# nelaturuharsha/TurboPrune

Measured on NVIDIA H100. Metric: images_per_sec_resnet50_erk80_train_step, higher is better.
Workload: dtype bf16

## Files before the change

include/turboprune_b200.h:

```cpp
#ifndef TURBOPRUNE_B200_H
#define TURBOPRUNE_B200_H

#include <stddef.h>
#include <stdint.h>

#ifdef __cplusplus
extern "C" {
#endif

#define TP_OK                 0
#define TP_ERR_INVALID       -1
#define TP_ERR_WORKSPACE     -2
#define TP_ERR_CUDA          -3
#define TP_ERR_K_RANGE       -4
#define TP_ERR_UNSUPPORTED   -5
#define TP_ERR_DEVICE        -6

const char* tp_strerror(int code);
const char* tp_last_cuda_error(void);
int         tp_abi_version(void);
int         tp_device_sm_count(void);
int         tp_set_pdl(int on);

#define TP_SCORE_MAG      0
#define TP_SCORE_SNIP     1
#define TP_SCORE_SYNFLOW  2

size_t tp_topk_workspace_bytes(int n_seg, int64_t total_numel);
int tp_topk_threshold_mask(const void* const* w, const void* const* g, const void* const* m,
                           void* const* mask_out, const int64_t* numel, int n_seg,
                           int64_t k, int score_kind, float* thr_out,
                           void* ws, size_t ws_bytes, int64_t* info_out, void* stream);
int tp_topk_enqueue(const void* const* w, const void* const* g, const void* const* m,
                    void* const* mask_out, const int64_t* numel, int n_seg,
                    int64_t k, int score_kind, float* thr_out,
                    void* ws, size_t ws_bytes, int table_cached, void* stream);
int tp_topk_finish(const void* const* m, void* const* mask_out, const int64_t* numel, int n_seg,
                   int64_t k, int score_kind, float* thr_out,
                   void* ws, size_t ws_bytes, int64_t* info_out, void* stream);

int tp_apply_threshold(const void* const* w, const void* const* g, const void* const* m,
                       void* const* mask_out, const int64_t* numel, int n_seg,
                       int score_kind, const float* thr, void* ws, size_t ws_bytes, void* stream);

int tp_count_zeros(const void* const* m, const int64_t* numel, int n_seg,
                   int64_t* zeros_out, void* ws, size_t ws_bytes, void* stream);

size_t tp_rigl_workspace_bytes(int n_seg, int64_t total_numel);
int tp_rigl_select(const void* const* w, const void* const* g, const void* const* mask, void* const* new_mask_out,
                   const int64_t* numel, const int64_t* k, int n_seg, int64_t* counts_out, void* ws, size_t ws_bytes,
                   void* stream);
int tp_rigl_apply(void* const* mask, const void* const* new_mask, void* const* w, void* const* momentum,
                  const int64_t* numel, int n_seg, void* ws, size_t ws_bytes, void* stream);
int tp_rigl_apply_states(void* const* mask, const void* const* new_mask, void* const* w, void* const* states, int n_states,
                         const int64_t* numel, int n_seg, void* ws, size_t ws_bytes, void* stream);

int tp_stage_weights(const void* w, const void* mask, int cout, int cin, int r, int s,
                     void* wf, int cin_p, int wf_ld, void* wd, int cout_p, int cin_p2,
                     void* kmask_f, void* kmask_d, void* stream);
size_t tp_kblock_mask_words(int64_t columns);

typedef struct tp_stage_item {
  const void* w; const void* mask;
  void* wf; void* wd;
  int32_t cout, cin, r, s, cin_p, cout_p, wf_ld;
  void* kmask_f; void* kmask_d;
} tp_stage_item;
size_t tp_stage_batched_workspace_bytes(int n_items);
int tp_stage_weights_batched(const tp_stage_item* items, int n_items, int table_cached, void* kmask_all, size_t kmask_bytes,
                             void* ws, size_t ws_bytes, void* stream);

int tp_to_nhwc_bf16(const void* src, int src_dtype, int64_t sn, int64_t sc, int64_t sh, int64_t sw,
                    int n, int c, int h, int w, void* dst, int c_pad, void* stream);

int tp_im2col_c8(const void* x, int n, int h, int w, int r, int s, int stride_h, int stride_w,
                 int pad_h, int pad_w, int p, int q, void* xcol, int kp, void* stream);

int tp_im2col_stem(const void* src, int src_dtype, int64_t sn, int64_t sc, int64_t sh, int64_t sw,
                   int n, int c, int h, int w, int r, int s, int cg, int stride_h, int stride_w, int pad_h, int pad_w,
                   int p, int q, void* xcol, int kp, void* stream);

int tp_cifar_augment(const void* src, void* out, const int64_t* idx, const int64_t* shifts, const uint8_t* flip,
                     const int64_t* cut_y, const int64_t* cut_x, int cut_size,
                     int n, int c, int h, int w, int r, void* stream);
typedef struct tp_crop_entry {
  const void* src;
  int32_t H, W;
  int32_t top, left, h, w;
  int32_t flip;
  int32_t reserved;
} tp_crop_entry;
int tp_resized_crop(const tp_crop_entry* table, int n, int size, const float* mean255, const float* std255, void* out,
                    void* stream);
int tp_synth_normal(void* out, int64_t numel, uint64_t seed, uint64_t counter_offset, int raw_words, void* stream);
int tp_synth_labels(void* out, int64_t numel, int num_classes, uint64_t seed, uint64_t counter_offset, void* stream);

typedef struct tp_conv_desc {
  int32_t n, h, w, cin;
  int32_t cout, r, s;
  int32_t stride_h, stride_w, pad_h, pad_w;
  int32_t p, q;
} tp_conv_desc;

size_t tp_conv_workspace_bytes(const tp_conv_desc* d, int op);

int tp_conv_fprop(const tp_conv_desc* d, const void* x, const void* wf, const void* bias_f32,
                  void* y, void* ws, size_t ws_bytes, void* stream);
size_t tp_conv_stats_rows(const tp_conv_desc* d);
int tp_conv_fprop_stats(const tp_conv_desc* d, const void* x, const void* wf, const void* kmask_f, const void* bias_f32,
                        void* y, void* stats, void* ws, size_t ws_bytes, void* stream);
int tp_conv_dgrad(const tp_conv_desc* d, const void* dy, const void* wd, const void* kmask_d, const void* addend,
                  void* dx, void* ws, size_t ws_bytes, void* stream);
size_t tp_conv_dgrad_partial_rows(const tp_conv_desc* d);
int tp_conv_dgrad_bnrelu(const tp_conv_desc* d, const void* dy, const void* wd, const void* kmask_d,
                         const void* bn_y, const void* bn_weight, const void* bn_bias, const void* bn_mean, const void* bn_invstd,
                         void* g, void* partial, void* stream);
int tp_conv_wgrad(const tp_conv_desc* d, const void* x, const void* dy, const void* mask, const void* kmask_f,
                  int cin_real, void* dw, void* db, void* ws, size_t ws_bytes, void* stream);

int tp_conv_fprop_f32(const tp_conv_desc* d, const void* x, const void* wf, const void* bias_f32, void* y, void* stream);
int tp_conv_dgrad_f32(const tp_conv_desc* d, const void* dy, const void* wd, void* dx, void* stream);
int tp_wgrad_split3(const void* src, int64_t sn, int64_t sc, int64_t sh, int64_t sw,
                    int n, int c, int h, int w, void* dst, int c_pad, int lo_block, void* stream);
int tp_stage_weights_f32(const void* w, const void* mask, int cout, int cin, int r, int s,
                         void* wf, int cin_p, int wf_ld, void* wd, int cout_p, void* stream);
int tp_stage_weights_batched_f32(const tp_stage_item* items, int n_items, int table_cached, void* ws, size_t ws_bytes,
                                 void* stream);
int tp_to_nhwc_f32(const void* src, int64_t sn, int64_t sc, int64_t sh, int64_t sw,
                   int n, int c, int h, int w, void* dst, int c_pad, void* stream);
int tp_im2col_stem_f32(const void* src, int64_t sn, int64_t sc, int64_t sh, int64_t sw,
                       int n, int c, int h, int w, int r, int s, int cg, int stride_h, int stride_w, int pad_h, int pad_w,
                       int p, int q, void* xcol, int kp, void* stream);

int tp_bn_forward_ext(const void* y, const void* residual, void* z, int64_t M, int C,
                      const void* weight, const void* bias, void* running_mean, void* running_var,
                      void* num_batches_tracked, float momentum, float eps, int training, int relu,
                      void* save_mean, void* save_invstd, const void* ext_stats, int64_t ext_rows,
                      void* ws, size_t ws_bytes, void* stream);

size_t tp_bn_workspace_bytes(int64_t m, int c);
int tp_bn_forward(const void* y, const void* residual, void* z, int64_t m, int c,
                  const void* weight, const void* bias, void* running_mean, void* running_var,
                  void* num_batches_tracked, float momentum, float eps, int training, int relu,
                  void* save_mean, void* save_invstd, void* ws, size_t ws_bytes, void* stream);
int tp_bn_backward(const void* dz, const void* z, const void* y, int64_t m, int c, const void* weight, const void* bias,
                   const void* save_mean, const void* save_invstd, int relu, void* dy, void* dres,
                   void* dweight, void* dbias, void* ws, size_t ws_bytes, void* stream);

int tp_bn_backward_ext(const void* g, const void* y, int64_t M, int C, const void* weight, const void* bias,
                       const void* save_mean, const void* save_invstd, const void* partial_rows, int64_t n_rows,
                       void* dy, void* dweight, void* dbias, void* ws, size_t ws_bytes, void* stream);
int tp_maxpool_forward(const void* x, void* y, void* idx, int n, int h, int w, int c, int k, int stride, int pad,
                       int p, int q, void* stream);
int tp_maxpool_backward(const void* dy, const void* idx, void* dx, int n, int h, int w, int c, int k, int stride, int pad,
                        int p, int q, void* stream);

int tp_sgd_momentum(void* const* w, const void* const* g, void* const* buf, const int64_t* numel,
                    int n_seg, const float* lr_dev, float momentum, float weight_decay,
                    int first_step, int table_cached, void* ws, size_t ws_bytes, void* stream);
size_t tp_segtable_workspace_bytes(int n_seg);
int tp_adamw(void* const* w, const void* const* g, void* const* exp_avg, void* const* exp_avg_sq, void* const* step,
             const int64_t* numel, int n_seg, const float* inv_lr_dev, const float* decay_dev,
             double beta1, double beta2, double eps, int table_cached, void* ws, size_t ws_bytes, void* stream);

int tp_p2p_allreduce_mask(void* const* peer_bufs, void* const* signal_pads, int rank, int world,
                          int64_t numel, const void* mask, float scale, void* out,
                          int algo, int timeout_ms, int* status_dev, void* stream);

int tp_p2p_allreduce_nvls(void* const* peer_bufs, void* const* signal_pads, void* multicast_buf, int rank, int world,
                          int64_t numel, const void* mask, float scale, void* out,
                          int timeout_ms, int* status_dev, void* stream);

#ifdef __cplusplus
}
#endif
#endif
```

turboprune_b200/_cabi.py:

```python
import ctypes
import os
from ctypes import POINTER, c_char_p, c_double, c_float, c_int, c_int32, c_int64, c_size_t, c_uint64, c_void_p

from . import build as _build

TP_SCORE_MAG, TP_SCORE_SNIP, TP_SCORE_SYNFLOW = 0, 1, 2
TP_ERR_K_RANGE = -4

_lib = None


class ConvDesc(ctypes.Structure):
    _fields_ = [(n, c_int32) for n in
                ("n", "h", "w", "cin", "cout", "r", "s", "stride_h", "stride_w", "pad_h", "pad_w", "p", "q")]


class StageItem(ctypes.Structure):
    _fields_ = [("w", c_void_p), ("mask", c_void_p), ("wf", c_void_p), ("wd", c_void_p)] + \
               [(n, c_int32) for n in ("cout", "cin", "r", "s", "cin_p", "cout_p", "wf_ld")] + \
               [("kmask_f", c_void_p), ("kmask_d", c_void_p)]


class CropEntry(ctypes.Structure):
    _fields_ = [("src", c_void_p)] + [(n, c_int32) for n in ("H", "W", "top", "left", "h", "w", "flip", "reserved")]


SIGNATURES = {
    "tp_strerror": (c_char_p, [c_int]),
    "tp_last_cuda_error": (c_char_p, []),
    "tp_abi_version": (c_int, []),
    "tp_device_sm_count": (c_int, []),
    "tp_set_pdl": (c_int, [c_int]),
    "tp_topk_workspace_bytes": (c_size_t, [c_int, c_int64]),
    "tp_topk_threshold_mask": (c_int, [POINTER(c_void_p), POINTER(c_void_p), POINTER(c_void_p), POINTER(c_void_p),
                                       POINTER(c_int64), c_int, c_int64, c_int, c_void_p, c_void_p, c_size_t,
                                       POINTER(c_int64), c_void_p]),
    "tp_topk_enqueue": (c_int, [POINTER(c_void_p), POINTER(c_void_p), POINTER(c_void_p), POINTER(c_void_p),
                                POINTER(c_int64), c_int, c_int64, c_int, c_void_p, c_void_p, c_size_t, c_int, c_void_p]),
    "tp_topk_finish": (c_int, [POINTER(c_void_p), POINTER(c_void_p), POINTER(c_int64), c_int, c_int64, c_int, c_void_p,
                               c_void_p, c_size_t, POINTER(c_int64), c_void_p]),
    "tp_apply_threshold": (c_int, [POINTER(c_void_p), POINTER(c_void_p), POINTER(c_void_p), POINTER(c_void_p),
                                   POINTER(c_int64), c_int, c_int, c_void_p, c_void_p, c_size_t, c_void_p]),
    "tp_count_zeros": (c_int, [POINTER(c_void_p), POINTER(c_int64), c_int, c_void_p, c_void_p, c_size_t, c_void_p]),
    "tp_rigl_workspace_bytes": (c_size_t, [c_int, c_int64]),
    "tp_rigl_select": (c_int, [POINTER(c_void_p), POINTER(c_void_p), POINTER(c_void_p), POINTER(c_void_p), POINTER(c_int64),
                               POINTER(c_int64), c_int, c_void_p, c_void_p, c_size_t, c_void_p]),
    "tp_rigl_apply": (c_int, [POINTER(c_void_p), POINTER(c_void_p), POINTER(c_void_p), POINTER(c_void_p), POINTER(c_int64), c_int,
                              c_void_p, c_size_t, c_void_p]),
    "tp_stage_weights": (c_int, [c_void_p, c_void_p, c_int, c_int, c_int, c_int, c_void_p, c_int, c_int, c_void_p, c_int,
                                 c_int, c_void_p, c_void_p, c_void_p]),
    "tp_kblock_mask_words": (c_size_t, [c_int64]),
    "tp_stage_batched_workspace_bytes": (c_size_t, [c_int]),
    "tp_stage_weights_batched": (c_int, [POINTER(StageItem), c_int, c_int, c_void_p, c_size_t, c_void_p, c_size_t, c_void_p]),
    "tp_to_nhwc_bf16": (c_int, [c_void_p, c_int, c_int64, c_int64, c_int64, c_int64, c_int, c_int, c_int, c_int,
                                c_void_p, c_int, c_void_p]),
    "tp_im2col_c8": (c_int, [c_void_p] + [c_int] * 11 + [c_void_p, c_int, c_void_p]),
    "tp_im2col_stem": (c_int, [c_void_p, c_int, c_int64, c_int64, c_int64, c_int64] + [c_int] * 13 + [c_void_p, c_int, c_void_p]),
    "tp_cifar_augment": (c_int, [c_void_p, c_void_p, c_void_p, c_void_p, c_void_p, c_void_p, c_void_p, c_int, c_int, c_int, c_int, c_int, c_int, c_void_p]),
    "tp_resized_crop": (c_int, [c_void_p, c_int, c_int, POINTER(c_float), POINTER(c_float), c_void_p, c_void_p]),
    "tp_synth_normal": (c_int, [c_void_p, c_int64, c_uint64, c_uint64, c_int, c_void_p]),
    "tp_synth_labels": (c_int, [c_void_p, c_int64, c_int, c_uint64, c_uint64, c_void_p]),
    "tp_conv_workspace_bytes": (c_size_t, [POINTER(ConvDesc), c_int]),
    "tp_conv_fprop": (c_int, [POINTER(ConvDesc), c_void_p, c_void_p, c_void_p, c_void_p, c_void_p, c_size_t, c_void_p]),
    "tp_conv_stats_rows": (c_size_t, [POINTER(ConvDesc)]),
    "tp_conv_fprop_stats": (c_int, [POINTER(ConvDesc), c_void_p, c_void_p, c_void_p, c_void_p, c_void_p, c_void_p, c_void_p, c_size_t, c_void_p]),
    "tp_conv_dgrad": (c_int, [POINTER(ConvDesc), c_void_p, c_void_p, c_void_p, c_void_p, c_void_p, c_void_p, c_size_t, c_void_p]),
    "tp_conv_dgrad_partial_rows": (c_size_t, [POINTER(ConvDesc)]),
    "tp_conv_dgrad_bnrelu": (c_int, [POINTER(ConvDesc), c_void_p, c_void_p, c_void_p, c_void_p, c_void_p, c_void_p, c_void_p, c_void_p,
                                     c_void_p, c_void_p, c_void_p]),
    "tp_bn_backward_ext": (c_int, [c_void_p, c_void_p, c_int64, c_int, c_void_p, c_void_p, c_void_p, c_void_p, c_void_p, c_int64,
                                   c_void_p, c_void_p, c_void_p, c_void_p, c_size_t, c_void_p]),
    "tp_conv_wgrad": (c_int, [POINTER(ConvDesc), c_void_p, c_void_p, c_void_p, c_void_p, c_int, c_void_p, c_void_p, c_void_p,
                              c_size_t, c_void_p]),
    "tp_sgd_momentum": (c_int, [POINTER(c_void_p), POINTER(c_void_p), POINTER(c_void_p), POINTER(c_int64), c_int,
                                c_void_p, c_float, c_float, c_int, c_int, c_void_p, c_size_t, c_void_p]),
    "tp_segtable_workspace_bytes": (c_size_t, [c_int]),
    "tp_adamw": (c_int, [POINTER(c_void_p), POINTER(c_void_p), POINTER(c_void_p), POINTER(c_void_p), POINTER(c_void_p),
                         POINTER(c_int64), c_int, c_void_p, c_void_p, c_double, c_double, c_double, c_int, c_void_p,
                         c_size_t, c_void_p]),
    "tp_rigl_apply_states": (c_int, [POINTER(c_void_p), POINTER(c_void_p), POINTER(c_void_p), POINTER(c_void_p), c_int,
                                     POINTER(c_int64), c_int, c_void_p, c_size_t, c_void_p]),
    "tp_p2p_allreduce_mask": (c_int, [POINTER(c_void_p), POINTER(c_void_p), c_int, c_int, c_int64, c_void_p, c_float,
                                      c_void_p, c_int, c_int, c_void_p, c_void_p]),
    "tp_bn_workspace_bytes": (c_size_t, [c_int64, c_int]),
    "tp_bn_forward": (c_int, [c_void_p, c_void_p, c_void_p, c_int64, c_int, c_void_p, c_void_p, c_void_p, c_void_p, c_void_p,
                              c_float, c_float, c_int, c_int, c_void_p, c_void_p, c_void_p, c_size_t, c_void_p]),
    "tp_bn_forward_ext": (c_int, [c_void_p, c_void_p, c_void_p, c_int64, c_int, c_void_p, c_void_p, c_void_p, c_void_p, c_void_p,
                                  c_float, c_float, c_int, c_int, c_void_p, c_void_p, c_void_p, c_int64, c_void_p, c_size_t, c_void_p]),
    "tp_bn_backward": (c_int, [c_void_p, c_void_p, c_void_p, c_int64, c_int, c_void_p, c_void_p, c_void_p, c_void_p, c_int, c_void_p,
                               c_void_p, c_void_p, c_void_p, c_void_p, c_size_t, c_void_p]),
    "tp_maxpool_forward": (c_int, [c_void_p, c_void_p, c_void_p] + [c_int] * 9 + [c_void_p]),
    "tp_maxpool_backward": (c_int, [c_void_p, c_void_p, c_void_p] + [c_int] * 9 + [c_void_p]),
    "tp_p2p_allreduce_nvls": (c_int, [POINTER(c_void_p), POINTER(c_void_p), c_void_p, c_int, c_int, c_int64, c_void_p, c_float,
                                      c_void_p, c_int, c_void_p, c_void_p]),
    "tp_conv_fprop_f32": (c_int, [POINTER(ConvDesc), c_void_p, c_void_p, c_void_p, c_void_p, c_void_p]),
    "tp_conv_dgrad_f32": (c_int, [POINTER(ConvDesc), c_void_p, c_void_p, c_void_p, c_void_p]),
    "tp_wgrad_split3": (c_int, [c_void_p, c_int64, c_int64, c_int64, c_int64, c_int, c_int, c_int, c_int, c_void_p, c_int, c_int,
                                c_void_p]),
    "tp_stage_weights_f32": (c_int, [c_void_p, c_void_p, c_int, c_int, c_int, c_int, c_void_p, c_int, c_int, c_void_p, c_int,
                                     c_void_p]),
    "tp_stage_weights_batched_f32": (c_int, [POINTER(StageItem), c_int, c_int, c_void_p, c_size_t, c_void_p]),
    "tp_to_nhwc_f32": (c_int, [c_void_p, c_int64, c_int64, c_int64, c_int64, c_int, c_int, c_int, c_int, c_void_p, c_int, c_void_p]),
    "tp_im2col_stem_f32": (c_int, [c_void_p, c_int64, c_int64, c_int64, c_int64] + [c_int] * 13 + [c_void_p, c_int, c_void_p]),
}


def lib_path() -> str:
    return _build.lib_path()


def load(build_if_missing: bool = False):
    global _lib
    if _lib is not None:
        return _lib
    path = lib_path()
    if not os.path.isfile(path):
        if build_if_missing:
            _build.build()
        else:
            raise RuntimeError(
                f"turboprune_b200: CUDA library not built ({path} missing). "
                "Run `python -c 'import __graft_entry__ as g; g.build()'`; there is no CPU fallback.")
    lib = ctypes.CDLL(path)
    for name, (res, args) in SIGNATURES.items():
        fn = getattr(lib, name)
        fn.restype = res
        fn.argtypes = args
    _lib = lib
    return lib


class TurboPruneError(RuntimeError):
    def __init__(self, code, where):
        lib = load()
        msg = lib.tp_strerror(code).decode()
        detail = lib.tp_last_cuda_error().decode() if code == -3 else ""
        super().__init__(f"{where}: {msg} (code {code}) {detail}".strip())
        self.code = code


def check(code: int, where: str):
    if code != 0:
        raise TurboPruneError(code, where)


def ptr_array(tensors):
    if tensors is None:
        return None
    arr = (c_void_p * len(tensors))()
    for i, t in enumerate(tensors):
        arr[i] = t.data_ptr() if t is not None else None
    return arr


def i64_array(vals):
    arr = (c_int64 * len(vals))()
    for i, v in enumerate(vals):
        arr[i] = int(v)
    return arr


def stream_ptr(device=None):
    import torch
    return c_void_p(torch.cuda.current_stream(device).cuda_stream)
```

turboprune_b200/csrc/tp_igemm.cu:

```cuda
#include "tp_common.cuh"
#include "tp_ptx.cuh"
#include <cuda.h>
#include <mutex>

namespace tp {
using namespace ptx;

constexpr int kBlockM = 128;
constexpr int kBlockK = 64;
constexpr int kConsumers = 256;
constexpr int kThreads = kConsumers + 32;
constexpr int kProducerWarp = kConsumers / 32;
constexpr int kFwdThreads = 3 * 128;
constexpr int kMaxTaps = 64;

constexpr int kFwdProducerRegs = 56, kFwdConsumerRegs = 224;
static_assert(kFwdProducerRegs * 128 + kFwdConsumerRegs * 256 <= 168 * kFwdThreads, "fwd register split");

__host__ __device__ constexpr int fwd_stages(int block_n) { return block_n == 128 ? 5 : 8; }
__host__ __device__ constexpr int fwd_stg_bytes(int block_n) { return kBlockM * block_n * 2; }
__host__ __device__ constexpr int fwd_smem(int block_n) {
  return fwd_stages(block_n) * (kBlockM * kBlockK * 2 + block_n * kBlockK * 2) + 2 * fwd_stg_bytes(block_n) + 1024 + 512;
}

struct TapEntry { uint16_t off_w, off_h; int32_t kofs; };

constexpr int kMaxCls = 4;

struct ClsEntry {
  int M;
  int P_it, Q_it;
  int ntaps, tap0;
  int base_w, base_h;
  int oah, oaw;
  int tile0, m_groups;
};

struct FwdParams {
  int M, N;
  int ncls;
  ClsEntry cls[kMaxCls];
  int cchunks;
  int a_mode;
  int step_w, step_h;
  long long out_img_pix;
  int out_row_pix;
  int osh, osw;
  int linear;
  int ldc;
  int staged_store;
  __nv_bfloat16* out;
  const float* bias;
  const __nv_bfloat16* addend;
  float* stats;
  const __nv_bfloat16* bn_y;
  const float* bn_weight; const float* bn_bias; const float* bn_mean; const float* bn_invstd;
  const uint32_t* kmask;
  int kmask_words;
  TapEntry taps[kMaxTaps];
};

__device__ __forceinline__ const uint32_t* live_kmask(const uint32_t* km, int words, int N) {
  if (km && __ldg(km + (size_t)((N + 63) >> 6) * words) == 0u) return nullptr;
  return km;
}

struct KSkip {
  const uint32_t* base; int words, g0, g1; int cur_w; uint32_t bits;
  __device__ __forceinline__ void begin(const uint32_t* km, int wds, int n0, int block_n, int N) {
    base = km; words = wds; cur_w = -1; bits = 0u;
    g0 = n0 >> 6; g1 = min((min(n0 + block_n, N) + 63) >> 6, ((N + 63) >> 6));
  }
  __device__ __forceinline__ bool on(int kb) {
    const int wi = kb >> 5;
    if (wi != cur_w) {
      cur_w = wi; bits = 0u;
      if (wi < words) for (int g = g0; g < g1; ++g) bits |= __ldg(base + (size_t)g * words + wi);
      else bits = 0xffffffffu;
    }
    return (bits >> (kb & 31)) & 1u;
  }
  __device__ __forceinline__ bool take(int kb, bool last, bool any) { return on(kb) || (last && !any); }
};

struct WgParams {
  int Mc;
  int Kpix;
  int P_it, Q_it;
  int chunks, cchunks;
  int nb;
  int b_mode;
  int base_w, base_h, step_w, step_h;
  int m_tiles, n_tiles, splits, kb_per_split, kblocks;
  float* partial;
  const uint32_t* kmask;
  int kmask_words;
  TapEntry taps[kMaxTaps];
};

struct WgItem {
  int split, tile, m_t, n_t, chunk0, nvalid, kb0, kb1;
  __device__ __forceinline__ void set_tile(int m, int n, int m_tiles, int nb, int chunks) {
    m_t = m; n_t = n; tile = n * m_tiles + m;
    chunk0 = n * nb; nvalid = min(nb, chunks - chunk0);
  }
  __device__ __forceinline__ bool empty(const uint32_t* __restrict__ km, int words, int Mc) const {
    const int row_groups = (Mc + 63) >> 6;
    for (int r = 2 * m_t; r < 2 * m_t + 2 && r < row_groups; ++r)
      for (int c = chunk0; c < chunk0 + nvalid; ++c)
        if ((__ldg(km + (size_t)r * words + (c >> 5)) >> (c & 31)) & 1u) return false;
    return true;
  }
};

__device__ __forceinline__ WgItem wg_item(const WgParams& p, int nb, int item) {
  WgItem w;
  const int ntile = p.m_tiles * p.n_tiles;
  w.split = item / ntile;
  const int tile = item - w.split * ntile, n_t = tile / p.m_tiles;
  w.set_tile(tile - n_t * p.m_tiles, n_t, p.m_tiles, nb, p.chunks);
  w.kb0 = w.split * p.kb_per_split; w.kb1 = min(p.kblocks, w.kb0 + p.kb_per_split);
  return w;
}

__device__ __forceinline__ void decompose_pixel(int m, int P, int Q, int& n, int& p, int& q) {
  q = m % Q; int t = m / Q; p = t % P; n = t / P;
}

struct AMaps { CUtensorMap m[kMaxCls]; };

__device__ __forceinline__ void decode_tile(const FwdParams& p, int tile, int n_tiles, int& c, int& m_g, int& n_t) {
  c = 0;
#pragma unroll
  for (int j = 1; j < kMaxCls; ++j) if (j < p.ncls && tile >= p.cls[j].tile0) c = j;
  const int local = tile - p.cls[c].tile0;
  m_g = local / n_tiles; n_t = local - m_g * n_tiles;
}

template <int BLOCK_N, typename T = __nv_bfloat16>
__device__ __forceinline__ void fwd_mma_block(float (&acc)[BLOCK_N], uint32_t a_addr, uint32_t b_addr, uint32_t accumulate) {
  const uint64_t adesc = make_smem_desc(a_addr, 16, 1024);
  const uint64_t adesc_hi = make_smem_desc(a_addr + 64 * kBlockK * 2, 16, 1024);
  const uint64_t bdesc = make_smem_desc(b_addr, 16, 1024);
#pragma unroll
  for (int k = 0; k < kBlockK / 16; ++k) {
    if constexpr (sizeof(T) == 4) {
      if constexpr (BLOCK_N == 128) {
        wgmma_m64n128_tf32(acc, adesc + (uint64_t)(2 * k), bdesc + (uint64_t)(2 * k), accumulate | (uint32_t)k);
        wgmma_m64n128_tf32(acc + BLOCK_N / 2, adesc_hi + (uint64_t)(2 * k), bdesc + (uint64_t)(2 * k), accumulate | (uint32_t)k);
      } else {
        wgmma_m64n64_tf32(acc, adesc + (uint64_t)(2 * k), bdesc + (uint64_t)(2 * k), accumulate | (uint32_t)k);
        wgmma_m64n64_tf32(acc + BLOCK_N / 2, adesc_hi + (uint64_t)(2 * k), bdesc + (uint64_t)(2 * k), accumulate | (uint32_t)k);
      }
    } else if constexpr (BLOCK_N == 128) {
      wgmma_m64n128<0, 0>(acc, adesc + (uint64_t)(2 * k), bdesc + (uint64_t)(2 * k), accumulate | (uint32_t)k);
      wgmma_m64n128<0, 0>(acc + BLOCK_N / 2, adesc_hi + (uint64_t)(2 * k), bdesc + (uint64_t)(2 * k), accumulate | (uint32_t)k);
    } else {
      wgmma_m64n64<0, 0>(acc, adesc + (uint64_t)(2 * k), bdesc + (uint64_t)(2 * k), accumulate | (uint32_t)k);
      wgmma_m64n64<0, 0>(acc + BLOCK_N / 2, adesc_hi + (uint64_t)(2 * k), bdesc + (uint64_t)(2 * k), accumulate | (uint32_t)k);
    }
  }
}

template <int BLOCK_N, bool MULTI, bool BNB, typename T = __nv_bfloat16>
__global__ void __launch_bounds__(kFwdThreads, 1)
k_igemm_fwd(const __grid_constant__ AMaps tmA, const __grid_constant__ CUtensorMap tmB,
            const __grid_constant__ FwdParams p) {
  static_assert(BLOCK_N == 64 || BLOCK_N == 128, "wgmma N of the fwd kernel");
  static_assert(!BNB || !MULTI, "BatchNorm-backward epilogue: single class");
  constexpr bool kF32 = sizeof(T) == 4;
  static_assert(!kF32 || !BNB, "fp32 operands: no BatchNorm-backward epilogue");
  constexpr int kKe = 128 / (int)sizeof(T);
  constexpr int kABytes = kBlockM * kBlockK * 2;
  constexpr int kBBytes = BLOCK_N * kBlockK * 2;
  constexpr int kStageBytes = kABytes + kBBytes;
  constexpr int kStages = fwd_stages(BLOCK_N);
  extern __shared__ __align__(1024) uint8_t smem_raw[];
  uint8_t* smem = (uint8_t*)(((uintptr_t)smem_raw + 1023) & ~(uintptr_t)1023);
  pdl_trigger();
  constexpr int kStgBytes = fwd_stg_bytes(BLOCK_N);
  constexpr int kChunkStg = kBlockM * 64 * 2;
  uint8_t* const stg_base = smem + kStages * kStageBytes;
  uint64_t* full_bar = (uint64_t*)(stg_base + 2 * kStgBytes);
  uint64_t* empty_bar = full_bar + kStages;
  uint64_t* order_bar = empty_bar + kStages;
  int* ring_pos = (int*)(order_bar + 2);

  const int warp = threadIdx.x >> 5, lane = threadIdx.x & 31;
  const int n_tiles = (p.N + BLOCK_N - 1) / BLOCK_N;
  const int total_tiles = p.cls[p.ncls - 1].tile0 + p.cls[p.ncls - 1].m_groups * n_tiles;
  const int my_items = total_tiles > (int)blockIdx.x ? (total_tiles - (int)blockIdx.x + (int)gridDim.x - 1) / (int)gridDim.x : 0;
  auto get_tile = [&](int w, int& ci, int& m_g, int& n_t) {
    ci = 0;
    const int tile = (int)blockIdx.x + w * (int)gridDim.x;
    if (MULTI) decode_tile(p, tile, n_tiles, ci, m_g, n_t);
    else { m_g = tile / n_tiles; n_t = tile - m_g * n_tiles; }
  };

  if (threadIdx.x == 0) {
    for (int j = 0; j < p.ncls; ++j) prefetch_tmap(&tmA.m[j]);
    prefetch_tmap(&tmB);
    for (int i = 0; i < kStages; ++i) { mbar_init(&full_bar[i], 1); mbar_init(&empty_bar[i], 1); }
    mbar_init(&order_bar[0], 1); mbar_init(&order_bar[1], 1);
    fence_mbar_init();
  }
  __syncthreads();
  pdl_wait();

  if (warp < 4) {
    setmaxnreg_dec<kFwdProducerRegs>();
    if (threadIdx.x == 0) {
      int stage = 0; uint32_t phase = 0;
      const uint32_t* const km = kF32 ? nullptr : live_kmask(p.kmask, p.kmask_words, p.N);
      for (int w = 0; w < my_items; ++w) {
        int ci, m_g, n_t; get_tile(w, ci, m_g, n_t);
        const ClsEntry& ce = p.cls[MULTI ? ci : 0];
        const CUtensorMap* const mapA = &tmA.m[MULTI ? ci : 0];
        const int m0 = m_g * kBlockM;
        int cn = 0, cp = 0, cq = 0;
        if (p.a_mode == 1) decompose_pixel(m0, ce.P_it, ce.Q_it, cn, cp, cq);
        const int cw = ce.base_w + cq * p.step_w, ch = ce.base_h + cp * p.step_h;
        auto load_block = [&](const TapEntry& te, int cc) {
          mbar_wait(&empty_bar[stage], phase ^ 1);
          uint8_t* sA = smem + stage * kStageBytes;
          uint8_t* sB = sA + kABytes;
          mbar_arrive_expect_tx(&full_bar[stage], kStageBytes);
          if (p.a_mode == 1)
            tma_load_im2col_4d(sA, mapA, &full_bar[stage], cc * kKe, cw, ch, cn, te.off_w, te.off_h);
          else
            tma_load_2d(sA, mapA, &full_bar[stage], te.kofs + cc * kKe, m0);
          tma_load_2d(sB, &tmB, &full_bar[stage], te.kofs + cc * kKe, n_t * BLOCK_N);
          if (++stage == kStages) { stage = 0; phase ^= 1; }
        };
        const int tap_base = MULTI ? ce.tap0 : 0;
        if (!km) {
          for (int tap = 0; tap < ce.ntaps; ++tap) {
            const TapEntry te = p.taps[tap_base + tap];
            for (int cc = 0; cc < p.cchunks; ++cc) load_block(te, cc);
          }
        } else {
          KSkip ks; bool any = false;
          ks.begin(km, p.kmask_words, n_t * BLOCK_N, BLOCK_N, p.N);
          for (int tap = 0; tap < ce.ntaps; ++tap) {
            const TapEntry te = p.taps[tap_base + tap];
            for (int cc = 0; cc < p.cchunks; ++cc) {
              const bool last = tap == ce.ntaps - 1 && cc == p.cchunks - 1;
              if (!ks.take((te.kofs >> 6) + cc, last, any)) continue;
              any = true;
              load_block(te, cc);
            }
          }
        }
      }
    }
  } else {
    setmaxnreg_inc<kFwdConsumerRegs>();
    const int cw = (warp >> 2) - 1;
    const int q = warp & 3;
    const int wtid = threadIdx.x & 127;
    const int bar_id = 1 + cw;
    const uint32_t* const km = kF32 ? nullptr : live_kmask(p.kmask, p.kmask_words, p.N);
    const uint32_t stg = smem_u32(stg_base + cw * kStgBytes);
    const int fr0 = q * 16 + (lane >> 2);
    const uint32_t fsw = (uint32_t)(lane >> 2);
    const uint32_t frag_base = stg + (uint32_t)(fr0 * 128 + (lane & 3) * 4);
    const int r_in = lane >> 3, c16 = lane & 7;
    const uint32_t buf = stg + (uint32_t)(q * 32 * 128);
    const uint32_t rd_even = buf + r_in * 128 + ((uint32_t)(c16 ^ r_in) << 4);
    const uint32_t rd_odd = buf + (r_in + 4) * 128 + ((uint32_t)(c16 ^ (r_in + 4)) << 4);
    for (int it = 0, w = cw; w < my_items; ++it, w += 2) {
      int ci, m_g, n_t; get_tile(w, ci, m_g, n_t);
      const ClsEntry& ce = p.cls[MULTI ? ci : 0];
      const bool has_acc = MULTI ? ce.ntaps > 0 : true;
      const int m_t = m_g;

      int stage = 0; uint32_t phase = 0;
      const int turn = it + cw;
      if (turn > 0) {
        mbar_wait(&order_bar[cw], (uint32_t)((turn - 1) & 1));
        const int pos = *(volatile int*)ring_pos;
        stage = pos >> 1; phase = (uint32_t)(pos & 1);
      }
      bar_sync(bar_id, 128);
      auto pass_turn = [&]() {
        if (wtid == 0) { *(volatile int*)ring_pos = stage * 2 + (int)phase; mbar_arrive(&order_bar[cw ^ 1]); }
      };
      float acc[BLOCK_N];
      if (has_acc) {
#pragma unroll
        for (int i = 0; i < BLOCK_N; ++i) acc[i] = 0.f;
        int prev = -1;
        auto mma_block = [&](uint32_t accumulate) {
          mbar_wait(&full_bar[stage], phase);
          const uint32_t s_addr = smem_u32(smem + stage * kStageBytes);
          wgmma_fence();
          fwd_mma_block<BLOCK_N, T>(acc, s_addr, s_addr + kABytes, accumulate);
          wgmma_commit();
          wgmma_wait<1>();
          if (prev >= 0 && wtid == 0) mbar_arrive(&empty_bar[prev]);
          prev = stage;
          if (++stage == kStages) { stage = 0; phase ^= 1; }
        };
        KSkip ks; uint32_t any = 0;
        if (km) ks.begin(km, p.kmask_words, n_t * BLOCK_N, BLOCK_N, p.N);
        for (int tap = 0; tap < ce.ntaps; ++tap) {
          const int kb0 = p.taps[(MULTI ? ce.tap0 : 0) + tap].kofs >> 6;
          for (int cc = 0; cc < p.cchunks; ++cc) {
            const bool last = tap == ce.ntaps - 1 && cc == p.cchunks - 1;
            if (km && !ks.take(kb0 + cc, last, any)) continue;
            mma_block(any);
            any = 1;
          }
        }
        pass_turn();
        wgmma_wait<0>();
        acc_fence(acc);
        if (prev >= 0 && wtid == 0) mbar_arrive(&empty_bar[prev]);
      } else {
        pass_turn();
      }

      const long long wrow0 = (long long)m_t * kBlockM + q * 32;
      const int rows_left = (int)(ce.M - wrow0 < 32 ? (ce.M - wrow0 < 0 ? 0 : ce.M - wrow0) : 32);
      const long long ldc = p.ldc;
      const int N = p.N;
      long long ooff[MULTI ? 8 : 1];
      const long long rbase = (wrow0 + r_in) * ldc + c16 * 8;
      if (MULTI && p.staged_store) {
        int n, pp, qq; decompose_pixel((int)(wrow0 + r_in), ce.P_it, ce.Q_it, n, pp, qq);
#pragma unroll
        for (int i = 0; i < 8; ++i) {
          const long long px = (long long)n * p.out_img_pix + (long long)(pp * p.osh + ce.oah) * p.out_row_pix + (qq * p.osw + ce.oaw);
          ooff[i] = px * ldc + c16 * 8;
          qq += 4;
          while (qq >= ce.Q_it) { qq -= ce.Q_it; if (++pp == ce.P_it) { pp = 0; ++n; } }
        }
      }
      auto row_off = [&](int i) -> long long { return MULTI ? ooff[MULTI ? i : 0] : rbase + (long long)(i * 4) * ldc; };
      if constexpr (kF32) {
        float* const out = reinterpret_cast<float*>(p.out);
        const bool pair_ok = (p.ldc & 1) == 0 && (((uintptr_t)out) & 7) == 0;
#pragma unroll
        for (int mh = 0; mh < 2; ++mh)
#pragma unroll
          for (int h = 0; h < 2; ++h) {
            const int row = m_t * kBlockM + fr0 + 8 * h + 64 * mh;
            if (row >= ce.M) continue;
            long long opix = row;
            if (MULTI || !p.linear) {
              int n, pp, qq; decompose_pixel(row, ce.P_it, ce.Q_it, n, pp, qq);
              opix = (long long)n * p.out_img_pix + (long long)(pp * p.osh + ce.oah) * p.out_row_pix + (qq * p.osw + ce.oaw);
            }
            float* const orow = out + opix * p.ldc;
#pragma unroll
            for (int j = 0; j < BLOCK_N / 8; ++j) {
              const int n = n_t * BLOCK_N + 8 * j + 2 * (lane & 3);
              if (n >= N) continue;
              const int i = mh * (BLOCK_N / 2) + 4 * j + 2 * h;
              float f0 = has_acc ? acc[i] : 0.f, f1 = has_acc ? acc[i + 1] : 0.f;
              if (p.bias && has_acc) {
                f0 += p.bias[n];
                if (n + 1 < N) f1 += p.bias[n + 1];
              }
              if (n + 1 < N && pair_ok) *reinterpret_cast<float2*>(orow + n) = make_float2(f0, f1);
              else {
                orow[n] = f0;
                if (n + 1 < N) orow[n + 1] = f1;
              }
            }
          }
        continue;
      }
      if (MULTI && !has_acc) {
        if (p.staged_store) {
#pragma unroll 1
          for (int c = 0; c < BLOCK_N; c += 64) {
            const int n0 = n_t * BLOCK_N + c;
            if (n0 >= N) break;
            if (n0 + c16 * 8 + 8 > N) continue;
            uint4 z[8];
#pragma unroll
            for (int i = 0; i < 8; ++i) {
              z[i] = make_uint4(0u, 0u, 0u, 0u);
              if (p.addend && i * 4 + r_in < rows_left) z[i] = *reinterpret_cast<const uint4*>(p.addend + row_off(i) + n0);
            }
#pragma unroll
            for (int i = 0; i < 8; ++i)
              if (i * 4 + r_in < rows_left) *reinterpret_cast<uint4*>(p.out + row_off(i) + n0) = z[i];
          }
        } else {
          const int row = m_t * kBlockM + wtid;
          if (row < ce.M) {
            int n, pp, qq; decompose_pixel(row, ce.P_it, ce.Q_it, n, pp, qq);
            const long long opix = (long long)n * p.out_img_pix + (long long)(pp * p.osh + ce.oah) * p.out_row_pix + (qq * p.osw + ce.oaw);
            for (int j = n_t * BLOCK_N; j < min(p.N, (n_t + 1) * BLOCK_N); ++j)
              p.out[opix * p.ldc + j] = p.addend ? p.addend[opix * p.ldc + j] : __float2bfloat16_rn(0.f);
          }
        }
        continue;
      }
      if (p.staged_store) {
        __nv_bfloat16* const gout = p.out;
        const __nv_bfloat16* const gadd = p.addend;
        const float* bias = p.bias;
        float* stats = p.stats ? p.stats + (long long)(m_t * 4 + q) * 2 * N + c16 * 8 : nullptr;
        if (gadd) {
          __syncwarp();
#pragma unroll
          for (int ch = 0; ch < BLOCK_N / 64; ++ch) {
            const int n0 = n_t * BLOCK_N + ch * 64;
            if (n0 >= N) break;
            const bool col_ok = n0 + c16 * 8 + 8 <= N;
            uint4 a[8];
#pragma unroll
            for (int i = 0; i < 8; ++i) {
              a[i] = make_uint4(0u, 0u, 0u, 0u);
              if (i * 4 + r_in < rows_left && col_ok) a[i] = *reinterpret_cast<const uint4*>(gadd + row_off(i) + n0);
            }
#pragma unroll
            for (int i = 0; i < 8; ++i) sts128(((i & 1) ? rd_odd : rd_even) + (uint32_t)(ch * kChunkStg + (i >> 1) * 1024), a[i]);
          }
        }
        bar_sync(bar_id, 128);
#pragma unroll
        for (int ch = 0; ch < BLOCK_N / 64; ++ch) {
          const int n0 = n_t * BLOCK_N + ch * 64;
          if (n0 >= N) break;
#pragma unroll
          for (int mh = 0; mh < 2; ++mh)
#pragma unroll
            for (int h = 0; h < 2; ++h)
#pragma unroll
              for (int j = 0; j < 8; ++j) {
                const int i = mh * (BLOCK_N / 2) + 4 * (ch * 8 + j) + 2 * h;
                float f0 = acc[i], f1 = acc[i + 1];
                const int n = n0 + 8 * j + 2 * (lane & 3);
                if (bias) {
                  if (n < N) f0 += bias[n];
                  if (n + 1 < N) f1 += bias[n + 1];
                }
                const uint32_t addr = frag_base + (uint32_t)(ch * kChunkStg + (64 * mh + 8 * h) * 128) + (((uint32_t)j ^ fsw) << 4);
                if (gadd) {
                  const uint32_t a = lds32(addr);
                  const float2 t2 = __bfloat1622float2(*reinterpret_cast<const __nv_bfloat162*>(&a));
                  f0 += t2.x; f1 += t2.y;
                }
                const __nv_bfloat162 hv = __floats2bfloat162_rn(f0, f1);
                sts32(addr, *reinterpret_cast<const uint32_t*>(&hv));
              }
        }
        bar_sync(bar_id, 128);
#pragma unroll 1
        for (int ch = 0; ch < BLOCK_N / 64; ++ch) {
          const int n0 = n_t * BLOCK_N + ch * 64;
          if (n0 >= N) break;
          const bool col_ok = n0 + c16 * 8 + 8 <= N;
          uint4 o[8];
#pragma unroll
          for (int i = 0; i < 8; ++i) o[i] = lds128(((i & 1) ? rd_odd : rd_even) + (uint32_t)(ch * kChunkStg + (i >> 1) * 1024));
          float s1[8], s2[8];
#pragma unroll
          for (int qq = 0; qq < 8; ++qq) { s1[qq] = 0.f; s2[qq] = 0.f; }
          if (BNB) {
            uint4 yv[8];
#pragma unroll
            for (int i = 0; i < 8; ++i) {
              yv[i] = make_uint4(0u, 0u, 0u, 0u);
              if (i * 4 + r_in < rows_left && col_ok) yv[i] = *reinterpret_cast<const uint4*>(p.bn_y + row_off(i) + n0);
            }
            float sc[8], sf[8], is_[8], nm[8];
            if (col_ok) {
              const int cb = n0 + c16 * 8;
#pragma unroll
              for (int qq = 0; qq < 8; qq += 4) {
                const float4 one4 = make_float4(1.f, 1.f, 1.f, 1.f), zero4 = make_float4(0.f, 0.f, 0.f, 0.f);
                const float4 a4 = p.bn_weight ? *reinterpret_cast<const float4*>(p.bn_weight + cb + qq) : one4;
                const float4 b4 = p.bn_bias ? *reinterpret_cast<const float4*>(p.bn_bias + cb + qq) : zero4;
                const float4 m4 = *reinterpret_cast<const float4*>(p.bn_mean + cb + qq), i4 = *reinterpret_cast<const float4*>(p.bn_invstd + cb + qq);
                is_[qq] = i4.x; is_[qq + 1] = i4.y; is_[qq + 2] = i4.z; is_[qq + 3] = i4.w;
                nm[qq] = m4.x; nm[qq + 1] = m4.y; nm[qq + 2] = m4.z; nm[qq + 3] = m4.w;
                sc[qq] = a4.x * i4.x; sc[qq + 1] = a4.y * i4.y; sc[qq + 2] = a4.z * i4.z; sc[qq + 3] = a4.w * i4.w;
                sf[qq] = fmaf(-m4.x, sc[qq], b4.x); sf[qq + 1] = fmaf(-m4.y, sc[qq + 1], b4.y);
                sf[qq + 2] = fmaf(-m4.z, sc[qq + 2], b4.z); sf[qq + 3] = fmaf(-m4.w, sc[qq + 3], b4.w);
              }
            } else {
#pragma unroll
              for (int qq = 0; qq < 8; ++qq) { sc[qq] = 0.f; sf[qq] = 0.f; is_[qq] = 0.f; nm[qq] = 0.f; }
            }
#pragma unroll
            for (int i = 0; i < 8; ++i) {
              if (i * 4 + r_in < rows_left) {
                __nv_bfloat162* gh = reinterpret_cast<__nv_bfloat162*>(&o[i]);
                const __nv_bfloat162* yh = reinterpret_cast<const __nv_bfloat162*>(&yv[i]);
#pragma unroll
                for (int qq = 0; qq < 4; ++qq) {
                  float2 d2 = __bfloat1622float2(gh[qq]);
                  const float2 y2 = __bfloat1622float2(yh[qq]);
                  if (!(fmaf(y2.x, sc[2 * qq], sf[2 * qq]) > 0.f)) d2.x = 0.f;
                  if (!(fmaf(y2.y, sc[2 * qq + 1], sf[2 * qq + 1]) > 0.f)) d2.y = 0.f;
                  gh[qq] = __floats2bfloat162_rn(d2.x, d2.y);
                  s1[2 * qq] += d2.x;     s2[2 * qq] = fmaf(d2.x, (y2.x - nm[2 * qq]) * is_[2 * qq], s2[2 * qq]);
                  s1[2 * qq + 1] += d2.y; s2[2 * qq + 1] = fmaf(d2.y, (y2.y - nm[2 * qq + 1]) * is_[2 * qq + 1], s2[2 * qq + 1]);
                }
              }
            }
          }
#pragma unroll
          for (int i = 0; i < 8; ++i)
            if (i * 4 + r_in < rows_left && col_ok) *reinterpret_cast<uint4*>(gout + row_off(i) + n0) = o[i];
          if (!BNB && stats) {
#pragma unroll
            for (int i = 0; i < 8; ++i) {
              if (i * 4 + r_in < rows_left) {
                const __nv_bfloat162* h2 = reinterpret_cast<const __nv_bfloat162*>(&o[i]);
#pragma unroll
                for (int qq = 0; qq < 4; ++qq) {
                  const float2 t2 = __bfloat1622float2(h2[qq]);
                  s1[2 * qq] += t2.x; s2[2 * qq] = fmaf(t2.x, t2.x, s2[2 * qq]);
                  s1[2 * qq + 1] += t2.y; s2[2 * qq + 1] = fmaf(t2.y, t2.y, s2[2 * qq + 1]);
                }
              }
            }
          }
          if (BNB || stats) {
#pragma unroll
            for (int qq = 0; qq < 8; ++qq) {
              s1[qq] += __shfl_xor_sync(0xffffffffu, s1[qq], 8);  s2[qq] += __shfl_xor_sync(0xffffffffu, s2[qq], 8);
              s1[qq] += __shfl_xor_sync(0xffffffffu, s1[qq], 16); s2[qq] += __shfl_xor_sync(0xffffffffu, s2[qq], 16);
            }
            if (r_in == 0 && col_ok) {
              float4* d1 = reinterpret_cast<float4*>(stats + n0);
              float4* d2 = reinterpret_cast<float4*>(stats + N + n0);
              d1[0] = make_float4(s1[0], s1[1], s1[2], s1[3]); d1[1] = make_float4(s1[4], s1[5], s1[6], s1[7]);
              d2[0] = make_float4(s2[0], s2[1], s2[2], s2[3]); d2[1] = make_float4(s2[4], s2[5], s2[6], s2[7]);
            }
          }
        }
      } else {
#pragma unroll
        for (int mh = 0; mh < 2; ++mh)
#pragma unroll
          for (int h = 0; h < 2; ++h) {
            const int row = m_t * kBlockM + fr0 + 8 * h + 64 * mh;
            if (row >= ce.M) continue;
            long long opix = row;
            if (MULTI || !p.linear) {
              int n, pp, qq; decompose_pixel(row, ce.P_it, ce.Q_it, n, pp, qq);
              opix = (long long)n * p.out_img_pix + (long long)(pp * p.osh + ce.oah) * p.out_row_pix + (qq * p.osw + ce.oaw);
            }
            __nv_bfloat16* const orow = p.out + opix * p.ldc;
#pragma unroll
            for (int j = 0; j < BLOCK_N / 8; ++j)
#pragma unroll
              for (int e = 0; e < 2; ++e) {
                const int n = n_t * BLOCK_N + 8 * j + 2 * (lane & 3) + e;
                if (n >= N) continue;
                float f = acc[mh * (BLOCK_N / 2) + 4 * j + 2 * h + e];
                if (p.bias) f += p.bias[n];
                if (p.addend) f += __bfloat162float(p.addend[opix * p.ldc + n]);
                orow[n] = __float2bfloat16_rn(f);
              }
          }
      }
    }
  }
}

template <int NB>
__device__ __forceinline__ void wgrad_mma_block(float (&acc)[NB * 32], uint32_t a_addr, uint32_t b_addr, bool first) {
  constexpr uint32_t kChunk = 64 * kBlockK * 2;
#pragma unroll
  for (int k = 0; k < kBlockK / 16; ++k) {
    const uint32_t acc_on = (!first || k > 0) ? 1u : 0u;
    const uint64_t adesc = make_smem_desc(a_addr + (uint32_t)(2048 * k), kChunk, 1024);
    const uint32_t bk = b_addr + (uint32_t)(2048 * k);
    if constexpr (NB >= 2) wgmma_m64n128<1, 1>(acc, adesc, make_smem_desc(bk, kChunk, 1024), acc_on);
    else wgmma_m64n64<1, 1>(acc, adesc, make_smem_desc(bk, kChunk, 1024), acc_on);
    if constexpr (NB == 4) wgmma_m64n128<1, 1>(acc + 64, adesc, make_smem_desc(bk + 2 * kChunk, kChunk, 1024), acc_on);
    if constexpr (NB == 3) wgmma_m64n64<1, 1>(acc + 64, adesc, make_smem_desc(bk + 2 * kChunk, kChunk, 1024), acc_on);
  }
}

template <int NB>
__global__ void __launch_bounds__(kThreads, 1)
k_igemm_wgrad(const __grid_constant__ CUtensorMap tmA ,
              const __grid_constant__ CUtensorMap tmB ,
              const __grid_constant__ WgParams p) {
  constexpr int kABytes = kBlockM * kBlockK * 2;
  constexpr int kChunkBytes = 64 * kBlockK * 2;
  constexpr int kMaxNb = 4;
  constexpr int kStageBytes = kABytes + kMaxNb * kChunkBytes;
  constexpr int kStages = 4;
  pdl_trigger();
  extern __shared__ __align__(1024) uint8_t smem_raw[];
  uint8_t* smem = (uint8_t*)(((uintptr_t)smem_raw + 1023) & ~(uintptr_t)1023);
  uint64_t* full_bar = (uint64_t*)(smem + kStages * kStageBytes);
  uint64_t* empty_bar = full_bar + kStages;

  const int warp = threadIdx.x >> 5, lane = threadIdx.x & 31;
  const int items = p.m_tiles * p.n_tiles * p.splits;
  constexpr int ncols = NB * 64;

  if (threadIdx.x == 0) {
    prefetch_tmap(&tmA); prefetch_tmap(&tmB);
    for (int i = 0; i < kStages; ++i) { mbar_init(&full_bar[i], 1); mbar_init(&empty_bar[i], kConsumers / 128); }
    fence_mbar_init();
  }
  __syncthreads();
  pdl_wait();
  const uint32_t* const km = live_kmask(p.kmask, p.kmask_words, p.Mc);

  if (warp == kProducerWarp) {
    if (lane == 0) {
      int stage = 0; uint32_t phase = 0;
      for (int item = blockIdx.x; item < items; item += gridDim.x) {
        const WgItem it = wg_item(p, NB, item);
        if (km && it.empty(km, p.kmask_words, p.Mc)) continue;
        const int m_t = it.m_t, chunk0 = it.chunk0, nvalid = it.nvalid, kb0 = it.kb0, kb1 = it.kb1;
        int c_c[4]; uint16_t c_ow[4], c_oh[4];
#pragma unroll
        for (int j = 0; j < 4; ++j) {
          const int chunk = min(chunk0 + j, p.chunks - 1), tap = chunk / p.cchunks;
          c_c[j] = (chunk - tap * p.cchunks) * 64; c_ow[j] = p.taps[tap].off_w; c_oh[j] = p.taps[tap].off_h;
        }
        int cn, cp, cq; decompose_pixel(kb0 * kBlockK, p.P_it, p.Q_it, cn, cp, cq);
        const int sq = kBlockK % p.Q_it, t1 = kBlockK / p.Q_it, sp = t1 % p.P_it, sn = t1 / p.P_it;
        for (int kb = kb0; kb < kb1; ++kb) {
          const int pix0 = kb * kBlockK;
          mbar_wait(&empty_bar[stage], phase ^ 1);
          mbar_arrive_expect_tx(&full_bar[stage], kABytes + nvalid * kChunkBytes);
          uint8_t* sA = smem + stage * kStageBytes;
          uint8_t* sB = sA + kABytes;
          tma_load_2d(sA, &tmA, &full_bar[stage], m_t * kBlockM, pix0);
          tma_load_2d(sA + kChunkBytes, &tmA, &full_bar[stage], m_t * kBlockM + 64, pix0);
          if (p.b_mode == 1) {
            const int cw = p.base_w + cq * p.step_w, ch = p.base_h + cp * p.step_h;
#pragma unroll
            for (int j = 0; j < 4; ++j)
              if (j < nvalid)
                tma_load_im2col_4d(sB + j * kChunkBytes, &tmB, &full_bar[stage], c_c[j], cw, ch, cn, c_ow[j], c_oh[j]);
            cq += sq; if (cq >= p.Q_it) { cq -= p.Q_it; cp += 1; }
            cp += sp; if (cp >= p.P_it) { cp -= p.P_it; cn += 1; }
            cn += sn;
          } else {
#pragma unroll
            for (int j = 0; j < 4; ++j)
              if (j < nvalid) tma_load_2d(sB + j * kChunkBytes, &tmB, &full_bar[stage], (chunk0 + j) * 64, pix0);
          }
          if (++stage == kStages) { stage = 0; phase ^= 1; }
        }
      }
    }
  } else {
    const int wg = warp >> 2;
    int stage = 0; uint32_t phase = 0;
    for (int item = blockIdx.x; item < items; item += gridDim.x) {
      const WgItem it = wg_item(p, NB, item);
      if (km && it.empty(km, p.kmask_words, p.Mc)) continue;
      const int kb0 = it.kb0, kb1 = it.kb1;
      float acc[NB * 32];
#pragma unroll
      for (int i = 0; i < NB * 32; ++i) acc[i] = 0.f;
      int prev = -1;
      for (int kb = kb0; kb < kb1; ++kb) {
        mbar_wait(&full_bar[stage], phase);
        const uint32_t a_addr = smem_u32(smem + stage * kStageBytes);
        wgmma_fence();
        wgrad_mma_block<NB>(acc, a_addr + (uint32_t)(wg * kChunkBytes), a_addr + kABytes, kb == kb0);
        wgmma_commit();
        wgmma_wait<1>();
        if (prev >= 0 && (threadIdx.x & 127) == 0) mbar_arrive(&empty_bar[prev]);
        prev = stage;
        if (++stage == kStages) { stage = 0; phase ^= 1; }
      }
      wgmma_wait<0>();
      acc_fence(acc);
      if (prev >= 0 && (threadIdx.x & 127) == 0) mbar_arrive(&empty_bar[prev]);
      float* ptile = p.partial + ((long long)it.tile * p.splits + it.split) * kBlockM * ncols;
      const int r0 = wg * 64 + (warp & 3) * 16 + (lane >> 2);
#pragma unroll
      for (int j = 0; j < ncols / 8; ++j)
#pragma unroll
        for (int h = 0; h < 2; ++h)
          *reinterpret_cast<float2*>(ptile + (long long)(r0 + 8 * h) * ncols + 8 * j + 2 * (lane & 3)) =
              make_float2(acc[4 * j + 2 * h], acc[4 * j + 2 * h + 1]);
    }
  }
}

__global__ void __launch_bounds__(256) k_wgrad_finalize(const float* __restrict__ partial, const float* __restrict__ mask,
                                                        float* __restrict__ dw, int cout, int cin_real, int cin_p, int rs,
                                                        int nb, int m_tiles, int splits, int sl,
                                                        const uint32_t* __restrict__ kmask, int kmask_words) {
  pdl_enter();
  __shared__ float s_lane[256];
  const uint32_t* const km = live_kmask(kmask, kmask_words, cout);
  const int co = blockIdx.x;
  const int r = co % kBlockM;
  const int ktot = rs * cin_p;
  const int ncols = nb * 64;
  const int KT = 256 / sl;
  const int kl = threadIdx.x % KT, sj = threadIdx.x / KT;
  const int kk = blockIdx.y * KT + kl;
  const long long sstride = (long long)kBlockM * ncols;
  float a[8] = {0.f, 0.f, 0.f, 0.f, 0.f, 0.f, 0.f, 0.f};
  bool skipped = false;
  if (kk < ktot) {
    const int chunk = kk >> 6;
    WgItem it; it.set_tile(co / kBlockM, chunk / nb, m_tiles, nb, (ktot + 63) >> 6);
    skipped = km && it.empty(km, kmask_words, cout);
    if (!skipped) {
      const float* base = partial + (((long long)it.tile * splits) * kBlockM + r) * ncols + (chunk - it.chunk0) * 64 + (kk & 63);
      int sp = sj;
      for (; sp + 7 * sl < splits; sp += 8 * sl) {
        float v[8];
#pragma unroll
        for (int j = 0; j < 8; ++j) v[j] = __ldcs(base + (long long)(sp + j * sl) * sstride);
#pragma unroll
        for (int j = 0; j < 8; ++j) a[j] += v[j];
      }
      for (; sp < splits; sp += sl) a[0] += __ldcs(base + (long long)sp * sstride);
    }
  }
  s_lane[sj * KT + kl] = ((a[0] + a[1]) + (a[2] + a[3])) + ((a[4] + a[5]) + (a[6] + a[7]));
  __syncthreads();
  if (sj == 0 && kk < ktot) {
    float acc = 0.f;
    for (int j = 0; j < sl; ++j) acc += s_lane[j * KT + kl];
    const int tap = kk / cin_p, ci = kk - tap * cin_p;
    if (ci < cin_real) {
      const long long o = ((long long)co * cin_real + ci) * rs + tap;
      dw[o] = skipped ? 0.f : mask[o] * acc;
    }
  }
}

__global__ void __launch_bounds__(256) k_colsum_part(const __nv_bfloat16* __restrict__ dy, long long npix, int c, int ldc,
                                                     float* __restrict__ part) {
  pdl_enter();
  __shared__ float s_acc[256][9];
  const int tx = threadIdx.x, ty = threadIdx.y, TX = blockDim.x, TY = blockDim.y;
  const int cvec = blockIdx.y * TX + tx;
  const bool act = cvec * 8 < c;
  float a[8];
#pragma unroll
  for (int i = 0; i < 8; ++i) a[i] = 0.f;
  auto add8 = [&](const uint4& v) {
    const __nv_bfloat162* h = reinterpret_cast<const __nv_bfloat162*>(&v);
#pragma unroll
    for (int i = 0; i < 4; ++i) { const float2 f = __bfloat1622float2(h[i]); a[2 * i] += f.x; a[2 * i + 1] += f.y; }
  };
  if (act) {
    const long long stride = (long long)gridDim.x * TY;
    long long p = (long long)blockIdx.x * TY + ty;
    const __nv_bfloat16* src = dy + (size_t)cvec * 8;
    for (; p + 3 * stride < npix; p += 4 * stride) {
      uint4 v[4];
#pragma unroll
      for (int u = 0; u < 4; ++u) v[u] = *reinterpret_cast<const uint4*>(src + (size_t)(p + u * stride) * ldc);
#pragma unroll
      for (int u = 0; u < 4; ++u) add8(v[u]);
    }
    for (; p < npix; p += stride) add8(*reinterpret_cast<const uint4*>(src + (size_t)p * ldc));
  }
  const int tid = ty * TX + tx;
#pragma unroll
  for (int i = 0; i < 8; ++i) s_acc[tid][i] = a[i];
  __syncthreads();
  if (ty == 0 && act) {
    float r[8];
#pragma unroll
    for (int i = 0; i < 8; ++i) r[i] = 0.f;
    for (int j = 0; j < TY; ++j)
#pragma unroll
      for (int i = 0; i < 8; ++i) r[i] += s_acc[j * TX + tx][i];
#pragma unroll
    for (int i = 0; i < 8; ++i) part[(size_t)blockIdx.x * c + cvec * 8 + i] = r[i];
  }
}

__global__ void __launch_bounds__(256) k_colsum_fold(const float* __restrict__ part, int nparts, int c, float* __restrict__ db) {
  pdl_enter();
  const int ch = blockIdx.x * blockDim.x + threadIdx.x;
  if (ch >= c) return;
  float s0 = 0.f, s1 = 0.f, s2 = 0.f, s3 = 0.f;
  int j = 0;
  for (; j + 3 < nparts; j += 4) {
    s0 += part[(size_t)j * c + ch]; s1 += part[(size_t)(j + 1) * c + ch];
    s2 += part[(size_t)(j + 2) * c + ch]; s3 += part[(size_t)(j + 3) * c + ch];
  }
  for (; j < nparts; ++j) s0 += part[(size_t)j * c + ch];
  db[ch] = (s0 + s1) + (s2 + s3);
}

typedef CUresult (*PFN_encodeTiled)(CUtensorMap*, CUtensorMapDataType, cuuint32_t, void*, const cuuint64_t*, const cuuint64_t*,
                                    const cuuint32_t*, const cuuint32_t*, CUtensorMapInterleave, CUtensorMapSwizzle,
                                    CUtensorMapL2promotion, CUtensorMapFloatOOBfill);
typedef CUresult (*PFN_encodeIm2col)(CUtensorMap*, CUtensorMapDataType, cuuint32_t, void*, const cuuint64_t*, const cuuint64_t*,
                                     const int*, const int*, cuuint32_t, cuuint32_t, const cuuint32_t*, CUtensorMapInterleave,
                                     CUtensorMapSwizzle, CUtensorMapL2promotion, CUtensorMapFloatOOBfill);
static PFN_encodeTiled g_encodeTiled = nullptr;
static PFN_encodeIm2col g_encodeIm2col = nullptr;
static int g_driver_version = 0;

static int load_driver_fns() {
  static std::once_flag once;
  static int rc = TP_OK;
  std::call_once(once, []() {
    void* f1 = nullptr; void* f2 = nullptr;
    cudaDriverEntryPointQueryResult q;
    if (cudaGetDriverEntryPoint("cuTensorMapEncodeTiled", &f1, cudaEnableDefault, &q) != cudaSuccess || !f1 ||
        cudaGetDriverEntryPoint("cuTensorMapEncodeIm2col", &f2, cudaEnableDefault, &q) != cudaSuccess || !f2) {
      set_last_cuda_error(cudaErrorUnknown, "cudaGetDriverEntryPoint(cuTensorMapEncode*)");
      rc = TP_ERR_CUDA;
      return;
    }
    g_encodeTiled = (PFN_encodeTiled)f1;
    g_encodeIm2col = (PFN_encodeIm2col)f2;
    cudaDriverGetVersion(&g_driver_version);
  });
  return rc;
}

static int fail_cu(CUresult r, const char* what) {
  static thread_local char buf[128];
  snprintf(buf, sizeof(buf), "%s -> CUresult %d", what, (int)r);
  set_last_cuda_error(cudaErrorInvalidValue, buf);
  return TP_ERR_CUDA;
}

static int make_tiled_map(CUtensorMap* m, const void* ptr, uint64_t cols, uint64_t rows, uint64_t ld_elems, uint32_t box_rows,
                          bool f32 = false) {
  cuuint64_t dims[2] = {cols, rows};
  cuuint64_t strides[1] = {ld_elems * (f32 ? 4 : 2)};
  cuuint32_t box[2] = {f32 ? 32u : 64u, box_rows};
  cuuint32_t es[2] = {1, 1};
  CUresult r = g_encodeTiled(m, f32 ? CU_TENSOR_MAP_DATA_TYPE_FLOAT32 : CU_TENSOR_MAP_DATA_TYPE_BFLOAT16, 2, const_cast<void*>(ptr),
                             dims, strides, box, es,
                             CU_TENSOR_MAP_INTERLEAVE_NONE, CU_TENSOR_MAP_SWIZZLE_128B,
                             CU_TENSOR_MAP_L2_PROMOTION_L2_256B, CU_TENSOR_MAP_FLOAT_OOB_FILL_NONE);
  if (r != CUDA_SUCCESS) return fail_cu(r, "cuTensorMapEncodeTiled");
  return TP_OK;
}

static int make_im2col_map(CUtensorMap* m, const void* ptr, int n, int h, int w, int c,
                           int base_w, int base_h, int step_w, int step_h, int P_it, int Q_it, uint32_t pixels, bool f32 = false) {
  const cuuint64_t es_b = f32 ? 4 : 2;
  cuuint64_t dims[4] = {(cuuint64_t)c, (cuuint64_t)w, (cuuint64_t)h, (cuuint64_t)n};
  cuuint64_t strides[3] = {(cuuint64_t)c * es_b, (cuuint64_t)w * c * es_b, (cuuint64_t)h * w * c * es_b};
  int lower[2] = {base_w, base_h};
  int upper[2] = {(Q_it - 1) * step_w + 1 + base_w - w, (P_it - 1) * step_h + 1 + base_h - h};
  cuuint32_t es[4] = {1, (cuuint32_t)step_w, (cuuint32_t)step_h, 1};
  CUresult r = g_encodeIm2col(m, f32 ? CU_TENSOR_MAP_DATA_TYPE_FLOAT32 : CU_TENSOR_MAP_DATA_TYPE_BFLOAT16, 4, const_cast<void*>(ptr),
                              dims, strides, lower, upper,
                              f32 ? 32 : 64, pixels, es, CU_TENSOR_MAP_INTERLEAVE_NONE, CU_TENSOR_MAP_SWIZZLE_128B,
                              CU_TENSOR_MAP_L2_PROMOTION_L2_256B, CU_TENSOR_MAP_FLOAT_OOB_FILL_NONE);
  if (r != CUDA_SUCCESS) return fail_cu(r, "cuTensorMapEncodeIm2col");
  if (g_driver_version <= 13010 && (size_t)n * h * w * c * es_b < 131072)
    reinterpret_cast<uint64_t*>(m)[1] &= ~(1ull << 21);
  return TP_OK;
}

struct WgGeom {
  int chunks, nb, m_tiles, n_tiles, kblocks, smax;
  size_t partial_bytes(int splits) const { return (size_t)m_tiles * n_tiles * splits * kBlockM * nb * 64 * sizeof(float); }
};

static WgGeom wgrad_geom(const tp_conv_desc* d) {
  WgGeom g;
  g.chunks = (d->r * d->s * d->cin + 63) / 64;
  g.nb = g.chunks >= 4 ? 4 : g.chunks;
  g.m_tiles = (d->cout + kBlockM - 1) / kBlockM;
  g.n_tiles = (g.chunks + g.nb - 1) / g.nb;
  g.kblocks = (int)(((long long)d->n * d->p * d->q + 63) / 64);
  g.smax = (2 * sm_count()) / (g.m_tiles * g.n_tiles);
  if (g.smax > g.kblocks) g.smax = g.kblocks;
  if (g.smax < 1) g.smax = 1;
  return g;
}

static int pick_wgrad_splits(const WgGeom& g) {
  const int sms = sm_count();
  const int tiles = g.m_tiles * g.n_tiles, kblocks = g.kblocks, nb = g.nb;
  const double c_kb = 0.30;
  const double c_part = 0.33 * nb;
  const double c_fin = 0.013 * nb;
  int best = 1; double best_cost = 1e30;
  for (int s = 1; s <= g.smax; ++s) {
    const int kb = (kblocks + s - 1) / s;
    const int s_eff = (kblocks + kb - 1) / kb;
    const long long items = (long long)tiles * s_eff;
    const long long waves = (items + sms - 1) / sms;
    const double cost = (double)waves * (kb * c_kb + c_part) + (double)items * c_fin;
    if (cost < best_cost - 1e-9) { best_cost = cost; best = s_eff; }
  }
  return best;
}

static bool is_plain_gemm(const tp_conv_desc* d) {
  return d->r == 1 && d->s == 1 && d->stride_h == 1 && d->stride_w == 1 && d->pad_h == 0 && d->pad_w == 0;
}

static void fill_taps(TapEntry* taps, int R, int S, int cin) {
  for (int r = 0; r < R; ++r) for (int s = 0; s < S; ++s) {
    TapEntry& t = taps[r * S + s];
    t.off_w = (uint16_t)s; t.off_h = (uint16_t)r; t.kofs = (r * S + s) * cin;
  }
}

static int pick_block_n(long long m_tiles, int n) {
  const int sms = sm_count();
  int best = 64; double best_score = -1;
  const int cands[2] = {128, 64};
  const double weight[2] = {1.0, 0.82};
  for (int i = 0; i < 2; ++i) {
    int bn = cands[i];
    if (bn > 64 && n <= bn / 2) continue;
    long long tiles = m_tiles * ((n + bn - 1) / bn);
    long long waves = (tiles + sms - 1) / sms;
    double eff = (double)tiles / (double)(waves * sms) * weight[i];
    if (eff > best_score) { best_score = eff; best = bn; }
  }
  return best;
}

constexpr int kSmemMax = 232448;

template <int BN, bool MULTI, bool BNB = false, typename T = __nv_bfloat16>
static int launch_fwd(const AMaps& a, const CUtensorMap& b, FwdParams& p, cudaStream_t st) {
  constexpr int smem = fwd_smem(BN);
  static_assert(smem <= kSmemMax, "fwd smem budget");
  const int n_tiles = (p.N + BN - 1) / BN;
  static bool attr_set = false;
  if (!attr_set) {
    TP_CUDA_CHECK(cudaFuncSetAttribute(k_igemm_fwd<BN, MULTI, BNB, T>, cudaFuncAttributeMaxDynamicSharedMemorySize, smem));
    attr_set = true;
  }
  long long ctiles = 0;
  for (int c = 0; c < p.ncls; ++c) {
    p.cls[c].m_groups = (int)((p.cls[c].M + kBlockM - 1) / kBlockM);
    if (ctiles > 0x7fffffffll) return TP_ERR_UNSUPPORTED;
    p.cls[c].tile0 = (int)ctiles;
    ctiles += (long long)p.cls[c].m_groups * n_tiles;
  }
  if (ctiles > 0x7fffffffll || ctiles <= 0) return TP_ERR_UNSUPPORTED;
  const int grid = (int)(ctiles < sm_count() ? ctiles : sm_count());
  TP_CUDA_CHECK(launch(k_igemm_fwd<BN, MULTI, BNB, T>, dim3(grid), dim3(kFwdThreads), (size_t)smem, st, a, b, p));
  TP_LAUNCH_CHECK();
  return TP_OK;
}

static int run_fwd(const AMaps& a, const CUtensorMap& b, FwdParams& p, int bn, cudaStream_t st, bool f32 = false) {
  p.linear = p.ncls == 1 && p.osh == 1 && p.osw == 1 && p.cls[0].oah == 0 && p.cls[0].oaw == 0 &&
             p.out_row_pix == p.cls[0].Q_it && p.out_img_pix == (long long)p.cls[0].P_it * p.cls[0].Q_it;
  if (f32) {
    if (p.stats || p.bn_y || p.addend || p.kmask) return TP_ERR_UNSUPPORTED;
    p.staged_store = 0;
    if (!p.linear) {
      if (bn == 128) return launch_fwd<128, true, false, float>(a, b, p, st);
      return launch_fwd<64, true, false, float>(a, b, p, st);
    }
    if (bn == 128) return launch_fwd<128, false, false, float>(a, b, p, st);
    return launch_fwd<64, false, false, float>(a, b, p, st);
  }
  p.staged_store = (p.ldc % 8 == 0 && p.N % 8 == 0 && (((uintptr_t)p.out) & 15) == 0 &&
                    (!p.addend || (((uintptr_t)p.addend) & 15) == 0)) ? 1 : 0;
  if (p.stats && !(p.staged_store && p.linear)) return TP_ERR_UNSUPPORTED;
  const bool multi = !p.linear;
  if (multi) {
    if (bn == 128) return launch_fwd<128, true>(a, b, p, st);
    return launch_fwd<64, true>(a, b, p, st);
  }
  if (p.bn_y) {
    if (!p.staged_store || !p.stats) return TP_ERR_UNSUPPORTED;
    if (bn == 128) return launch_fwd<128, false, true>(a, b, p, st);
    return launch_fwd<64, false, true>(a, b, p, st);
  }
  if (bn == 128) return launch_fwd<128, false>(a, b, p, st);
  return launch_fwd<64, false>(a, b, p, st);
}

template <int NB>
static int launch_wgrad(int grid, const CUtensorMap& ta, const CUtensorMap& tb, const WgParams& p, cudaStream_t st) {
  constexpr int smem = 4 * (kBlockM * kBlockK * 2 + 4 * 64 * kBlockK * 2) + 1024 + 256;
  static bool attr_set = false;
  if (!attr_set) {
    TP_CUDA_CHECK(cudaFuncSetAttribute(k_igemm_wgrad<NB>, cudaFuncAttributeMaxDynamicSharedMemorySize, smem));
    attr_set = true;
  }
  TP_CUDA_CHECK(launch(k_igemm_wgrad<NB>, dim3(grid), dim3(kThreads), (size_t)smem, st, ta, tb, p));
  TP_LAUNCH_CHECK();
  return TP_OK;
}

}

using namespace tp;

extern "C" {

size_t tp_conv_workspace_bytes(const tp_conv_desc* d, int op) {
  if (!d) return 0;
  if (op != 2) return 256;
  const WgGeom g = wgrad_geom(d);
  return g.partial_bytes(g.smax) + 1024;
}

size_t tp_conv_stats_rows(const tp_conv_desc* d) {
  if (!d) return 0;
  const long long M = (long long)d->n * d->p * d->q;
  return (size_t)((M + kBlockM - 1) / kBlockM) * 4;
}

int tp_conv_fprop(const tp_conv_desc* d, const void* x, const void* wf, const void* bias_f32,
                  void* y, void* ws, size_t ws_bytes, void* stream) {
  return tp_conv_fprop_stats(d, x, wf, nullptr, bias_f32, y, nullptr, ws, ws_bytes, stream);
}

static int conv_fprop_impl(const tp_conv_desc* d, const void* x, const void* wf, const void* kmask_f, const void* bias_f32,
                           void* y, void* stats, void* stream, bool f32);

int tp_conv_fprop_stats(const tp_conv_desc* d, const void* x, const void* wf, const void* kmask_f, const void* bias_f32,
                        void* y, void* stats, void* ws, size_t ws_bytes, void* stream) {
  (void)ws; (void)ws_bytes;
  return conv_fprop_impl(d, x, wf, kmask_f, bias_f32, y, stats, stream, false);
}

int tp_conv_fprop_f32(const tp_conv_desc* d, const void* x, const void* wf, const void* bias_f32, void* y, void* stream) {
  return conv_fprop_impl(d, x, wf, nullptr, bias_f32, y, nullptr, stream, true);
}

static int conv_fprop_impl(const tp_conv_desc* d, const void* x, const void* wf, const void* kmask_f, const void* bias_f32,
                           void* y, void* stats, void* stream, bool f32) {
  if (!d || !x || !wf || !y) return TP_ERR_INVALID;
  if (stats && (d->cout % 8 != 0 || (((uintptr_t)y) & 15) != 0 || (((uintptr_t)stats) & 15) != 0)) return TP_ERR_UNSUPPORTED;
  if (d->cin % 8 != 0 || d->r * d->s > kMaxTaps) return TP_ERR_UNSUPPORTED;
  if (d->r * d->s > 1 && d->cin % 64 != 0) return TP_ERR_UNSUPPORTED;
  int rc = load_driver_fns(); if (rc) return rc;
  rc = bind_device_of(d ? (const void*)x : nullptr); if (rc) return rc;
  cudaStream_t st = (cudaStream_t)stream;
  FwdParams p = {};
  p.M = d->n * d->p * d->q; p.N = d->cout;
  p.ncls = 1;
  ClsEntry& ce = p.cls[0];
  ce.M = p.M; ce.P_it = d->p; ce.Q_it = d->q; ce.ntaps = d->r * d->s; ce.tap0 = 0; ce.oah = 0; ce.oaw = 0;
  const int ke = f32 ? 32 : 64;
  p.cchunks = (d->cin + ke - 1) / ke;
  p.out_img_pix = (long long)d->p * d->q; p.out_row_pix = d->q;
  p.osh = 1; p.osw = 1;
  p.ldc = d->cout; p.out = (__nv_bfloat16*)y; p.bias = (const float*)bias_f32;
  p.stats = (float*)stats;
  p.kmask = (const uint32_t*)kmask_f; p.kmask_words = (int)tp_kblock_mask_words((int64_t)d->r * d->s * d->cin);
  fill_taps(p.taps, d->r, d->s, d->cin);
  AMaps ta; CUtensorMap tb;
  if (is_plain_gemm(d)) {
    p.a_mode = 0;
    rc = make_tiled_map(&ta.m[0], x, (uint64_t)d->cin, (uint64_t)p.M, (uint64_t)d->cin, kBlockM, f32); if (rc) return rc;
  } else {
    p.a_mode = 1;
    ce.base_w = -d->pad_w; ce.base_h = -d->pad_h; p.step_w = d->stride_w; p.step_h = d->stride_h;
    rc = make_im2col_map(&ta.m[0], x, d->n, d->h, d->w, d->cin, ce.base_w, ce.base_h, p.step_w, p.step_h, d->p, d->q, kBlockM, f32);
    if (rc) return rc;
  }
  for (int c = 1; c < kMaxCls; ++c) ta.m[c] = ta.m[0];
  const int bn = pick_block_n((p.M + kBlockM - 1) / kBlockM, p.N);
  rc = make_tiled_map(&tb, wf, (uint64_t)d->r * d->s * d->cin, (uint64_t)d->cout, (uint64_t)d->r * d->s * d->cin, (uint32_t)bn, f32);
  if (rc) return rc;
  return run_fwd(ta, tb, p, bn, st, f32);
}

struct BnGate { const void* y; const float* weight; const float* bias; const float* mean; const float* invstd; float* partial; };

static int conv_dgrad_impl(const tp_conv_desc* d, const void* dy, const void* wd, const void* kmask_d, const void* addend,
                           void* dx, const BnGate* gate, void* stream, bool f32 = false);

int tp_conv_dgrad(const tp_conv_desc* d, const void* dy, const void* wd, const void* kmask_d, const void* addend,
                  void* dx, void* ws, size_t ws_bytes, void* stream) {
  (void)ws; (void)ws_bytes;
  return conv_dgrad_impl(d, dy, wd, kmask_d, addend, dx, nullptr, stream);
}

int tp_conv_dgrad_f32(const tp_conv_desc* d, const void* dy, const void* wd, void* dx, void* stream) {
  return conv_dgrad_impl(d, dy, wd, nullptr, nullptr, dx, nullptr, stream, true);
}

int tp_conv_dgrad_bnrelu(const tp_conv_desc* d, const void* dy, const void* wd, const void* kmask_d,
                         const void* bn_y, const void* bn_weight, const void* bn_bias, const void* bn_mean, const void* bn_invstd,
                         void* g, void* partial, void* stream) {
  if (!d || !bn_y || !bn_mean || !bn_invstd || !partial) return TP_ERR_INVALID;
  if (d->stride_h != 1 || d->stride_w != 1 || d->cin % 8 != 0) return TP_ERR_UNSUPPORTED;
  if ((((uintptr_t)bn_y) | ((uintptr_t)bn_weight) | ((uintptr_t)bn_bias) | ((uintptr_t)bn_mean) | ((uintptr_t)bn_invstd) | ((uintptr_t)partial)) & 15)
    return TP_ERR_UNSUPPORTED;
  BnGate bn = {bn_y, (const float*)bn_weight, (const float*)bn_bias, (const float*)bn_mean, (const float*)bn_invstd, (float*)partial};
  return conv_dgrad_impl(d, dy, wd, kmask_d, nullptr, g, &bn, stream);
}

size_t tp_conv_dgrad_partial_rows(const tp_conv_desc* d) {
  if (!d) return 0;
  const long long M = (long long)d->n * d->h * d->w;
  return (size_t)((M + kBlockM - 1) / kBlockM) * 4;
}

static int conv_dgrad_impl(const tp_conv_desc* d, const void* dy, const void* wd, const void* kmask_d, const void* addend,
                           void* dx, const BnGate* gate, void* stream, bool f32) {
  if (!d || !dy || !wd || !dx) return TP_ERR_INVALID;
  const int cop = d->cout;
  if (cop % 8 != 0 || d->r * d->s > kMaxTaps) return TP_ERR_UNSUPPORTED;
  if (d->r * d->s > 1 && cop % 64 != 0) return TP_ERR_UNSUPPORTED;
  int rc = load_driver_fns(); if (rc) return rc;
  rc = bind_device_of(d ? (const void*)dy : nullptr); if (rc) return rc;
  cudaStream_t st = (cudaStream_t)stream;
  const int R = d->r, S = d->s;
  const long long ktot = (long long)R * S * cop;
  const int sh = d->stride_h, sw = d->stride_w;
  FwdParams p = {};
  p.N = d->cin;
  p.cchunks = f32 ? (cop + 31) / 32 : (cop + 63) / 64;
  p.out_img_pix = (long long)d->h * d->w; p.out_row_pix = d->w;
  p.ldc = d->cin; p.out = (__nv_bfloat16*)dx; p.bias = nullptr; p.addend = (const __nv_bfloat16*)addend;
  p.kmask = (const uint32_t*)kmask_d; p.kmask_words = (int)tp_kblock_mask_words(ktot);
  p.step_w = 1; p.step_h = 1;
  if (gate) {
    p.bn_y = (const __nv_bfloat16*)gate->y; p.bn_weight = gate->weight; p.bn_bias = gate->bias; p.bn_mean = gate->mean; p.bn_invstd = gate->invstd;
    p.stats = gate->partial;
  }
  AMaps ta; CUtensorMap tb;
  if (sh == 1 && sw == 1) {
    p.M = d->n * d->h * d->w;
    p.ncls = 1; p.osh = 1; p.osw = 1;
    ClsEntry& ce = p.cls[0];
    ce.M = p.M; ce.P_it = d->h; ce.Q_it = d->w; ce.ntaps = R * S; ce.tap0 = 0; ce.oah = 0; ce.oaw = 0;
    fill_taps(p.taps, R, S, cop);
    if (is_plain_gemm(d)) {
      p.a_mode = 0;
      rc = make_tiled_map(&ta.m[0], dy, (uint64_t)cop, (uint64_t)p.M, (uint64_t)cop, kBlockM, f32); if (rc) return rc;
    } else {
      p.a_mode = 1;
      ce.base_w = -(S - 1 - d->pad_w); ce.base_h = -(R - 1 - d->pad_h);
      rc = make_im2col_map(&ta.m[0], dy, d->n, d->p, d->q, cop, ce.base_w, ce.base_h, 1, 1, d->h, d->w, kBlockM, f32);
      if (rc) return rc;
    }
    for (int c = 1; c < kMaxCls; ++c) ta.m[c] = ta.m[0];
  } else {
    if (sh * sw > kMaxCls || R * S > kMaxTaps) return TP_ERR_UNSUPPORTED;
    p.a_mode = 1; p.osh = sh; p.osw = sw;
    int nc = 0, nt = 0; long long Mtot = 0;
    for (int a = 0; a < sh; ++a) for (int b = 0; b < sw; ++b) {
      const int Hc = (d->h - a + sh - 1) / sh, Wc = (d->w - b + sw - 1) / sw;
      if (Hc <= 0 || Wc <= 0) continue;
      ClsEntry& ce = p.cls[nc];
      ce.M = d->n * Hc * Wc; ce.P_it = Hc; ce.Q_it = Wc; ce.oah = a; ce.oaw = b; ce.tap0 = nt; ce.ntaps = 0;
      int dh_min = 1 << 30, dw_min = 1 << 30;
      for (int r = 0; r < R; ++r) if ((a + d->pad_h - r) % sh == 0) dh_min = min(dh_min, (a + d->pad_h - r) / sh);
      for (int s = 0; s < S; ++s) if ((b + d->pad_w - s) % sw == 0) dw_min = min(dw_min, (b + d->pad_w - s) / sw);
      if (dh_min != (1 << 30) && dw_min != (1 << 30)) {
        for (int r = 0; r < R; ++r) {
          if ((a + d->pad_h - r) % sh != 0) continue;
          for (int s = 0; s < S; ++s) {
            if ((b + d->pad_w - s) % sw != 0) continue;
            TapEntry& t = p.taps[nt++];
            t.off_h = (uint16_t)((a + d->pad_h - r) / sh - dh_min);
            t.off_w = (uint16_t)((b + d->pad_w - s) / sw - dw_min);
            t.kofs = ((R - 1 - r) * S + (S - 1 - s)) * cop;
            ++ce.ntaps;
          }
        }
      } else { dh_min = 0; dw_min = 0; }
      ce.base_w = dw_min; ce.base_h = dh_min;
      rc = make_im2col_map(&ta.m[nc], dy, d->n, d->p, d->q, cop, ce.base_w, ce.base_h, 1, 1, Hc, Wc, kBlockM, f32); if (rc) return rc;
      Mtot += ce.M; ++nc;
    }
    if (nc == 0) return TP_OK;
    for (int c = nc; c < kMaxCls; ++c) ta.m[c] = ta.m[0];
    p.ncls = nc; p.M = (int)Mtot;
  }
  long long m_tiles = 0;
  for (int c = 0; c < p.ncls; ++c) m_tiles += (p.cls[c].M + kBlockM - 1) / kBlockM;
  const int bn = pick_block_n(m_tiles, p.N);
  rc = make_tiled_map(&tb, wd, (uint64_t)ktot, (uint64_t)d->cin, (uint64_t)ktot, (uint32_t)bn, f32); if (rc) return rc;
  return run_fwd(ta, tb, p, bn, st, f32);
}

int tp_conv_wgrad(const tp_conv_desc* d, const void* x, const void* dy, const void* mask, const void* kmask_f,
                  int cin_real, void* dw, void* db, void* ws, size_t ws_bytes, void* stream) {
  if (!d || !x || !dy || !mask || !dw || !ws) return TP_ERR_INVALID;
  if (d->cin % 8 != 0 || d->cout % 8 != 0 || d->r * d->s > kMaxTaps || cin_real > d->cin) return TP_ERR_UNSUPPORTED;
  if (d->r * d->s > 1 && d->cin % 64 != 0) return TP_ERR_UNSUPPORTED;
  int rc = load_driver_fns(); if (rc) return rc;
  rc = bind_device_of(d ? (const void*)x : nullptr); if (rc) return rc;
  cudaStream_t st = (cudaStream_t)stream;
  const int rs = d->r * d->s;
  WgParams p = {};
  p.Mc = d->cout;
  p.Kpix = d->n * d->p * d->q;
  p.P_it = d->p; p.Q_it = d->q;
  const WgGeom g = wgrad_geom(d);
  p.chunks = g.chunks;
  p.cchunks = (d->cin + 63) / 64;
  p.nb = g.nb;
  p.m_tiles = g.m_tiles;
  p.n_tiles = g.n_tiles;
  p.kblocks = g.kblocks;
  const int sms = sm_count();
  int splits = pick_wgrad_splits(g);
  p.kb_per_split = (p.kblocks + splits - 1) / splits;
  splits = (p.kblocks + p.kb_per_split - 1) / p.kb_per_split;
  p.splits = splits;
  if (ws_bytes < g.partial_bytes(splits)) return TP_ERR_WORKSPACE;
  p.partial = (float*)ws;
  p.kmask = (const uint32_t*)kmask_f; p.kmask_words = (int)tp_kblock_mask_words((int64_t)rs * d->cin);
  fill_taps(p.taps, d->r, d->s, d->cin);
  CUtensorMap ta, tb;
  rc = make_tiled_map(&ta, dy, (uint64_t)d->cout, (uint64_t)p.Kpix, (uint64_t)d->cout, 64); if (rc) return rc;
  if (is_plain_gemm(d)) {
    p.b_mode = 0;
    rc = make_tiled_map(&tb, x, (uint64_t)d->cin, (uint64_t)p.Kpix, (uint64_t)d->cin, 64); if (rc) return rc;
  } else {
    p.b_mode = 1;
    p.base_w = -d->pad_w; p.base_h = -d->pad_h; p.step_w = d->stride_w; p.step_h = d->stride_h;
    rc = make_im2col_map(&tb, x, d->n, d->h, d->w, d->cin, p.base_w, p.base_h, p.step_w, p.step_h, d->p, d->q, 64);
    if (rc) return rc;
  }
  const int items = p.m_tiles * p.n_tiles * splits;
  const int grid = items < sms ? items : sms;
  switch (p.nb) {
    case 1: rc = launch_wgrad<1>(grid, ta, tb, p, st); break;
    case 2: rc = launch_wgrad<2>(grid, ta, tb, p, st); break;
    case 3: rc = launch_wgrad<3>(grid, ta, tb, p, st); break;
    default: rc = launch_wgrad<4>(grid, ta, tb, p, st); break;
  }
  if (rc) return rc;
  const int sl = splits >= 64 ? 8 : (splits >= 32 ? 4 : (splits >= 16 ? 2 : 1));
  const int fin_kt = 256 / sl;
  launch(k_wgrad_finalize, dim3(d->cout, (rs * d->cin + fin_kt - 1) / fin_kt), 256, 0, st,
      p.partial, (const float*)mask, (float*)dw, d->cout, cin_real, d->cin, rs, p.nb, p.m_tiles, splits, sl,
      p.kmask, p.kmask_words);
  TP_LAUNCH_CHECK();
  if (db) {
    const int c = d->cout, cv = c / 8;
    int tx = 1;
    while (tx < cv && tx < 256) tx <<= 1;
    const int ty = 256 / tx, ctiles = (cv + tx - 1) / tx;
    long long gx = ((long long)p.Kpix + (long long)ty * 4 - 1) / ((long long)ty * 4);
    const long long want = (long long)sms * 4 / ctiles, fit = (long long)(ws_bytes / ((size_t)c * sizeof(float)));
    if (gx > want) gx = want;
    if (gx > fit) gx = fit;
    if (gx < 1) gx = 1;
    if ((((uintptr_t)dy) & 15) != 0) return TP_ERR_INVALID;
    launch(k_colsum_part, dim3((unsigned)gx, (unsigned)ctiles), dim3(tx, ty), 0, st, (const __nv_bfloat16*)dy, (long long)p.Kpix, c, c, (float*)ws);
    launch(k_colsum_fold, (c + 255) / 256, 256, 0, st, (const float*)ws, (int)gx, c, (float*)db);
    TP_LAUNCH_CHECK();
  }
  return TP_OK;
}

}
```

turboprune_b200/csrc/tp_optim.cu:

```cuda
#include "tp_common.cuh"
#include <vector>

namespace tp {

constexpr int kCoT = 8;
constexpr int kSlabFloats = 8192;

template <typename T> __device__ __forceinline__ T to_operand(float v);
template <> __device__ __forceinline__ __nv_bfloat16 to_operand<__nv_bfloat16>(float v) { return __float2bfloat16_rn(v); }
template <> __device__ __forceinline__ float to_operand<float>(float v) { return v; }

template <typename T>
__device__ __forceinline__ void stage_slab(const float* __restrict__ w, const float* __restrict__ mask, int co0, int cout,
                                           int c0, int c1, int cin, int rs, T* __restrict__ wf, int cin_p, int wf_ld,
                                           T* __restrict__ wd, int cout_p, bool zero_pad, float* s_slab,
                                           uint32_t* __restrict__ kmf, int kmf_words, uint32_t* __restrict__ kmd, int kmd_words) {
  const int t = threadIdx.x;
  const int cw = c1 - c0;
  const int per_co = cw * rs;
  const int nco = min(kCoT, cout - co0);
  for (int i = t; i < nco * per_co; i += blockDim.x) {
    const int cl = i / per_co, j = i - cl * per_co;
    const long long gi = ((long long)(co0 + cl) * cin + c0) * rs + j;
    const float mk = mask[gi], prod = mk * w[gi];
    s_slab[i] = prod;
    if (kmf && prod == 0.f && mk != 0.f) {
      const int c = j / rs, tap = j - c * rs, kb = (tap * cin_p + c0 + c) >> 6;
      atomicOr(&kmf[(size_t)(co0 >> 6) * kmf_words + (kb >> 5)], 1u << (kb & 31));
    }
  }
  __syncthreads();
  for (int i = t; i < nco * per_co; i += blockDim.x) {
    const int cl = i / per_co, j = i - cl * per_co;
    const int tap = j / cw, c = j - tap * cw;
    wf[(long long)(co0 + cl) * wf_ld + tap * cin_p + c0 + c] = to_operand<T>(s_slab[cl * per_co + c * rs + tap]);
  }
  if (wd) {
    for (int j = t; j < per_co; j += blockDim.x) {
      const int c = j / rs, tap = j - c * rs;
      float f[kCoT];
#pragma unroll
      for (int cl = 0; cl < kCoT; ++cl) f[cl] = cl < nco ? s_slab[cl * per_co + j] : 0.f;
      T* dst = wd + ((long long)(c0 + c) * rs + (rs - 1 - tap)) * cout_p + co0;
      if (co0 + kCoT <= cout_p) {
        if constexpr (sizeof(T) == 4) {
          reinterpret_cast<float4*>(dst)[0] = make_float4(f[0], f[1], f[2], f[3]);
          reinterpret_cast<float4*>(dst)[1] = make_float4(f[4], f[5], f[6], f[7]);
        } else {
          uint4 v;
          __nv_bfloat162* hv = reinterpret_cast<__nv_bfloat162*>(&v);
#pragma unroll
          for (int q = 0; q < 4; ++q) hv[q] = __floats2bfloat162_rn(f[2 * q], f[2 * q + 1]);
          *reinterpret_cast<uint4*>(dst) = v;
        }
      } else {
        for (int cl = 0; cl < kCoT && co0 + cl < cout_p; ++cl) dst[cl] = to_operand<T>(f[cl]);
      }
    }
  }
  if (kmf || (kmd && wd)) {
    const int warp = t >> 5, lane = t & 31, nwarps = blockDim.x >> 5;
    if (kmf) {
      for (int tap = 0; tap < rs; ++tap) {
        const int col0 = tap * cin_p + c0, col1 = tap * cin_p + c1;
        for (int kb = (col0 >> 6) + warp; kb <= ((col1 - 1) >> 6); kb += nwarps) {
          const int a = max(col0, kb << 6), b = min(col1, (kb + 1) << 6), wdt = b - a;
          bool nz = false;
          for (int e = lane; e < nco * wdt; e += 32) {
            const int cl = e / wdt, c = a + (e - cl * wdt) - tap * cin_p - c0;
            nz |= s_slab[cl * per_co + c * rs + tap] != 0.f;
          }
          if (__any_sync(0xffffffffu, nz) && lane == 0) atomicOr(&kmf[(size_t)(co0 >> 6) * kmf_words + (kb >> 5)], 1u << (kb & 31));
        }
      }
    }
    if (kmd && wd) {
      const int g0 = c0 >> 6, g1 = (c1 - 1) >> 6;
      for (int item = warp; item < rs * (g1 - g0 + 1); item += nwarps) {
        const int tap = item / (g1 - g0 + 1), g = g0 + item % (g1 - g0 + 1);
        const int a = max(c0, g << 6), b = min(c1, (g + 1) << 6), wdt = b - a;
        bool nz = false;
        for (int e = lane; e < nco * wdt; e += 32) {
          const int cl = e / wdt, c = a + (e - cl * wdt) - c0;
          nz |= s_slab[cl * per_co + c * rs + tap] != 0.f;
        }
        const int kb = ((rs - 1 - tap) * cout_p + co0) >> 6;
        if (__any_sync(0xffffffffu, nz) && lane == 0) atomicOr(&kmd[(size_t)g * kmd_words + (kb >> 5)], 1u << (kb & 31));
      }
    }
  }
  if (zero_pad && c0 == 0 && cin_p > cin) {
    const int padw = cin_p - cin;
    for (int i = t; i < nco * padw * rs; i += blockDim.x) {
      const int cl = i / (padw * rs), j = i - cl * (padw * rs);
      const int tap = j / padw, c = j - tap * padw;
      wf[(long long)(co0 + cl) * wf_ld + tap * cin_p + cin + c] = to_operand<T>(0.f);
    }
  }
}

template <typename T>
__global__ void __launch_bounds__(256) k_stage_weights(const float* __restrict__ w, const float* __restrict__ mask,
                                                       int cout, int cin, int rs,
                                                       T* __restrict__ wf, int cin_p,
                                                       T* __restrict__ wd, int cout_p, int wf_ld,
                                                       uint32_t* __restrict__ kmf, int kmf_words,
                                                       uint32_t* __restrict__ kmd, int kmd_words) {
  pdl_enter();
  extern __shared__ float s_slab[];
  const int CC = (cin + gridDim.y - 1) / gridDim.y;
  const int c0 = blockIdx.y * CC;
  const int c1 = min(cin, c0 + CC);
  if (c0 >= c1) return;
  stage_slab(w, mask, blockIdx.x * kCoT, cout, c0, c1, cin, rs, wf, cin_p, wf_ld, wd, cout_p, true, s_slab, kmf, kmf_words, kmd, kmd_words);
}

struct StageItem {
  const float* w; const float* mask; __nv_bfloat16* wf; __nv_bfloat16* wd;
  int cout, cin, rs, cin_p, cout_p, ysplit, cc, wf_ld;
  long long cta0;
  uint32_t* kmf; uint32_t* kmd;
  int kmf_words, kmd_words;
};

template <typename T>
__global__ void __launch_bounds__(256) k_stage_weights_batched(const StageItem* __restrict__ items, int n_items) {
  pdl_enter();
  extern __shared__ float s_slab[];
  int lo = 0, hi = n_items - 1;
  const long long b = blockIdx.x;
  while (lo < hi) {
    const int mid = (lo + hi + 1) >> 1;
    if (items[mid].cta0 <= b) lo = mid; else hi = mid - 1;
  }
  const StageItem it = items[lo];
  const int local = (int)(b - it.cta0);
  const int ct = local / it.ysplit, y = local - ct * it.ysplit;
  const int c0 = y * it.cc, c1 = min(it.cin, c0 + it.cc);
  if (ct * kCoT >= it.cout || c0 >= c1) return;
  stage_slab(it.w, it.mask, ct * kCoT, it.cout, c0, c1, it.cin, it.rs, reinterpret_cast<T*>(it.wf), it.cin_p, it.wf_ld,
             reinterpret_cast<T*>(it.wd), it.cout_p, false, s_slab, it.kmf, it.kmf_words, it.kmd, it.kmd_words);
}

__device__ __forceinline__ void kmask_count_empty(uint32_t* km, int rows, int words, int kblocks) {
  __shared__ unsigned int s_n;
  if (threadIdx.x == 0) s_n = 0;
  __syncthreads();
  unsigned int n = 0;
  for (int i = threadIdx.x; i < rows * words; i += blockDim.x) {
    const int wi = i % words;
    const int valid = min(32, kblocks - wi * 32);
    const uint32_t vm = valid >= 32 ? 0xffffffffu : ((1u << valid) - 1u);
    n += __popc(~km[i] & vm);
  }
  if (n) atomicAdd(&s_n, n);
  __syncthreads();
  if (threadIdx.x == 0) km[(size_t)rows * words] = s_n;
  __syncthreads();
}

__global__ void __launch_bounds__(256) k_kmask_summary(const StageItem* __restrict__ items, int n_items) {
  pdl_enter();
  const StageItem it = items[blockIdx.x];
  if (it.kmf) kmask_count_empty(it.kmf, (it.cout + 63) / 64, it.kmf_words, (it.wf_ld + 63) / 64);
  if (it.kmd && it.wd) kmask_count_empty(it.kmd, (it.cin + 63) / 64, it.kmd_words, (it.rs * it.cout_p + 63) / 64);
}

__global__ void __launch_bounds__(256) k_kmask_summary1(uint32_t* kmf, int rows_f, int words_f, int kb_f,
                                                         uint32_t* kmd, int rows_d, int words_d, int kb_d) {
  pdl_enter();
  if (kmf) kmask_count_empty(kmf, rows_f, words_f, kb_f);
  if (kmd) kmask_count_empty(kmd, rows_d, words_d, kb_d);
}

__global__ void k_zero_bf16(__nv_bfloat16* p, long long n) {
  pdl_enter();
  long long i = blockIdx.x * (long long)blockDim.x + threadIdx.x;
  long long stride = (long long)gridDim.x * blockDim.x;
  for (; i < n; i += stride) p[i] = __float2bfloat16_rn(0.f);
}

template <typename T>
__global__ void __launch_bounds__(256) k_to_nhwc(const T* __restrict__ src, long long sn, long long sc, long long sh, long long sw,
                                                 int n, int c, int h, int w, __nv_bfloat16* __restrict__ dst, int c_pad) {
  pdl_enter();
  long long total = (long long)n * h * w * c_pad;
  long long i = blockIdx.x * (long long)blockDim.x + threadIdx.x;
  long long stride = (long long)gridDim.x * blockDim.x;
  for (; i < total; i += stride) {
    int ci = (int)(i % c_pad);
    long long pix = i / c_pad;
    int wi = (int)(pix % w);
    long long t2 = pix / w;
    int hi = (int)(t2 % h);
    int ni = (int)(t2 / h);
    float v = 0.f;
    if (ci < c) v = (float)src[ni * sn + ci * sc + hi * sh + wi * sw];
    dst[i] = __float2bfloat16_rn(v);
  }
}

__global__ void __launch_bounds__(256) k_to_nhwc_f32(const float* __restrict__ src, long long sn, long long sc, long long sh, long long sw,
                                                     int n, int c, int h, int w, float* __restrict__ dst, int c_pad) {
  pdl_enter();
  const long long total = (long long)n * h * w * c_pad;
  long long i = blockIdx.x * (long long)blockDim.x + threadIdx.x;
  const long long stride = (long long)gridDim.x * blockDim.x;
  for (; i < total; i += stride) {
    const int ci = (int)(i % c_pad);
    const long long pix = i / c_pad;
    const int wi = (int)(pix % w);
    const long long t2 = pix / w;
    const int hi = (int)(t2 % h), ni = (int)(t2 / h);
    dst[i] = ci < c ? src[ni * sn + ci * sc + hi * sh + wi * sw] : 0.f;
  }
}

__global__ void __launch_bounds__(256) k_wgrad_split3(const float* __restrict__ src, long long sn, long long sc, long long sh, long long sw,
                                                      int n, int c, int h, int w, __nv_bfloat16* __restrict__ dst, int c_pad,
                                                      int lo_block) {
  pdl_enter();
  const long long total = (long long)n * h * w * c_pad;
  long long i = blockIdx.x * (long long)blockDim.x + threadIdx.x;
  const long long stride = (long long)gridDim.x * blockDim.x;
  for (; i < total; i += stride) {
    const int ci = (int)(i % c_pad);
    const long long pix = i / c_pad;
    const int wi = (int)(pix % w);
    const long long t2 = pix / w;
    const int hi_ = (int)(t2 % h), ni = (int)(t2 / h);
    const float v = ci < c ? src[ni * sn + ci * sc + hi_ * sh + wi * sw] : 0.f;
    const __nv_bfloat16 vh = __float2bfloat16_rn(v);
    const __nv_bfloat16 vl = __float2bfloat16_rn(v - __bfloat162float(vh));
#pragma unroll
    for (int b = 0; b < 3; ++b) dst[i + b * total] = b == lo_block ? vl : vh;
  }
}


__global__ void __launch_bounds__(256) k_im2col_c8(const uint4* __restrict__ x, int n, int h, int w,
                                                   int R, int S, int stride_h, int stride_w, int pad_h, int pad_w,
                                                   int P, int Q, uint4* __restrict__ xcol, int kp8) {
  pdl_enter();
  const long long total = (long long)n * P * Q * kp8;
  long long i = blockIdx.x * (long long)blockDim.x + threadIdx.x;
  const long long step = (long long)gridDim.x * blockDim.x;
  for (; i < total; i += step) {
    const int cell = (int)(i % kp8);
    const long long pix = i / kp8;
    uint4 v = make_uint4(0u, 0u, 0u, 0u);
    if (cell < R * S) {
      const int r = cell / S, s = cell - r * S;
      const int q = (int)(pix % Q); const long long t2 = pix / Q;
      const int pp = (int)(t2 % P); const int ni = (int)(t2 / P);
      const int hi = pp * stride_h - pad_h + r, wi = q * stride_w - pad_w + s;
      if (hi >= 0 && hi < h && wi >= 0 && wi < w) v = x[((long long)ni * h + hi) * w + wi];
    }
    xcol[i] = v;
  }
}

template <typename T>
__global__ void __launch_bounds__(256) k_im2col_stem(const T* __restrict__ src, long long sn, long long sc, long long sh, long long sw,
                                                     int n, int c, int h, int w, int R, int S, int cg, int stride_h, int stride_w,
                                                     int pad_h, int pad_w, int P, int Q, uint4* __restrict__ xcol, int kp8) {
  pdl_enter();
  extern __shared__ uint32_t s_col[];
  const int kp = kp8 * 8;
  for (int e = threadIdx.x; e < kp; e += blockDim.x) {
    uint32_t v = 0xFFFFFFFFu;
    const int tap = e / cg, ch = e - tap * cg;
    if (tap < R * S && ch < c) { const int r = tap / S, s_ = tap - r * S; v = ((uint32_t)r << 16) | ((uint32_t)s_ << 8) | (uint32_t)ch; }
    s_col[e] = v;
  }
  __syncthreads();
  const long long total = (long long)n * P * Q * kp8;
  long long i = blockIdx.x * (long long)blockDim.x + threadIdx.x;
  const long long step = (long long)gridDim.x * blockDim.x;
  for (; i < total; i += step) {
    const int cell = (int)(i % kp8);
    const long long pix = i / kp8;
    const int q = (int)(pix % Q); const long long t2 = pix / Q;
    const int pp = (int)(t2 % P); const int ni = (int)(t2 / P);
    const int h0 = pp * stride_h - pad_h, w0 = q * stride_w - pad_w;
    const T* base = src + ni * sn;
    float f[8];
#pragma unroll
    for (int j = 0; j < 8; ++j) {
      const uint32_t cd = s_col[cell * 8 + j];
      const int hi = h0 + (int)(cd >> 16), wi = w0 + (int)((cd >> 8) & 0xFF);
      f[j] = 0.f;
      if (cd != 0xFFFFFFFFu && hi >= 0 && hi < h && wi >= 0 && wi < w) f[j] = (float)base[hi * sh + wi * sw + (long long)(cd & 0xFF) * sc];
    }
    uint4 v;
    __nv_bfloat162* hv = reinterpret_cast<__nv_bfloat162*>(&v);
#pragma unroll
    for (int j = 0; j < 4; ++j) hv[j] = __floats2bfloat162_rn(f[2 * j], f[2 * j + 1]);
    xcol[i] = v;
  }
}

template <typename T, typename TO = __nv_bfloat16>
__global__ void __launch_bounds__(256) k_im2col_stem_rows(const T* __restrict__ src, long long sn, long long sc, long long sh, long long sw,
                                                          int n, int c, int h, int w, int R, int S, int cg, int stride_h, int stride_w,
                                                          int pad_h, int pad_w, int P, int Q, int QS, uint4* __restrict__ xcol, int kp8) {
  pdl_enter();
  constexpr bool kF32 = sizeof(TO) == 4;
  extern __shared__ __align__(16) unsigned short s_patch[];
  float* const s_patch_f = reinterpret_cast<float*>(s_patch);
  const int pw = (QS - 1) * stride_w + S;
  const int pitch = pw * c;
  const int zero_slot = R * pitch;
  const int strips_q = (Q + QS - 1) / QS;
  const long long n_strips = (long long)n * P * strips_q;
  const int cells_per_pass = blockDim.x / kp8 * kp8 > 0 ? blockDim.x / kp8 : 0;
  const int cell = threadIdx.x % kp8, plane = threadIdx.x / kp8;
  const bool worker = plane < cells_per_pass;
  int off[8];
#pragma unroll
  for (int j = 0; j < 8; ++j) {
    const int e = cell * 8 + j, tap = e / cg, ch = e - tap * cg;
    off[j] = zero_slot;
    if (tap < R * S && ch < c) { const int r = tap / S, s_ = tap - r * S; off[j] = r * pitch + s_ * c + ch; }
  }
  for (long long strip = blockIdx.x; strip < n_strips; strip += gridDim.x) {
    const int sq = (int)(strip % strips_q); long long t = strip / strips_q;
    const int pp = (int)(t % P); const int ni = (int)(t / P);
    const int q0 = sq * QS, nq = min(QS, Q - q0);
    const int h0 = pp * stride_h - pad_h, w0 = q0 * stride_w - pad_w;
    __syncthreads();
    const T* base = src + ni * sn;
    const float inv_c = 1.0f / (float)c;
    for (int r = 0; r < R; ++r) {
      const int hh = h0 + r;
      const bool row_in = hh >= 0 && hh < h;
      const T* rowp = base + hh * sh;
      for (int rem = threadIdx.x; rem < pitch; rem += blockDim.x) {
        const int wi = (int)(((float)rem + 0.5f) * inv_c), ch = rem - wi * c;
        const int ww = w0 + wi;
        float v = 0.f;
        if (row_in && ww >= 0 && ww < w) v = (float)rowp[ww * sw + (long long)ch * sc];
        if constexpr (kF32) s_patch_f[r * pitch + rem] = v;
        else s_patch[r * pitch + rem] = __bfloat16_as_ushort(__float2bfloat16_rn(v));
      }
    }
    if constexpr (kF32) { if (threadIdx.x == 0) s_patch_f[zero_slot] = 0.f; }
    else { if (threadIdx.x == 0) s_patch[zero_slot] = 0; }
    __syncthreads();
    if (worker) {
      const long long row0 = ((long long)ni * P + pp) * Q + q0;
      for (int ql = plane; ql < nq; ql += cells_per_pass) {
        const int qo = ql * stride_w * c;
        if constexpr (kF32) {
          float hf[8];
#pragma unroll
          for (int j = 0; j < 8; ++j) hf[j] = s_patch_f[off[j] == zero_slot ? zero_slot : off[j] + qo];
          float4* const dst = reinterpret_cast<float4*>(xcol) + ((row0 + ql) * kp8 + cell) * 2;
          dst[0] = make_float4(hf[0], hf[1], hf[2], hf[3]);
          dst[1] = make_float4(hf[4], hf[5], hf[6], hf[7]);
        } else {
          unsigned short hv[8];
#pragma unroll
          for (int j = 0; j < 8; ++j) hv[j] = s_patch[off[j] == zero_slot ? zero_slot : off[j] + qo];
          uint4 v;
          v.x = hv[0] | ((unsigned)hv[1] << 16); v.y = hv[2] | ((unsigned)hv[3] << 16);
          v.z = hv[4] | ((unsigned)hv[5] << 16); v.w = hv[6] | ((unsigned)hv[7] << 16);
          xcol[(row0 + ql) * kp8 + cell] = v;
        }
      }
    }
  }
}

__global__ void __launch_bounds__(256) k_sgd(const Seg* __restrict__ segs, int n_seg, long long tiles,
                                             const float* __restrict__ lr_p, float mu, float wd, int first) {
  pdl_enter();
  const float lr = *lr_p;
  const int t = threadIdx.x;
  for (long long tile = blockIdx.x; tile < tiles; tile += gridDim.x) {
    const int si = find_seg(segs, n_seg, tile);
    const Seg sg = segs[si];
    const long long base = (tile - sg.tile0) * kTileElems;
    const long long rem = sg.n - base;
    const int n_in = rem < kTileElems ? (int)rem : kTileElems;
    float* wp = const_cast<float*>(sg.w) + base;
    const float* gp = sg.g + base;
    float* bp = sg.buf + base;
    bool vec = n_in == kTileElems && ((((uintptr_t)wp) | ((uintptr_t)gp) | ((uintptr_t)bp)) & 15) == 0;
    if (vec) {
#pragma unroll
      for (int it = 0; it < kTileElems / (256 * 4); ++it) {
        int q = it * 256 + t;
        float4 w = ((const float4*)wp)[q];
        float4 g = ld_stream((const float4*)gp + q);
        float4 b = first ? make_float4(0.f, 0.f, 0.f, 0.f) : ((const float4*)bp)[q];
        float4 d;
        d.x = fmaf(wd, w.x, g.x); d.y = fmaf(wd, w.y, g.y); d.z = fmaf(wd, w.z, g.z); d.w = fmaf(wd, w.w, g.w);
        if (!first) { b.x = __fadd_rn(__fmul_rn(mu, b.x), d.x); b.y = __fadd_rn(__fmul_rn(mu, b.y), d.y); b.z = __fadd_rn(__fmul_rn(mu, b.z), d.z); b.w = __fadd_rn(__fmul_rn(mu, b.w), d.w); }
        else b = d;
        w.x = fmaf(-lr, b.x, w.x); w.y = fmaf(-lr, b.y, w.y); w.z = fmaf(-lr, b.z, w.z); w.w = fmaf(-lr, b.w, w.w);
        ((float4*)bp)[q] = b;
        ((float4*)wp)[q] = w;
      }
    } else {
      for (int i = t; i < n_in; i += 256) {
        float w = wp[i], g = gp[i];
        float d = fmaf(wd, w, g);
        float b = first ? d : __fadd_rn(__fmul_rn(mu, bp[i]), d);
        bp[i] = b;
        wp[i] = fmaf(-lr, b, w);
      }
    }
  }
}

__device__ __forceinline__ float adamw_lerp(float m, float g, float wt, float omw, bool small) {
  return small ? fmaf(wt, __fsub_rn(g, m), m) : fmaf(-__fsub_rn(g, m), omw, g);
}

struct AdamWCoef { float c, w1, omw1, b2, w2, eps, s, b; bool decay, small; };

__device__ __forceinline__ void adamw_elem(float& w, float g, float& m, float& v, const AdamWCoef& k) {
  if (k.decay) w = __fmul_rn(w, k.c);
  m = adamw_lerp(m, g, k.w1, k.omw1, k.small);
  v = fmaf(k.w2, __fmul_rn(g, g), __fmul_rn(v, k.b2));
  const float d = __fdiv_rn(__fadd_rn(__fdiv_rn(__fsqrt_rn(v), k.b), k.eps), k.s);
  w = __fadd_rn(w, __fdiv_rn(m, d));
}

__global__ void k_adamw_count(const Seg* __restrict__ segs, int n_seg) {
  pdl_enter();
  const int i = blockIdx.x * blockDim.x + threadIdx.x;
  if (i < n_seg) {
    float* st = const_cast<float*>(segs[i].m);
    *st = __fadd_rn(*st, 1.f);
  }
}

__global__ void __launch_bounds__(256) k_adamw(const Seg* __restrict__ segs, int n_seg, long long tiles,
                                               const float* __restrict__ inv_lr_p, const float* __restrict__ decay_p,
                                               float b1, float b2, float w1, float w2, float eps) {
  pdl_enter();
  AdamWCoef k;
  const float inv_lr = *inv_lr_p;
  k.decay = decay_p != nullptr;
  k.c = k.decay ? *decay_p : 1.f;
  k.w1 = w1; k.omw1 = __fsub_rn(1.f, w1); k.small = fabsf(w1) < 0.5f;
  k.b2 = b2; k.w2 = w2; k.eps = eps;
  const int t = threadIdx.x;
  for (long long tile = blockIdx.x; tile < tiles; tile += gridDim.x) {
    const int si = find_seg(segs, n_seg, tile);
    const Seg sg = segs[si];
    const float step = *sg.m;
    k.s = __fdiv_rn(1.f, __fmul_rn(__fsub_rn(powf(b1, step), 1.f), inv_lr));
    k.b = __fsqrt_rn(-__fsub_rn(powf(b2, step), 1.f));
    const long long base = (tile - sg.tile0) * kTileElems;
    const long long rem = sg.n - base;
    const int n_in = rem < kTileElems ? (int)rem : kTileElems;
    float* wp = const_cast<float*>(sg.w) + base;
    const float* gp = sg.g + base;
    float* mp = sg.buf + base;
    float* vp = sg.mo + base;
    const bool vec = n_in == kTileElems && ((((uintptr_t)wp) | ((uintptr_t)gp) | ((uintptr_t)mp) | ((uintptr_t)vp)) & 15) == 0;
    if (vec) {
#pragma unroll
      for (int it = 0; it < kTileElems / (256 * 4); ++it) {
        const int q = it * 256 + t;
        float4 w = ((const float4*)wp)[q], m = ((const float4*)mp)[q], v = ((const float4*)vp)[q];
        const float4 g = ld_stream((const float4*)gp + q);
        adamw_elem(w.x, g.x, m.x, v.x, k); adamw_elem(w.y, g.y, m.y, v.y, k);
        adamw_elem(w.z, g.z, m.z, v.z, k); adamw_elem(w.w, g.w, m.w, v.w, k);
        ((float4*)mp)[q] = m;
        ((float4*)vp)[q] = v;
        ((float4*)wp)[q] = w;
      }
    } else {
      for (int i = t; i < n_in; i += 256) {
        float w = wp[i], m = mp[i], v = vp[i];
        adamw_elem(w, gp[i], m, v, k);
        mp[i] = m; vp[i] = v; wp[i] = w;
      }
    }
  }
}

}

using namespace tp;

extern "C" {

size_t tp_kblock_mask_words(int64_t columns) {
  if (columns <= 0) return 0;
  return (size_t)(((columns + 63) / 64 + 31) / 32);
}

int tp_stage_weights(const void* w, const void* mask, int cout, int cin, int r, int s,
                     void* wf, int cin_p, int wf_ld, void* wd, int cout_p, int cin_p2,
                     void* kmask_f, void* kmask_d, void* stream) {
  if (!w || !mask || !wf || cout <= 0 || cin <= 0 || r <= 0 || s <= 0 || cin_p < cin) return TP_ERR_INVALID;
  if (wd && (cout_p < cout || cin_p2 < cin)) return TP_ERR_INVALID;
  if (wf_ld <= 0) wf_ld = r * s * cin_p;
  if (wf_ld < r * s * cin_p) return TP_ERR_INVALID;
  cudaStream_t st = (cudaStream_t)stream;
  const int rs = r * s;
  int max_c = kSlabFloats / (kCoT * rs); if (max_c < 1) return TP_ERR_UNSUPPORTED;
  int ysplit = (cin + max_c - 1) / max_c;
  int cc = (cin + ysplit - 1) / ysplit;
  size_t smem = (size_t)kCoT * cc * rs * sizeof(float);
  if (wd) {
    long long nz = (long long)cin_p2 * rs * cout_p;
    if (cout_p > cout || cin_p2 > cin) {
      launch(k_zero_bf16, (unsigned)min((nz + 255) / 256, (long long)sm_count() * 16), 256, 0, st, (__nv_bfloat16*)wd, nz);
    }
  }
  const int kmf_words = (int)tp_kblock_mask_words(wf_ld), kmd_words = (int)tp_kblock_mask_words((int64_t)rs * cout_p);
  if (kmask_f) TP_CUDA_CHECK(cudaMemsetAsync(kmask_f, 0, ((size_t)((cout + 63) / 64) * kmf_words + 1) * 4, st));
  if (kmask_d && wd) TP_CUDA_CHECK(cudaMemsetAsync(kmask_d, 0, ((size_t)((cin + 63) / 64) * kmd_words + 1) * 4, st));
  dim3 grid((cout + kCoT - 1) / kCoT, ysplit);
  launch(k_stage_weights<__nv_bfloat16>, grid, 256, smem, st, (const float*)w, (const float*)mask, cout, cin, rs,
                                           (__nv_bfloat16*)wf, cin_p, (__nv_bfloat16*)wd, cout_p, wf_ld,
                                           (uint32_t*)kmask_f, kmf_words, (uint32_t*)kmask_d, kmd_words);
  if (kmask_f || (kmask_d && wd))
    launch(k_kmask_summary1, 1, 256, 0, st, (uint32_t*)kmask_f, (cout + 63) / 64, kmf_words, (wf_ld + 63) / 64,
                                         wd ? (uint32_t*)kmask_d : nullptr, (cin + 63) / 64, kmd_words, (rs * cout_p + 63) / 64);
  TP_LAUNCH_CHECK();
  return TP_OK;
}

int tp_stage_weights_f32(const void* w, const void* mask, int cout, int cin, int r, int s,
                         void* wf, int cin_p, int wf_ld, void* wd, int cout_p, void* stream) {
  if (!w || !mask || !wf || cout <= 0 || cin <= 0 || r <= 0 || s <= 0 || cin_p < cin) return TP_ERR_INVALID;
  if (wd && cout_p < cout) return TP_ERR_INVALID;
  if (wf_ld <= 0) wf_ld = r * s * cin_p;
  if (wf_ld < r * s * cin_p) return TP_ERR_INVALID;
  cudaStream_t st = (cudaStream_t)stream;
  const int rs = r * s;
  int max_c = kSlabFloats / (kCoT * rs); if (max_c < 1) return TP_ERR_UNSUPPORTED;
  const int ysplit = (cin + max_c - 1) / max_c;
  const int cc = (cin + ysplit - 1) / ysplit;
  const size_t smem = (size_t)kCoT * cc * rs * sizeof(float);
  if (wd && cout_p > cout) TP_CUDA_CHECK(cudaMemsetAsync(wd, 0, (size_t)cin * rs * cout_p * sizeof(float), st));
  launch(k_stage_weights<float>, dim3((cout + kCoT - 1) / kCoT, ysplit), 256, smem, st, (const float*)w, (const float*)mask,
         cout, cin, rs, (float*)wf, cin_p, (float*)wd, cout_p, wf_ld, (uint32_t*)nullptr, 0, (uint32_t*)nullptr, 0);
  TP_LAUNCH_CHECK();
  return TP_OK;
}

size_t tp_stage_batched_workspace_bytes(int n_items) {
  return n_items > 0 ? (size_t)n_items * sizeof(StageItem) + 512 : 0;
}

static int stage_batched_impl(const tp_stage_item* items, int n_items, int table_cached, void* kmask_all, size_t kmask_bytes,
                              void* ws, size_t ws_bytes, void* stream, bool f32);

int tp_stage_weights_batched(const tp_stage_item* items, int n_items, int table_cached, void* kmask_all, size_t kmask_bytes,
                             void* ws, size_t ws_bytes, void* stream) {
  return stage_batched_impl(items, n_items, table_cached, kmask_all, kmask_bytes, ws, ws_bytes, stream, false);
}

int tp_stage_weights_batched_f32(const tp_stage_item* items, int n_items, int table_cached, void* ws, size_t ws_bytes, void* stream) {
  for (int i = 0; items && i < n_items; ++i)
    if (items[i].kmask_f || items[i].kmask_d) return TP_ERR_INVALID;
  return stage_batched_impl(items, n_items, table_cached, nullptr, 0, ws, ws_bytes, stream, true);
}

static int stage_batched_impl(const tp_stage_item* items, int n_items, int table_cached, void* kmask_all, size_t kmask_bytes,
                              void* ws, size_t ws_bytes, void* stream, bool f32) {
  if (!items || n_items <= 0 || !ws) return TP_ERR_INVALID;
  cudaStream_t st = (cudaStream_t)stream;
  Arena ar(ws, ws_bytes);
  StageItem* d_items = (StageItem*)ar.take(sizeof(StageItem) * n_items);
  if (!d_items) return TP_ERR_WORKSPACE;
  std::vector<StageItem> h(n_items);
  long long cta = 0; size_t smem = 0;
  for (int i = 0; i < n_items; ++i) {
    const tp_stage_item& q = items[i];
    if (!q.w || !q.mask || !q.wf || q.cout <= 0 || q.cin <= 0 || q.r <= 0 || q.s <= 0 || q.cin_p < q.cin) return TP_ERR_INVALID;
    if (q.wd && q.cout_p < q.cout) return TP_ERR_INVALID;
    const int rs = q.r * q.s;
    int max_c = kSlabFloats / (kCoT * rs); if (max_c < 1) return TP_ERR_UNSUPPORTED;
    const int ysplit = (q.cin + max_c - 1) / max_c;
    const int cc = (q.cin + ysplit - 1) / ysplit;
    StageItem& t = h[i];
    t.w = (const float*)q.w; t.mask = (const float*)q.mask; t.wf = (__nv_bfloat16*)q.wf; t.wd = (__nv_bfloat16*)q.wd;
    t.cout = q.cout; t.cin = q.cin; t.rs = rs; t.cin_p = q.cin_p; t.cout_p = q.cout_p; t.ysplit = ysplit; t.cc = cc;
    t.wf_ld = q.wf_ld > 0 ? q.wf_ld : rs * q.cin_p;
    if (t.wf_ld < rs * q.cin_p) return TP_ERR_INVALID;
    t.cta0 = cta;
    t.kmf = (uint32_t*)q.kmask_f; t.kmd = (uint32_t*)q.kmask_d;
    t.kmf_words = (int)tp_kblock_mask_words(t.wf_ld); t.kmd_words = (int)tp_kblock_mask_words((int64_t)rs * q.cout_p);
    cta += (long long)((q.cout + kCoT - 1) / kCoT) * ysplit;
    const size_t need = (size_t)kCoT * cc * rs * sizeof(float);
    if (need > smem) smem = need;
  }
  if (cta > 0x7fffffffll) return TP_ERR_UNSUPPORTED;
  if (!table_cached)
    TP_CUDA_CHECK(cudaMemcpyAsync(d_items, h.data(), sizeof(StageItem) * n_items, cudaMemcpyHostToDevice, st));
  if (kmask_all && kmask_bytes) TP_CUDA_CHECK(cudaMemsetAsync(kmask_all, 0, kmask_bytes, st));
  if (f32) launch(k_stage_weights_batched<float>, (unsigned)cta, 256, smem, st, d_items, n_items);
  else launch(k_stage_weights_batched<__nv_bfloat16>, (unsigned)cta, 256, smem, st, d_items, n_items);
  if (kmask_all && kmask_bytes) launch(k_kmask_summary, n_items, 256, 0, st, d_items, n_items);
  TP_LAUNCH_CHECK();
  return TP_OK;
}

int tp_to_nhwc_bf16(const void* src, int src_dtype, int64_t sn, int64_t sc, int64_t sh, int64_t sw,
                    int n, int c, int h, int w, void* dst, int c_pad, void* stream) {
  if (!src || !dst || n <= 0 || c <= 0 || h <= 0 || w <= 0 || c_pad < c) return TP_ERR_INVALID;
  cudaStream_t st = (cudaStream_t)stream;
  long long total = (long long)n * h * w * c_pad;
  unsigned grid = (unsigned)min((total + 255) / 256, (long long)sm_count() * 32);
  if (src_dtype == 0) launch(k_to_nhwc<float>, grid, 256, 0, st, (const float*)src, sn, sc, sh, sw, n, c, h, w, (__nv_bfloat16*)dst, c_pad);
  else if (src_dtype == 1) launch(k_to_nhwc<__nv_bfloat16>, grid, 256, 0, st, (const __nv_bfloat16*)src, sn, sc, sh, sw, n, c, h, w, (__nv_bfloat16*)dst, c_pad);
  else return TP_ERR_INVALID;
  TP_LAUNCH_CHECK();
  return TP_OK;
}

int tp_to_nhwc_f32(const void* src, int64_t sn, int64_t sc, int64_t sh, int64_t sw,
                   int n, int c, int h, int w, void* dst, int c_pad, void* stream) {
  if (!src || !dst || n <= 0 || c <= 0 || h <= 0 || w <= 0 || c_pad < c) return TP_ERR_INVALID;
  cudaStream_t st = (cudaStream_t)stream;
  const long long total = (long long)n * h * w * c_pad;
  const unsigned grid = (unsigned)min((total + 255) / 256, (long long)sm_count() * 32);
  launch(k_to_nhwc_f32, grid, 256, 0, st, (const float*)src, sn, sc, sh, sw, n, c, h, w, (float*)dst, c_pad);
  TP_LAUNCH_CHECK();
  return TP_OK;
}

int tp_wgrad_split3(const void* src, int64_t sn, int64_t sc, int64_t sh, int64_t sw,
                    int n, int c, int h, int w, void* dst, int c_pad, int lo_block, void* stream) {
  if (!src || !dst || n <= 0 || c <= 0 || h <= 0 || w <= 0 || c_pad < c || lo_block < 0 || lo_block > 2) return TP_ERR_INVALID;
  cudaStream_t st = (cudaStream_t)stream;
  const long long total = (long long)n * h * w * c_pad;
  const unsigned grid = (unsigned)min((total + 255) / 256, (long long)sm_count() * 32);
  launch(k_wgrad_split3, grid, 256, 0, st, (const float*)src, sn, sc, sh, sw, n, c, h, w, (__nv_bfloat16*)dst, c_pad, lo_block);
  TP_LAUNCH_CHECK();
  return TP_OK;
}

int tp_im2col_stem_f32(const void* src, int64_t sn, int64_t sc, int64_t sh, int64_t sw,
                       int n, int c, int h, int w, int r, int s, int cg, int stride_h, int stride_w, int pad_h, int pad_w,
                       int p, int q, void* xcol, int kp, void* stream) {
  if (!src || !xcol || n <= 0 || c <= 0 || c > 8 || cg < c || cg > 8 || kp % 8 != 0 || kp < r * s * cg) return TP_ERR_INVALID;
  if (r > 255 || s > 255 || kp > 8192) return TP_ERR_UNSUPPORTED;
  cudaStream_t st = (cudaStream_t)stream;
  const int QS = q < 128 ? q : 128;
  const int pw = (QS - 1) * stride_w + s;
  const size_t patch = ((size_t)r * pw * c + 8) * sizeof(float);
  if (patch > 80 * 1024 || kp / 8 > 256) return TP_ERR_UNSUPPORTED;
  if (patch > 48 * 1024)
    TP_CUDA_CHECK(cudaFuncSetAttribute(k_im2col_stem_rows<float, float>, cudaFuncAttributeMaxDynamicSharedMemorySize, (int)patch));
  const long long strips = (long long)n * p * ((q + QS - 1) / QS);
  const unsigned g2 = (unsigned)min(strips, (long long)sm_count() * 8);
  launch(k_im2col_stem_rows<float, float>, g2, 256, patch, st, (const float*)src, sn, sc, sh, sw, n, c, h, w, r, s, cg, stride_h,
         stride_w, pad_h, pad_w, p, q, QS, (uint4*)xcol, kp / 8);
  TP_LAUNCH_CHECK();
  return TP_OK;
}

int tp_im2col_c8(const void* x, int n, int h, int w, int r, int s, int stride_h, int stride_w,
                 int pad_h, int pad_w, int p, int q, void* xcol, int kp, void* stream) {
  if (!x || !xcol || n <= 0 || kp % 8 != 0 || kp < r * s * 8) return TP_ERR_INVALID;
  cudaStream_t st = (cudaStream_t)stream;
  const long long total = (long long)n * p * q * (kp / 8);
  unsigned grid = (unsigned)min((total + 255) / 256, (long long)sm_count() * 32);
  launch(k_im2col_c8, grid, 256, 0, st, (const uint4*)x, n, h, w, r, s, stride_h, stride_w, pad_h, pad_w, p, q, (uint4*)xcol, kp / 8);
  TP_LAUNCH_CHECK();
  return TP_OK;
}

int tp_im2col_stem(const void* src, int src_dtype, int64_t sn, int64_t sc, int64_t sh, int64_t sw,
                   int n, int c, int h, int w, int r, int s, int cg, int stride_h, int stride_w, int pad_h, int pad_w,
                   int p, int q, void* xcol, int kp, void* stream) {
  if (!src || !xcol || n <= 0 || c <= 0 || c > 8 || cg < c || cg > 8 || kp % 8 != 0 || kp < r * s * cg) return TP_ERR_INVALID;
  if (r > 255 || s > 255 || kp > 8192) return TP_ERR_UNSUPPORTED;
  cudaStream_t st = (cudaStream_t)stream;
  {
    const int QS = q < 128 ? q : 128;
    const int pw = (QS - 1) * stride_w + s;
    const size_t patch = ((size_t)r * pw * c + 8) * sizeof(unsigned short);
    const char* e = getenv("TP_STEM_IM2COL");
    if (patch <= 40 * 1024 && kp / 8 <= 256 && !(e && e[0] == 'c')) {
      const long long strips = (long long)n * p * ((q + QS - 1) / QS);
      const unsigned g2 = (unsigned)min(strips, (long long)sm_count() * 8);
      if (src_dtype == 0)
        launch(k_im2col_stem_rows<float>, g2, 256, patch, st, (const float*)src, sn, sc, sh, sw, n, c, h, w, r, s, cg, stride_h, stride_w, pad_h, pad_w, p, q, QS, (uint4*)xcol, kp / 8);
      else if (src_dtype == 1)
        launch(k_im2col_stem_rows<__nv_bfloat16>, g2, 256, patch, st, (const __nv_bfloat16*)src, sn, sc, sh, sw, n, c, h, w, r, s, cg, stride_h, stride_w, pad_h, pad_w, p, q, QS, (uint4*)xcol, kp / 8);
      else return TP_ERR_INVALID;
      TP_LAUNCH_CHECK();
      return TP_OK;
    }
  }
  const long long total = (long long)n * p * q * (kp / 8);
  unsigned grid = (unsigned)min((total + 255) / 256, (long long)sm_count() * 32);
  const size_t smem = (size_t)kp * sizeof(uint32_t);
  if (src_dtype == 0)
    launch(k_im2col_stem<float>, grid, 256, smem, st, (const float*)src, sn, sc, sh, sw, n, c, h, w, r, s, cg, stride_h, stride_w, pad_h, pad_w, p, q, (uint4*)xcol, kp / 8);
  else if (src_dtype == 1)
    launch(k_im2col_stem<__nv_bfloat16>, grid, 256, smem, st, (const __nv_bfloat16*)src, sn, sc, sh, sw, n, c, h, w, r, s, cg, stride_h, stride_w, pad_h, pad_w, p, q, (uint4*)xcol, kp / 8);
  else return TP_ERR_INVALID;
  TP_LAUNCH_CHECK();
  return TP_OK;
}

int tp_sgd_momentum(void* const* w, const void* const* g, void* const* buf, const int64_t* numel,
                    int n_seg, const float* lr_dev, float momentum, float weight_decay,
                    int first_step, int table_cached, void* ws, size_t ws_bytes, void* stream) {
  if (!numel || n_seg <= 0 || !lr_dev || !ws) return TP_ERR_INVALID;
  if (!table_cached && (!w || !g || !buf)) return TP_ERR_INVALID;
  cudaStream_t st = (cudaStream_t)stream;
  Arena ar(ws, ws_bytes);
  Seg* d_segs = nullptr; long long tiles = 0;
  if (table_cached) {
    d_segs = (Seg*)ar.take(sizeof(Seg) * n_seg);
    if (!d_segs) return TP_ERR_WORKSPACE;
    for (int i = 0; i < n_seg; ++i) tiles += (numel[i] + kTileElems - 1) / kTileElems;
  } else {
    int rc = upload_segs(ar, (const void* const*)w, g, nullptr, nullptr, buf, numel, n_seg, &d_segs, &tiles, nullptr, st);
    if (rc) return rc;
  }
  if (tiles == 0) return TP_OK;
  long long gmax = (long long)sm_count() * 8;
  launch(k_sgd, (unsigned)(tiles < gmax ? tiles : gmax), 256, 0, st, d_segs, n_seg, tiles, lr_dev, momentum, weight_decay, first_step);
  TP_LAUNCH_CHECK();
  return TP_OK;
}

int tp_adamw(void* const* w, const void* const* g, void* const* exp_avg, void* const* exp_avg_sq, void* const* step,
             const int64_t* numel, int n_seg, const float* inv_lr_dev, const float* decay_dev,
             double beta1, double beta2, double eps, int table_cached, void* ws, size_t ws_bytes, void* stream) {
  if (!numel || n_seg <= 0 || !inv_lr_dev || !ws) return TP_ERR_INVALID;
  if (!table_cached && (!w || !g || !exp_avg || !exp_avg_sq || !step)) return TP_ERR_INVALID;
  cudaStream_t st = (cudaStream_t)stream;
  Arena ar(ws, ws_bytes);
  Seg* d_segs = nullptr; long long tiles = 0;
  if (table_cached) {
    d_segs = (Seg*)ar.take(sizeof(Seg) * n_seg);
    if (!d_segs) return TP_ERR_WORKSPACE;
    for (int i = 0; i < n_seg; ++i) tiles += (numel[i] + kTileElems - 1) / kTileElems;
  } else {
    int rc = upload_segs(ar, (const void* const*)w, g, (const void* const*)step, exp_avg_sq, exp_avg, numel, n_seg,
                         &d_segs, &tiles, nullptr, st);
    if (rc) return rc;
  }
  launch(k_adamw_count, (unsigned)((n_seg + 255) / 256), 256, 0, st, (const Seg*)d_segs, n_seg);
  if (tiles > 0) {
    const long long gmax = (long long)sm_count() * 8;
    launch(k_adamw, (unsigned)(tiles < gmax ? tiles : gmax), 256, 0, st, (const Seg*)d_segs, n_seg, tiles, inv_lr_dev, decay_dev,
           (float)beta1, (float)beta2, (float)(1.0 - beta1), (float)(1.0 - beta2), (float)eps);
  }
  TP_LAUNCH_CHECK();
  return TP_OK;
}

}
```

turboprune_b200/ops.py:

```python
import ctypes
import threading
from contextlib import contextmanager
from ctypes import c_void_p
from typing import Callable, NamedTuple, Optional

import torch

from . import _cabi

_launches = 0


_precision = threading.local()


def current_precision():
    return getattr(_precision, "dtype", torch.bfloat16)


@contextmanager
def compute_precision(dtype):
    if dtype not in (torch.bfloat16, torch.float32):
        raise ValueError(f"compute_precision: bfloat16 or float32, not {dtype}")
    prev = getattr(_precision, "dtype", None)
    _precision.dtype = dtype
    try:
        yield
    finally:
        if prev is None:
            del _precision.dtype
        else:
            _precision.dtype = prev


_dense_grad = threading.local()


def dense_grad_enabled():
    return getattr(_dense_grad, "on", False)


@contextmanager
def dense_weight_grad(on=True):
    prev = dense_grad_enabled()
    _dense_grad.on = bool(on)
    try:
        yield
    finally:
        _dense_grad.on = prev


_ones_cache = {}


def _ones_like_mask(m):
    key = (tuple(m.shape), m.device)
    t = _ones_cache.get(key)
    if t is None:
        t = _ones_cache[key] = torch.ones(m.shape, dtype=torch.float32, device=m.device)
    return t


def _count(n=1):
    global _launches
    _launches += n


def launch_count() -> int:
    return _launches


class KernelTimer:

    def __init__(self):
        self.records = []

    def totals(self):
        out = {}
        for kind, flops, e0, e1 in self.records:
            ms = e0.elapsed_time(e1)
            t = out.setdefault(kind, [0.0, 0.0, 0])
            t[0] += ms; t[1] += flops; t[2] += 1
        return out


_timer = None


def set_timer(timer):
    global _timer
    _timer = timer


class _Timed:
    def __init__(self, kind, desc, cin_real=None):
        self.on = _timer is not None
        if self.on:
            cin = desc.cin if cin_real is None else cin_real
            self.flops = 2.0 * desc.n * desc.p * desc.q * desc.cout * cin * desc.r * desc.s
            self.kind = kind

    def __enter__(self):
        if self.on:
            self.e0 = torch.cuda.Event(enable_timing=True); self.e0.record()

    def __exit__(self, *a):
        if self.on:
            e1 = torch.cuda.Event(enable_timing=True); e1.record()
            _timer.records.append((self.kind, self.flops, self.e0, e1))


_grad_ready_hook = None


def set_grad_ready_hook(fn):
    global _grad_ready_hook
    _grad_ready_hook = fn


def get_grad_ready_hook():
    return _grad_ready_hook


def grad_ready(*slots):
    if _grad_ready_hook is not None:
        for s in slots:
            if s is not None:
                _grad_ready_hook(s.data_ptr())


WGRAD_SIDE_STREAM = False
_wgrad_streams = {}
_wgrad_pending = set()


def set_wgrad_side_stream(on: bool):
    global WGRAD_SIDE_STREAM
    WGRAD_SIDE_STREAM = bool(on)


def _wgrad_stream(device):
    st = _wgrad_streams.get(device.index)
    if st is None:
        st = _wgrad_streams[device.index] = torch.cuda.Stream(device)
    return st


def join_wgrad(device=None):
    for d in _wgrad_pending:
        if device is None or d == device:
            torch.cuda.current_stream(d).wait_stream(_wgrad_stream(d))
    _wgrad_pending.clear()


def _require_cuda(*tensors):
    for t in tensors:
        if t is not None and not t.is_cuda:
            raise RuntimeError("turboprune_b200 kernels need CUDA tensors (H100 / sm_90a); there is no CPU path")


_ws_cache = {}


def _workspace(nbytes: int, device, tag="default") -> torch.Tensor:
    key = (device.index, torch.cuda.current_stream(device).cuda_stream, tag)
    buf = _ws_cache.get(key)
    if buf is None or buf.numel() < nbytes:
        buf = torch.empty(max(int(nbytes), 1 << 16), dtype=torch.uint8, device=device)
        _ws_cache[key] = buf
    return buf


def topk_threshold_mask(ws, ms, k, gs=None, kind=_cabi.TP_SCORE_MAG, write_masks=True):
    lib = _cabi.load()
    _require_cuda(*ws, *ms)
    dev = ws[0].device
    ws = [w.detach().contiguous() for w in ws]
    ms = [m.detach().contiguous() for m in ms]
    gs = None if gs is None else [g.detach().contiguous() for g in gs]
    for t in ws + ms + (gs or []):
        if t.dtype != torch.float32:
            raise TypeError("pruning kernels operate on fp32 weights / masks / grads")
    numel = [w.numel() for w in ws]
    total = sum(numel)
    outs = [torch.empty_like(m) for m in ms] if write_masks else None
    thr = torch.empty((), dtype=torch.float32, device=dev)
    nbytes = lib.tp_topk_workspace_bytes(len(ws), total)
    wsb = _workspace(nbytes, dev, "topk")
    info = (ctypes.c_int64 * 4)()
    with torch.cuda.device(dev):
        rc = lib.tp_topk_threshold_mask(
            _cabi.ptr_array(ws), _cabi.ptr_array(gs), _cabi.ptr_array(ms), _cabi.ptr_array(outs),
            _cabi.i64_array(numel), len(ws), int(k), int(kind), c_void_p(thr.data_ptr()),
            c_void_p(wsb.data_ptr()), wsb.numel(), info, _cabi.stream_ptr(dev))
    if rc == _cabi.TP_ERR_K_RANGE:
        raise RuntimeError(f"kthvalue(): selected number k out of range for dimension 0 (k={k}, N={total})")
    _cabi.check(rc, "tp_topk_threshold_mask")
    _count(1)
    return outs, thr, {"path": int(info[0]), "candidates": int(info[1]), "n_lt": int(info[2]), "nan_thr": bool(info[3])}


class TopKPlan:

    def __init__(self, ws, ms, gs=None, kind=_cabi.TP_SCORE_MAG):
        self.lib = _cabi.load()
        self.dev = ws[0].device
        self.ws = [w.detach().contiguous() for w in ws]
        self.ms = [m.detach().contiguous() for m in ms]
        self.gs = None if gs is None else [g.detach().contiguous() for g in gs]
        self.outs = [torch.empty_like(m) for m in self.ms]
        self.thr = torch.empty((), dtype=torch.float32, device=self.dev)
        self.n = len(self.ws)
        self.total = sum(w.numel() for w in self.ws)
        self.kind = int(kind)
        self.wsb = torch.empty(self.lib.tp_topk_workspace_bytes(self.n, self.total), dtype=torch.uint8, device=self.dev)
        self.args = (_cabi.ptr_array(self.ws), _cabi.ptr_array(self.gs), _cabi.ptr_array(self.ms), _cabi.ptr_array(self.outs),
                     _cabi.i64_array([w.numel() for w in self.ws]))
        self.info = (ctypes.c_int64 * 4)()
        self._cached = False

    def enqueue(self, k):
        with torch.cuda.device(self.dev):
            rc = self.lib.tp_topk_enqueue(*self.args, self.n, int(k), self.kind, c_void_p(self.thr.data_ptr()),
                                          c_void_p(self.wsb.data_ptr()), self.wsb.numel(), int(self._cached),
                                          _cabi.stream_ptr(self.dev))
        if rc == _cabi.TP_ERR_K_RANGE:
            raise RuntimeError(f"kthvalue(): selected number k out of range for dimension 0 (k={k}, N={self.total})")
        _cabi.check(rc, "tp_topk_enqueue")
        self._cached = True
        _count(1)

    def finish(self, k):
        with torch.cuda.device(self.dev):
            rc = self.lib.tp_topk_finish(self.args[2], self.args[3], self.args[4], self.n, int(k), self.kind,
                                         c_void_p(self.thr.data_ptr()), c_void_p(self.wsb.data_ptr()), self.wsb.numel(),
                                         self.info, _cabi.stream_ptr(self.dev))
        _cabi.check(rc, "tp_topk_finish")
        return self.outs, self.thr, {"path": int(self.info[0]), "candidates": int(self.info[1]), "n_lt": int(self.info[2]),
                                     "nan_thr": bool(self.info[3])}

    def run(self, k):
        self.enqueue(k)
        return self.finish(k)

    def state(self):
        return topk_state(self.wsb, self.n)


_SELSTATE = ("<QQQQ IIIi II II QQQQ II 8Q", ("k", "n_lt", "n_eq", "n_cand", "lo", "hi", "thr_key", "status", "prefix",
                                           "prefix_mask", "c_lo", "c_hi", "before_lo", "before_hi", "k_rem", "n_cand2",
                                           "barrier", "pad"))


def topk_state(wsb, n_seg):
    import struct
    import numpy as np
    off = (64 * n_seg + 255) // 256 * 256
    raw = wsb[off:off + 256 + 4 * 4 * 2048].cpu().numpy().tobytes()
    fmt, names = _SELSTATE
    vals = struct.unpack_from(fmt.replace(" ", ""), raw, 0)
    st = dict(zip(names, vals[:len(names)]))
    st["t_phase"] = list(vals[len(names):])
    st["hist"] = np.frombuffer(raw, dtype=np.uint32, offset=256).copy()
    return st


def apply_threshold(ws, ms, thr, gs=None, kind=_cabi.TP_SCORE_MAG):
    lib = _cabi.load()
    _require_cuda(*ws, *ms, thr)
    dev = ws[0].device
    ws = [w.detach().contiguous() for w in ws]
    ms = [m.detach().contiguous() for m in ms]
    gs = None if gs is None else [g.detach().contiguous() for g in gs]
    outs = [torch.empty_like(m) for m in ms]
    thr = thr.to(device=dev, dtype=torch.float32).reshape(())
    wsb = _workspace(lib.tp_segtable_workspace_bytes(len(ws)), dev, "seg")
    with torch.cuda.device(dev):
        rc = lib.tp_apply_threshold(_cabi.ptr_array(ws), _cabi.ptr_array(gs), _cabi.ptr_array(ms), _cabi.ptr_array(outs),
                                    _cabi.i64_array([w.numel() for w in ws]), len(ws), int(kind),
                                    c_void_p(thr.data_ptr()), c_void_p(wsb.data_ptr()), wsb.numel(), _cabi.stream_ptr(dev))
    _cabi.check(rc, "tp_apply_threshold")
    _count()
    return outs


def count_zeros(ms):
    lib = _cabi.load()
    _require_cuda(*ms)
    dev = ms[0].device
    ms = [m.detach().contiguous() for m in ms]
    out = torch.empty(len(ms) + 1, dtype=torch.int64, device=dev)
    wsb = _workspace(lib.tp_segtable_workspace_bytes(len(ms)), dev, "seg")
    with torch.cuda.device(dev):
        rc = lib.tp_count_zeros(_cabi.ptr_array(ms), _cabi.i64_array([m.numel() for m in ms]), len(ms),
                                c_void_p(out.data_ptr()), c_void_p(wsb.data_ptr()), wsb.numel(), _cabi.stream_ptr(dev))
    _cabi.check(rc, "tp_count_zeros")
    _count()
    return out


def rigl_select(ws, gs, ms, new_ms, ks):
    lib = _cabi.load()
    _require_cuda(*ws, *gs, *ms, *new_ms)
    for t in list(ws) + list(gs) + list(ms) + list(new_ms):
        if t.dtype != torch.float32 or not t.is_contiguous():
            raise TypeError("rigl_select: contiguous fp32 weights / gradients / masks")
    dev = ws[0].device
    numel = [w.numel() for w in ws]
    if any(t.numel() != n for n, g, m, o in zip(numel, gs, ms, new_ms) for t in (g, m, o)):
        raise ValueError("rigl_select: weight, gradient and mask sizes differ")
    counts = torch.empty(len(ws), 2, dtype=torch.int64, device=dev)
    wsb = _workspace(lib.tp_rigl_workspace_bytes(len(ws), sum(numel)), dev, "rigl")
    with torch.cuda.device(dev):
        rc = lib.tp_rigl_select(_cabi.ptr_array(ws), _cabi.ptr_array(gs), _cabi.ptr_array(ms), _cabi.ptr_array(new_ms),
                                _cabi.i64_array(numel), _cabi.i64_array(ks), len(ws), c_void_p(counts.data_ptr()),
                                c_void_p(wsb.data_ptr()), wsb.numel(), _cabi.stream_ptr(dev))
    _cabi.check(rc, "tp_rigl_select")
    _count(20)
    return counts


def rigl_apply(ms, new_ms, ws, bufs=None):
    lib = _cabi.load()
    _require_cuda(*ms, *new_ms, *ws)
    bufs = [None] * len(ms) if bufs is None else list(bufs)
    for t in list(ms) + list(new_ms) + list(ws) + [b for b in bufs if b is not None]:
        if t.dtype != torch.float32 or not t.is_contiguous():
            raise TypeError("rigl_apply: contiguous fp32 masks / weights / momenta")
    dev = ms[0].device
    wsb = _workspace(lib.tp_segtable_workspace_bytes(len(ms)), dev, "seg")
    with torch.cuda.device(dev):
        rc = lib.tp_rigl_apply(_cabi.ptr_array(ms), _cabi.ptr_array(new_ms), _cabi.ptr_array(ws), _cabi.ptr_array(bufs),
                               _cabi.i64_array([m.numel() for m in ms]), len(ms), c_void_p(wsb.data_ptr()), wsb.numel(),
                               _cabi.stream_ptr(dev))
    _cabi.check(rc, "tp_rigl_apply")
    _count()


def rigl_apply_states(ms, new_ms, ws, states):
    lib = _cabi.load()
    _require_cuda(*ms, *new_ms, *ws)
    states = [list(s) for s in states]
    if any(len(s) != len(ms) for s in states):
        raise ValueError("rigl_apply_states: one state tensor (or None) per layer")
    for t in list(ms) + list(new_ms) + list(ws) + [b for s in states for b in s if b is not None]:
        if t.dtype != torch.float32 or not t.is_contiguous():
            raise TypeError("rigl_apply_states: contiguous fp32 masks / weights / optimizer states")
    dev = ms[0].device
    wsb = _workspace(lib.tp_segtable_workspace_bytes(len(ms) * max(len(states), 1)), dev, "seg")
    flat = [b for s in states for b in s]
    with torch.cuda.device(dev):
        rc = lib.tp_rigl_apply_states(_cabi.ptr_array(ms), _cabi.ptr_array(new_ms), _cabi.ptr_array(ws),
                                      _cabi.ptr_array(flat) if flat else None, len(states),
                                      _cabi.i64_array([m.numel() for m in ms]), len(ms), c_void_p(wsb.data_ptr()),
                                      wsb.numel(), _cabi.stream_ptr(dev))
    _cabi.check(rc, "tp_rigl_apply_states")
    _count()


def sgd_momentum_step(params, grads, bufs, lr_dev, momentum, weight_decay, first_step, table_ws=None, table_cached=False):
    lib = _cabi.load()
    dev = params[0].device
    wsb = table_ws if table_ws is not None else _workspace(lib.tp_segtable_workspace_bytes(len(params)), dev, "seg")
    with torch.cuda.device(dev):
        rc = lib.tp_sgd_momentum(_cabi.ptr_array(params), _cabi.ptr_array(grads), _cabi.ptr_array(bufs),
                                 _cabi.i64_array([p.numel() for p in params]), len(params),
                                 c_void_p(lr_dev.data_ptr()), float(momentum), float(weight_decay), int(bool(first_step)),
                                 int(bool(table_cached)), c_void_p(wsb.data_ptr()), wsb.numel(), _cabi.stream_ptr(dev))
    _cabi.check(rc, "tp_sgd_momentum")
    _count()


def adamw_step(params, grads, exp_avgs, exp_avg_sqs, steps, inv_lr_dev, decay_dev, beta1, beta2, eps, table_ws=None,
               table_cached=False):
    lib = _cabi.load()
    dev = params[0].device
    wsb = table_ws if table_ws is not None else _workspace(lib.tp_segtable_workspace_bytes(len(params)), dev, "seg")
    ptrs = [None] * 5 if table_cached else [_cabi.ptr_array(ts) for ts in (params, grads, exp_avgs, exp_avg_sqs, steps)]
    with torch.cuda.device(dev):
        rc = lib.tp_adamw(*ptrs, _cabi.i64_array([p.numel() for p in params]),
                          len(params), c_void_p(inv_lr_dev.data_ptr()), c_void_p(decay_dev.data_ptr()) if decay_dev is not None else None,
                          float(beta1), float(beta2), float(eps), int(bool(table_cached)), c_void_p(wsb.data_ptr()),
                          wsb.numel(), _cabi.stream_ptr(dev))
    _cabi.check(rc, "tp_adamw")
    _count(2)


def _round_up(x, m):
    return (x + m - 1) // m * m


def make_desc(n, h, w, cin, cout, r, s, stride, padding):
    sh, sw = stride
    ph, pw = padding
    p = (h + 2 * ph - r) // sh + 1
    q = (w + 2 * pw - s) // sw + 1
    return _cabi.ConvDesc(n, h, w, cin, cout, r, s, sh, sw, ph, pw, p, q)


def stem_geometry(cin, r, s):
    cg = cin
    return cg, _round_up(r * s * cg, 8)


KBLOCK_SKIP = True


def set_kblock_skip(on: bool):
    global KBLOCK_SKIP
    KBLOCK_SKIP = bool(on)


def kmask_shapes(cout, cin, r, s, wf_ld, cout_p):
    words = lambda cols: ((cols + 63) // 64 + 31) // 32
    return ((cout + 63) // 64, words(wf_ld)), ((cin + 63) // 64, words(r * s * cout_p))


def kblock_occupancy(kmask, columns):
    kb = (columns + 63) // 64
    rows = kmask_rows(kmask, columns)
    return int(kmask[-1].item()), rows.shape[0] * kb


def stage_weights(weight4d, mask4d, cin_p, need_dgrad, cout_p=None, wf_ld=0, want_kmask=None):
    lib = _cabi.load()
    cout, cin, r, s = weight4d.shape
    dev = weight4d.device
    if wf_ld and wf_ld > r * s * cin_p:
        wf = torch.zeros(cout, wf_ld, dtype=torch.bfloat16, device=dev)
    else:
        wf = torch.empty(cout, r * s * cin_p, dtype=torch.bfloat16, device=dev)
    wd = None
    cout_p = cout if cout_p is None else cout_p
    if need_dgrad:
        wd = torch.empty(cin, r * s * cout_p, dtype=torch.bfloat16, device=dev)
    kf = kd = None
    if KBLOCK_SKIP if want_kmask is None else want_kmask:
        sf, sd = kmask_shapes(cout, cin, r, s, wf.shape[1], cout_p)
        kf = torch.empty(sf[0] * sf[1] + 1, dtype=torch.int32, device=dev)
        kd = torch.empty(sd[0] * sd[1] + 1, dtype=torch.int32, device=dev) if wd is not None else None
    with torch.cuda.device(dev):
        rc = lib.tp_stage_weights(c_void_p(weight4d.data_ptr()), c_void_p(mask4d.data_ptr()), cout, cin, r, s,
                                  c_void_p(wf.data_ptr()), cin_p, int(wf_ld), c_void_p(wd.data_ptr()) if wd is not None else None,
                                  cout_p, cin, c_void_p(kf.data_ptr()) if kf is not None else None,
                                  c_void_p(kd.data_ptr()) if kd is not None else None, _cabi.stream_ptr(dev))
    _cabi.check(rc, "tp_stage_weights")
    _count()
    wf.kmask = kf
    if wd is not None:
        wd.kmask = kd
    return wf, wd


def kmask_rows(kmask, columns):
    words = ((columns + 63) // 64 + 31) // 32
    return kmask[:-1].view(-1, words)


def padded_cin(cin, r, s):
    return _round_up(cin, 64 if r * s > 1 else 8)


class LayerPlan(NamedTuple):
    cin_p: int
    cout_p: int
    has_wd: bool
    wf_ld: int

    @property
    def stem(self):
        return not self.has_wd


def layer_plan(cout, cin, r, s, need_dx=False):
    if cin <= 8 and (cin % 8 != 0 or r * s > 1) and not need_dx:
        cg, kp = stem_geometry(cin, r, s)
        return LayerPlan(cg, cout, False, kp)
    cin_p = padded_cin(cin, r, s)
    return LayerPlan(cin_p, _round_up(cout, 64 if r * s > 1 else 8), True, r * s * cin_p)


def _layer_descs(plan, weight_shape, x_shape, stride, padding):
    cout, cin, r, s = weight_shape
    n, _, h, w = x_shape
    desc = make_desc(n, h, w, plan.cin_p, cout, r, s, stride, padding)
    if plan.stem:
        gdesc = _cabi.ConvDesc(n * desc.p * desc.q, 1, 1, plan.wf_ld, cout, 1, 1, 1, 1, 0, 0, 1, 1)
        return desc, gdesc, gdesc, None
    padded = lambda c: _cabi.ConvDesc(n, h, w, c, plan.cout_p, r, s, desc.stride_h, desc.stride_w, desc.pad_h,
                                      desc.pad_w, desc.p, desc.q)
    wdesc = desc if plan.cout_p == cout else padded(plan.cin_p)
    return desc, desc, wdesc, wdesc if cin == plan.cin_p else padded(cin)


def _shape4(w):
    return tuple(w.shape) if w.dim() == 4 else (w.shape[0], w.shape[1], 1, 1)


class Staged(NamedTuple):
    wf: torch.Tensor
    wd: Optional[torch.Tensor]
    plan: LayerPlan


class _Shadow:

    def __init__(self, layers, dtype):
        dev = layers[0].weight.device
        self.staged = []
        for l in layers:
            w = l.weight
            if not w.is_cuda or w.dtype != torch.float32 or not w.is_contiguous():
                continue
            cout, cin, r, s = _shape4(w)
            plan = layer_plan(cout, cin, r, s)
            wf = torch.zeros(cout, plan.wf_ld, dtype=dtype, device=dev)
            wd = torch.zeros(cin, r * s * plan.cout_p, dtype=dtype, device=dev) if plan.has_wd else None
            self.staged.append((l, Staged(wf, wd, plan)))
        self.kmask_all = None
        if dtype == torch.bfloat16:
            sizes = []
            for l, st in self.staged:
                sf, sd = kmask_shapes(*_shape4(l.weight), st.plan.wf_ld, st.plan.cout_p)
                sizes.append((sf[0] * sf[1] + 1, sd[0] * sd[1] + 1 if st.wd is not None else 0))
            self.kmask_all = torch.zeros(max(sum(f + d for f, d in sizes), 1), dtype=torch.int32, device=dev)
            off = 0
            for (_, st), (f, d) in zip(self.staged, sizes):
                st.wf.kmask = self.kmask_all[off:off + f]
                if st.wd is not None:
                    st.wd.kmask = self.kmask_all[off + f:off + f + d]
                off += f + d
        lib = _cabi.load()
        self.ws = torch.empty(max(int(lib.tp_stage_batched_workspace_bytes(len(layers))), 256), dtype=torch.uint8, device=dev)
        self.key = self.items = None

    def set_table(self, key):
        items = (_cabi.StageItem * len(self.staged))()
        for it, (l, st) in zip(items, self.staged):
            it.w = l.weight.data_ptr(); it.mask = l.mask.data_ptr()
            it.wf = st.wf.data_ptr(); it.wd = st.wd.data_ptr() if st.wd is not None else None
            it.cout, it.cin, it.r, it.s = _shape4(l.weight)
            it.cin_p, it.cout_p, it.wf_ld = st.plan.cin_p, st.plan.cout_p, st.plan.wf_ld
            kf, kd = getattr(st.wf, "kmask", None), getattr(st.wd, "kmask", None)
            it.kmask_f = kf.data_ptr() if kf is not None else None
            it.kmask_d = kd.data_ptr() if kd is not None else None
        self.items, self.key = items, key


class WeightStager:

    def __init__(self, layers):
        self.layers = list(layers)
        self._shadows = {}

    def stage(self):
        lib = _cabi.load()
        for l in self.layers:
            if l.mask.device != l.weight.device or l.mask.dtype != torch.float32 or not l.mask.is_contiguous():
                l.mask = l.mask.to(device=l.weight.device, dtype=torch.float32).contiguous()
        key = tuple((l.weight.data_ptr(), l.mask.data_ptr()) for l in self.layers)
        dtype = current_precision()
        sh = self._shadows.get(dtype)
        if sh is None:
            sh = self._shadows[dtype] = _Shadow(self.layers, dtype)
        cached = key == sh.key
        if not cached:
            sh.set_table(key)
        if not sh.staged:
            return
        dev = self.layers[0].weight.device
        with torch.cuda.device(dev):
            if dtype == torch.bfloat16:
                rc = lib.tp_stage_weights_batched(sh.items, len(sh.staged), int(cached), c_void_p(sh.kmask_all.data_ptr()),
                                                  sh.kmask_all.numel() * 4, c_void_p(sh.ws.data_ptr()), sh.ws.numel(),
                                                  _cabi.stream_ptr(dev))
                _cabi.check(rc, "tp_stage_weights_batched")
            else:
                rc = lib.tp_stage_weights_batched_f32(sh.items, len(sh.staged), int(cached), c_void_p(sh.ws.data_ptr()),
                                                      sh.ws.numel(), _cabi.stream_ptr(dev))
                _cabi.check(rc, "tp_stage_weights_batched_f32")
        _count()
        for l, st in sh.staged:
            l.__dict__["_tp_staged"] = st

    def shadow(self, dtype=torch.bfloat16):
        sh = self._shadows.get(dtype)
        return list(sh.staged) if sh is not None else []

    def drop(self):
        for l in self.layers:
            l.__dict__.pop("_tp_staged", None)


def skipped_block_report(stager):
    rows, empty, total = [], 0, 0
    for l, st in stager.shadow(torch.bfloat16):
        e, t = kblock_occupancy(st.wf.kmask, st.wf.shape[1])
        rows.append((type(l).__name__, tuple(l.weight.shape), e, t))
        empty += e; total += t
    return {"empty_blocks": empty, "total_blocks": total, "fraction": empty / max(total, 1), "layers": rows}


def take_staged(layer):
    st = layer.__dict__.pop("_tp_staged", None)
    return st if st is not None and st.wf.dtype == current_precision() else None


def to_nhwc_bf16(x, c_pad):
    lib = _cabi.load()
    n, c, h, w = x.shape
    if x.dtype == torch.bfloat16 and c == c_pad and x.permute(0, 2, 3, 1).is_contiguous():
        return x.permute(0, 2, 3, 1)
    if x.dtype not in (torch.float32, torch.bfloat16):
        x = x.float()
    out = torch.empty(n, h, w, c_pad, dtype=torch.bfloat16, device=x.device)
    sn, sc, sh, sw = x.stride()
    with torch.cuda.device(x.device):
        rc = lib.tp_to_nhwc_bf16(c_void_p(x.data_ptr()), 0 if x.dtype == torch.float32 else 1, sn, sc, sh, sw,
                                 n, c, h, w, c_void_p(out.data_ptr()), c_pad, _cabi.stream_ptr(x.device))
    _cabi.check(rc, "tp_to_nhwc_bf16")
    _count()
    return out


def empty_cl(n, c, h, w, device, dtype=torch.bfloat16):
    return torch.empty((n, c, h, w), dtype=dtype, device=device, memory_format=torch.channels_last)


def im2col_stem(x, desc, kp, cg):
    lib = _cabi.load()
    n, c, h, w = x.shape
    if x.dtype not in (torch.float32, torch.bfloat16):
        x = x.float()
    out = torch.empty(n * desc.p * desc.q, kp, dtype=torch.bfloat16, device=x.device)
    sn, sc, sh, sw = x.stride()
    with torch.cuda.device(x.device):
        rc = lib.tp_im2col_stem(c_void_p(x.data_ptr()), 0 if x.dtype == torch.float32 else 1, sn, sc, sh, sw, n, c, h, w,
                                desc.r, desc.s, cg, desc.stride_h, desc.stride_w, desc.pad_h, desc.pad_w, desc.p, desc.q,
                                c_void_p(out.data_ptr()), kp, _cabi.stream_ptr(x.device))
    _cabi.check(rc, "tp_im2col_stem")
    _count()
    return out


def conv_fprop(desc, x_nhwc, wf, bias=None, out=None, want_stats=False):
    lib = _cabi.load()
    dev = x_nhwc.device
    y = out if out is not None else torch.empty(desc.n, desc.p, desc.q, desc.cout, dtype=torch.bfloat16, device=dev)
    stats = None
    if want_stats:
        stats = torch.empty(int(lib.tp_conv_stats_rows(ctypes.byref(desc))), 2, desc.cout, dtype=torch.float32, device=dev)
    with torch.cuda.device(dev), _Timed("fprop", desc):
        km = getattr(wf, "kmask", None) if KBLOCK_SKIP else None
        rc = lib.tp_conv_fprop_stats(ctypes.byref(desc), c_void_p(x_nhwc.data_ptr()), c_void_p(wf.data_ptr()),
                                     c_void_p(km.data_ptr()) if km is not None else None,
                                     c_void_p(bias.data_ptr()) if bias is not None else None, c_void_p(y.data_ptr()),
                                     c_void_p(stats.data_ptr()) if stats is not None else None,
                                     None, 0, _cabi.stream_ptr(dev))
    _cabi.check(rc, "tp_conv_fprop")
    _count()
    return (y, stats) if want_stats else y


def conv_dgrad(desc, dy_nhwc, wd, addend=None, kmask=None):
    lib = _cabi.load()
    dev = dy_nhwc.device
    dx = torch.empty(desc.n, desc.h, desc.w, desc.cin, dtype=torch.bfloat16, device=dev)
    with torch.cuda.device(dev), _Timed("dgrad", desc):
        km = (kmask if kmask is not None else getattr(wd, "kmask", None)) if KBLOCK_SKIP else None
        rc = lib.tp_conv_dgrad(ctypes.byref(desc), c_void_p(dy_nhwc.data_ptr()), c_void_p(wd.data_ptr()),
                               c_void_p(km.data_ptr()) if km is not None else None,
                               c_void_p(addend.data_ptr()) if addend is not None else None,
                               c_void_p(dx.data_ptr()), None, 0, _cabi.stream_ptr(dev))
    _cabi.check(rc, "tp_conv_dgrad")
    _count(1 if desc.stride_h == 1 and desc.stride_w == 1 else desc.stride_h * desc.stride_w)
    return dx


BN_BWD_FUSION = True


def set_bn_bwd_fusion(on: bool):
    global BN_BWD_FUSION
    BN_BWD_FUSION = bool(on)


def conv_dgrad_bnrelu(desc, dy_nhwc, wd, bn_src, kmask=None):
    lib = _cabi.load()
    dev = dy_nhwc.device
    y, weight, bias, mean, invstd = bn_src[:5]
    g = torch.empty(desc.n, desc.h, desc.w, desc.cin, dtype=torch.bfloat16, device=dev)
    rows = int(lib.tp_conv_dgrad_partial_rows(ctypes.byref(desc)))
    partial = torch.empty(rows, 2, desc.cin, dtype=torch.float32, device=dev)
    km = (kmask if kmask is not None else getattr(wd, "kmask", None)) if KBLOCK_SKIP else None
    P = lambda t: c_void_p(t.data_ptr()) if t is not None else None
    with torch.cuda.device(dev), _Timed("dgrad", desc):
        rc = lib.tp_conv_dgrad_bnrelu(ctypes.byref(desc), P(dy_nhwc), P(wd), P(km), P(y), P(weight), P(bias), P(mean), P(invstd),
                                      P(g), P(partial), _cabi.stream_ptr(dev))
    if rc == -5:
        return None
    _cabi.check(rc, "tp_conv_dgrad_bnrelu")
    _count()
    return g, partial


def conv_wgrad(desc, x_nhwc, dy_nhwc, mask4d, cin_real, want_db=False, dw_out=None, db_out=None, kmask=None):
    lib = _cabi.load()
    dev = x_nhwc.device
    dw = dw_out if dw_out is not None else torch.empty(desc.cout, cin_real, desc.r, desc.s, dtype=torch.float32, device=dev)
    db = (db_out if db_out is not None else torch.empty(desc.cout, dtype=torch.float32, device=dev)) if want_db else None
    nbytes = lib.tp_conv_workspace_bytes(ctypes.byref(desc), 2)
    wsb = _workspace(nbytes, dev, "wgrad")
    with torch.cuda.device(dev), _Timed("wgrad", desc):
        km = kmask if KBLOCK_SKIP else None
        rc = lib.tp_conv_wgrad(ctypes.byref(desc), c_void_p(x_nhwc.data_ptr()), c_void_p(dy_nhwc.data_ptr()),
                               c_void_p(mask4d.data_ptr()), c_void_p(km.data_ptr()) if km is not None else None,
                               cin_real, c_void_p(dw.data_ptr()),
                               c_void_p(db.data_ptr()) if db is not None else None,
                               c_void_p(wsb.data_ptr()), wsb.numel(), _cabi.stream_ptr(dev))
    _cabi.check(rc, "tp_conv_wgrad")
    _count(3 if want_db else 2)
    return dw, db


def stage_weights_f32(weight4d, mask4d, cin_p, need_dgrad, cout_p=None, wf_ld=0):
    lib = _cabi.load()
    cout, cin, r, s = weight4d.shape
    dev = weight4d.device
    wf = torch.zeros(cout, wf_ld, dtype=torch.float32, device=dev) if wf_ld and wf_ld > r * s * cin_p else \
        torch.empty(cout, r * s * cin_p, dtype=torch.float32, device=dev)
    cout_p = cout if cout_p is None else cout_p
    wd = torch.empty(cin, r * s * cout_p, dtype=torch.float32, device=dev) if need_dgrad else None
    with torch.cuda.device(dev):
        rc = lib.tp_stage_weights_f32(c_void_p(weight4d.data_ptr()), c_void_p(mask4d.data_ptr()), cout, cin, r, s,
                                      c_void_p(wf.data_ptr()), cin_p, int(wf_ld), c_void_p(wd.data_ptr()) if wd is not None else None,
                                      cout_p, _cabi.stream_ptr(dev))
    _cabi.check(rc, "tp_stage_weights_f32")
    _count()
    return wf, wd


def to_nhwc_f32(x, c_pad):
    n, c, h, w = x.shape
    if x.dtype != torch.float32:
        raise TypeError(f"to_nhwc_f32: fp32 input expected, got {x.dtype}")
    if c == c_pad and x.permute(0, 2, 3, 1).is_contiguous():
        return x.permute(0, 2, 3, 1)
    lib = _cabi.load()
    out = torch.empty(n, h, w, c_pad, dtype=torch.float32, device=x.device)
    sn, sc, sh, sw = x.stride()
    with torch.cuda.device(x.device):
        rc = lib.tp_to_nhwc_f32(c_void_p(x.data_ptr()), sn, sc, sh, sw, n, c, h, w, c_void_p(out.data_ptr()), c_pad,
                                _cabi.stream_ptr(x.device))
    _cabi.check(rc, "tp_to_nhwc_f32")
    _count()
    return out


def im2col_stem_f32(x, desc, kp, cg):
    lib = _cabi.load()
    n, c, h, w = x.shape
    out = torch.empty(n * desc.p * desc.q, kp, dtype=torch.float32, device=x.device)
    sn, sc, sh, sw = x.stride()
    with torch.cuda.device(x.device):
        rc = lib.tp_im2col_stem_f32(c_void_p(x.data_ptr()), sn, sc, sh, sw, n, c, h, w, desc.r, desc.s, cg, desc.stride_h,
                                    desc.stride_w, desc.pad_h, desc.pad_w, desc.p, desc.q, c_void_p(out.data_ptr()), kp,
                                    _cabi.stream_ptr(x.device))
    _cabi.check(rc, "tp_im2col_stem_f32")
    _count()
    return out


def conv_fprop_f32(desc, x_nhwc, wf, bias=None, out=None):
    lib = _cabi.load()
    dev = x_nhwc.device
    y = out if out is not None else torch.empty(desc.n, desc.p, desc.q, desc.cout, dtype=torch.float32, device=dev)
    with torch.cuda.device(dev), _Timed("fprop", desc):
        rc = lib.tp_conv_fprop_f32(ctypes.byref(desc), c_void_p(x_nhwc.data_ptr()), c_void_p(wf.data_ptr()),
                                   c_void_p(bias.data_ptr()) if bias is not None else None, c_void_p(y.data_ptr()),
                                   _cabi.stream_ptr(dev))
    _cabi.check(rc, "tp_conv_fprop_f32")
    _count()
    return y


def conv_dgrad_f32(desc, dy_nhwc, wd):
    lib = _cabi.load()
    dev = dy_nhwc.device
    dx = torch.empty(desc.n, desc.h, desc.w, desc.cin, dtype=torch.float32, device=dev)
    with torch.cuda.device(dev), _Timed("dgrad", desc):
        rc = lib.tp_conv_dgrad_f32(ctypes.byref(desc), c_void_p(dy_nhwc.data_ptr()), c_void_p(wd.data_ptr()),
                                   c_void_p(dx.data_ptr()), _cabi.stream_ptr(dev))
    _cabi.check(rc, "tp_conv_dgrad_f32")
    _count()
    return dx


def wgrad_split3(x, c_pad, lo_block):
    lib = _cabi.load()
    n, c, h, w = x.shape
    out = torch.empty(3 * n, h, w, c_pad, dtype=torch.bfloat16, device=x.device)
    sn, sc, sh, sw = x.stride()
    with torch.cuda.device(x.device):
        rc = lib.tp_wgrad_split3(c_void_p(x.data_ptr()), sn, sc, sh, sw, n, c, h, w, c_void_p(out.data_ptr()), c_pad, int(lo_block),
                                 _cabi.stream_ptr(x.device))
    _cabi.check(rc, "tp_wgrad_split3")
    _count()
    return out


def split_stacks(desc, x, dy, dy_c_pad):
    return wgrad_split3(x, desc.cin, 1), wgrad_split3(dy, dy_c_pad, 2)


def conv_wgrad_f32(desc, xs, dys, mask4d, cin_real, dw_out=None):
    d3 = _cabi.ConvDesc(3 * desc.n, desc.h, desc.w, desc.cin, desc.cout, desc.r, desc.s, desc.stride_h, desc.stride_w,
                        desc.pad_h, desc.pad_w, desc.p, desc.q)
    dw, _ = conv_wgrad(d3, xs, dys, mask4d, cin_real, False, dw_out=dw_out)
    return dw


def _check_f32(x, want_skip, want_stats):
    if want_skip or want_stats:
        raise RuntimeError("masked_conv2d at float32: the skip-gradient and BatchNorm-statistics epilogues exist in bf16 "
                           "only (a float32 model runs unfused)")
    if x.dtype != torch.float32:
        raise TypeError(f"masked layers at float32 need fp32 activations, got {x.dtype}")


class _Precision(NamedTuple):
    act: torch.dtype
    check: Callable
    stage: Callable
    nhwc: Callable
    im2col: Callable
    fprop: Callable
    dy: Callable
    dgrad: Callable
    wgrad_operands: Callable
    wgrad: Callable
    colsum_db: bool


_PRECISIONS = {
    torch.bfloat16: _Precision(
        act=torch.bfloat16, check=lambda x, want_skip, want_stats: None, stage=stage_weights, nhwc=to_nhwc_bf16,
        im2col=im2col_stem, fprop=conv_fprop, dy=to_nhwc_bf16, dgrad=conv_dgrad,
        wgrad_operands=lambda desc, x, dy: (x, dy), wgrad=conv_wgrad, colsum_db=True),
    torch.float32: _Precision(
        act=torch.float32, check=_check_f32, stage=stage_weights_f32, nhwc=to_nhwc_f32, im2col=im2col_stem_f32,
        fprop=conv_fprop_f32, dy=lambda dy, c_pad: dy.float(),
        dgrad=lambda desc, dy, wd, addend, kmask: conv_dgrad_f32(desc, to_nhwc_f32(dy, desc.cout), wd),
        wgrad_operands=lambda desc, x, dy: split_stacks(desc, x, dy, desc.cout),
        wgrad=lambda desc, xs, dys, mask, cin, want_db, dw_out=None, db_out=None, kmask=None:
            (conv_wgrad_f32(desc, xs, dys, mask, cin, dw_out=dw_out), None),
        colsum_db=False),
}


def _on_wgrad_stream(fn, *operands):
    dev = operands[0].device
    side = _wgrad_stream(dev)
    ev = torch.cuda.Event(); ev.record(torch.cuda.current_stream(dev))
    side.wait_event(ev)
    with torch.cuda.stream(side):
        out = fn()
    for t in operands:
        t.record_stream(side)
    _wgrad_pending.add(dev)
    return out


class MaskedConv2dFn(torch.autograd.Function):

    @staticmethod
    def forward(ctx, x, weight, mask, bias, stride, padding, want_skip=False, grad_slots=None, staged=None, want_stats=False,
                bn_src=None):
        _require_cuda(x, weight, mask)
        P = ctx.prec = _PRECISIONS[current_precision()]
        P.check(x, want_skip, want_stats)
        ctx.dense = dense_grad_enabled()
        ctx.set_materialize_grads(False)
        ctx.want_skip = want_skip
        ctx.grad_slots = grad_slots
        cout, cin, r, s = weight.shape
        n = x.shape[0]
        need_dx = ctx.needs_input_grad[0]
        m32 = mask.detach().contiguous()
        plan = ctx.plan = layer_plan(cout, cin, r, s, need_dx)
        desc, fdesc, ctx.wdesc, ctx.xdesc = _layer_descs(plan, weight.shape, x.shape, stride, padding)
        if plan.stem:
            xin = P.im2col(x, desc, plan.wf_ld, plan.cin_p)
        else:
            xin = P.nhwc(x, plan.cin_p)
        if staged is not None and staged.plan == plan:
            wf, wd = staged.wf, staged.wd
        else:
            wf, wd = P.stage(weight.detach().contiguous(), m32, plan.cin_p, need_dx, plan.cout_p,
                             wf_ld=plan.wf_ld if plan.stem else 0)
        y = empty_cl(n, cout, desc.p, desc.q, x.device, P.act)
        stats = None
        if want_stats:
            _, stats = conv_fprop(fdesc, xin, wf, bias, out=y, want_stats=True)
        else:
            P.fprop(fdesc, xin, wf, bias, out=y)
        ctx.bn_src = None
        if (bn_src is not None and BN_BWD_FUSION and need_dx and not want_skip and stride == (1, 1) and plan.cin_p == cin
                and bn_src[0].shape == xin.shape):
            ctx.bn_src = bn_src
        ctx.wd_kmask = getattr(wd, "kmask", None)
        ctx.wf_kmask = getattr(wf, "kmask", None)
        ctx.save_for_backward(xin.view(-1, plan.wf_ld, 1, 1) if plan.stem else xin.permute(0, 3, 1, 2), m32, wd)
        ctx.desc = desc
        ctx.cin = cin
        ctx.has_bias = bias is not None
        ctx.x_dtype = x.dtype
        if want_skip:
            if want_stats:
                ctx.mark_non_differentiable(stats)
                return y, x, stats
            return y, x
        if want_stats:
            ctx.mark_non_differentiable(stats)
            return y, stats
        return y

    @staticmethod
    def backward(ctx, dy, *rest):
        dskip = rest[0] if ctx.want_skip and rest else None
        if dy is None:
            return dskip, None, None, None, None, None, None, None, None, None, None
        P, plan, desc = ctx.prec, ctx.plan, ctx.desc
        cout = desc.cout
        need_dx, need_dw = ctx.needs_input_grad[0], ctx.needs_input_grad[1]
        need_db = ctx.has_bias and ctx.needs_input_grad[3]
        want_db = need_db and P.colsum_db
        dyl = P.dy(dy, plan.cout_p)
        x, m32, wd = ctx.saved_tensors
        dx = dw = db = None
        db_in_slot = False
        if need_dx:
            addend = to_nhwc_bf16(dskip, ctx.cin) if dskip is not None else None
            fused = None
            if ctx.bn_src is not None and addend is None:
                fused = conv_dgrad_bnrelu(ctx.xdesc, dyl, wd, ctx.bn_src, kmask=ctx.wd_kmask)
            if fused is not None:
                g, partial = fused
                from . import fused_norm
                fused_norm.offer_partials(g, partial, ctx.bn_src[5])
                dx = g.permute(0, 3, 1, 2)
            else:
                dx = P.dgrad(ctx.xdesc, dyl, wd, addend, ctx.wd_kmask).permute(0, 3, 1, 2)
            if dx.dtype != ctx.x_dtype:
                dx = dx.to(ctx.x_dtype)
        if need_dw:
            xa, dya = P.wgrad_operands(ctx.wdesc, x, dyl)
            m, kmask = (_ones_like_mask(m32), None) if ctx.dense else (m32, ctx.wf_kmask)
            if plan.stem:
                ones = torch.ones(cout, plan.wf_ld, 1, 1, dtype=torch.float32, device=m32.device)
                dwm, db = P.wgrad(ctx.wdesc, xa, dya, ones, plan.wf_ld, want_db)
                cin, r, s = m32.shape[1:]
                dw = dwm[:, :r * s * cin].reshape(cout, r * s, cin).permute(0, 2, 1).reshape(cout, cin, r, s)
                if not ctx.dense:
                    dw = dw * m32
            elif plan.cout_p != cout:
                m_p = torch.zeros(plan.cout_p, *m.shape[1:], dtype=torch.float32, device=m.device)
                m_p[:cout] = m
                dwp, dbp = P.wgrad(ctx.wdesc, xa, dya, m_p, ctx.cin, want_db)
                dw = dwp[:cout].contiguous()
                db = dbp[:cout].contiguous() if dbp is not None else None
            else:
                ws_, bs_ = ctx.grad_slots if ctx.grad_slots is not None else (None, None)
                dw_out = ws_ if ws_ is not None and ws_.is_contiguous() and ws_.numel() == m.numel() else None
                db_out = bs_ if want_db else None

                def run():
                    out = P.wgrad(ctx.wdesc, xa, dya, m, ctx.cin, want_db, dw_out, db_out, kmask)
                    grad_ready(dw_out, db_out)
                    return out
                if WGRAD_SIDE_STREAM and dw_out is not None and (db_out is not None or not want_db):
                    dw, db = _on_wgrad_stream(run, xa, dya, m)
                else:
                    dw, db = run()
                if dw_out is not None:
                    dw = None
                if db_out is not None:
                    db, db_in_slot = None, True
        if need_db and db is None and not db_in_slot:
            db = dy.float().sum(dim=(0, 2, 3))
        return dx, dw, None, db, None, None, None, None, None, None, None


def masked_conv2d(x, weight, mask, bias=None, stride=(1, 1), padding=(0, 0), want_skip=False, grad_slots=None, staged=None,
                  want_stats=False, bn_src=None):
    return MaskedConv2dFn.apply(x, weight, mask, bias, tuple(stride), tuple(padding), want_skip, grad_slots, staged, want_stats,
                                bn_src)


def masked_linear(x, weight2d, mask2d, bias=None, grad_slots=None, staged=None):
    shp = x.shape
    x2 = x.reshape(-1, shp[-1])
    y = MaskedConv2dFn.apply(x2.view(x2.shape[0], x2.shape[1], 1, 1), weight2d.view(*weight2d.shape, 1, 1),
                             mask2d.view(*mask2d.shape, 1, 1), bias, (1, 1), (0, 0), False, grad_slots, staged)
    return y.reshape(*shp[:-1], weight2d.shape[0])
```

Measured before the change: 6714.

## Gather stem 7x7 im2col in-kernel from packed image for fprop and wgrad

Replaces the materialized im2col buffer for the ResNet stem conv with a compact NHWC4 bf16 image. The forward and weight-gradient implicit-GEMM kernels now build the A/B tiles directly in shared memory from per-thread 7x7 windows. This removes writing and re-reading the large im2col tensor (about 152 columns per output pixel), at the cost of more producer-thread ALU work, extra producer warps in wgrad, and an L2 prefetch. It applies only to the bf16 stem geometry.

```diff
diff --git a/include/turboprune_b200.h b/include/turboprune_b200.h
--- a/include/turboprune_b200.h
+++ b/include/turboprune_b200.h
@@ -118,6 +118,13 @@
 int tp_conv_wgrad(const tp_conv_desc* d, const void* x, const void* dy, const void* mask, const void* kmask_f,
                   int cin_real, void* dw, void* db, void* ws, size_t ws_bytes, void* stream);
 
+int tp_stem_image(const void* src, int src_dtype, int64_t sn, int64_t sc, int64_t sh, int64_t sw,
+                  int n, int c, int h, int w, void* img, void* stream);
+int tp_conv_fprop_stem_stats(const tp_conv_desc* d, const void* img, const void* wf, const void* kmask_f, const void* bias_f32,
+                             void* y, void* stats, void* stream);
+int tp_conv_wgrad_stem(const tp_conv_desc* d, const void* img, const void* dy, const void* mask, void* dw, void* db,
+                       void* ws, size_t ws_bytes, void* stream);
+
 int tp_conv_fprop_f32(const tp_conv_desc* d, const void* x, const void* wf, const void* bias_f32, void* y, void* stream);
 int tp_conv_dgrad_f32(const tp_conv_desc* d, const void* dy, const void* wd, void* dx, void* stream);
 int tp_wgrad_split3(const void* src, int64_t sn, int64_t sc, int64_t sh, int64_t sw,
diff --git a/turboprune_b200/_cabi.py b/turboprune_b200/_cabi.py
--- a/turboprune_b200/_cabi.py
+++ b/turboprune_b200/_cabi.py
@@ -72,6 +72,12 @@
                                    c_void_p, c_void_p, c_void_p, c_void_p, c_size_t, c_void_p]),
     "tp_conv_wgrad": (c_int, [POINTER(ConvDesc), c_void_p, c_void_p, c_void_p, c_void_p, c_int, c_void_p, c_void_p, c_void_p,
                               c_size_t, c_void_p]),
+    "tp_stem_image": (c_int, [c_void_p, c_int, c_int64, c_int64, c_int64, c_int64, c_int, c_int, c_int, c_int, c_void_p,
+                              c_void_p]),
+    "tp_conv_fprop_stem_stats": (c_int, [POINTER(ConvDesc), c_void_p, c_void_p, c_void_p, c_void_p, c_void_p, c_void_p,
+                                         c_void_p]),
+    "tp_conv_wgrad_stem": (c_int, [POINTER(ConvDesc), c_void_p, c_void_p, c_void_p, c_void_p, c_void_p, c_void_p, c_size_t,
+                                   c_void_p]),
     "tp_sgd_momentum": (c_int, [POINTER(c_void_p), POINTER(c_void_p), POINTER(c_void_p), POINTER(c_int64), c_int,
                                 c_void_p, c_float, c_float, c_int, c_int, c_void_p, c_size_t, c_void_p]),
     "tp_segtable_workspace_bytes": (c_size_t, [c_int]),
diff --git a/turboprune_b200/csrc/tp_igemm.cu b/turboprune_b200/csrc/tp_igemm.cu
--- a/turboprune_b200/csrc/tp_igemm.cu
+++ b/turboprune_b200/csrc/tp_igemm.cu
@@ -2,6 +2,7 @@
 #include "tp_ptx.cuh"
 #include <cuda.h>
 #include <mutex>
+#include <type_traits>
 
 namespace tp {
 using namespace ptx;
@@ -24,6 +25,70 @@
 }
 
 struct TapEntry { uint16_t off_w, off_h; int32_t kofs; };
+
+__device__ __forceinline__ void decompose_pixel(int m, int P, int Q, int& n, int& p, int& q) {
+  q = m % Q; int t = m / Q; p = t % P; n = t / P;
+}
+
+constexpr int kStemR = 7, kStemS = 7, kStemC = 3, kStemCols = kStemR * kStemS * kStemC;
+constexpr int kStemK = 152;
+constexpr int kStemKBlocks = (kStemK + 63) / 64;
+
+struct StemSrc { const uint4* img; int h, w; };
+
+template <int R0, int NR>
+__device__ __forceinline__ void stem_load_windows(const StemSrc& src, bool valid, int n, int oh, int ow, uint4 (&win)[NR][4]) {
+  const int iw0 = 2 * ow - 4;
+#pragma unroll
+  for (int rr = 0; rr < NR; ++rr) {
+    const int ih = 2 * oh - 3 + R0 + rr;
+    const bool row_ok = valid && ih >= 0 && ih < src.h;
+    const long long pair0 = ((long long)n * src.h + ih) * (src.w >> 1) + (iw0 >> 1);
+#pragma unroll
+    for (int j = 0; j < 4; ++j) {
+      const int iw = iw0 + 2 * j;
+      win[rr][j] = make_uint4(0u, 0u, 0u, 0u);
+      if (row_ok && iw >= 0 && iw < src.w) win[rr][j] = __ldg(src.img + pair0 + j);
+    }
+  }
+}
+
+__device__ __forceinline__ void stem_prefetch_rows(const StemSrc& src, int first, int last, int P, int Q) {
+  int n0, oh0, ow0, n1, oh1, ow1;
+  decompose_pixel(first, P, Q, n0, oh0, ow0);
+  decompose_pixel(last, P, Q, n1, oh1, ow1);
+  const long long r0 = (long long)n0 * src.h + max(2 * oh0 - 3, 0);
+  const long long r1 = (long long)n1 * src.h + min(2 * oh1 + 3, src.h - 1);
+  const long long row_pairs = src.w >> 1;
+  const uint4* a = src.img + r0 * row_pairs;
+  const uint32_t bytes = (uint32_t)((r1 - r0 + 1) * row_pairs * 16);
+  asm volatile("cp.async.bulk.prefetch.L2.global [%0], %1;" :: "l"(a), "r"(bytes) : "memory");
+}
+
+template <int R0, int NR>
+__device__ __forceinline__ uint32_t stem_col(const uint4 (&win)[NR][4], int col) {
+  if (col >= kStemCols) return 0u;
+  const int tap = col / kStemC, c = col - tap * kStemC, r = tap / kStemS, s = tap - r * kStemS;
+  const int j = s + 1;
+  const uint4& v = win[r - R0][j >> 1];
+  const int word = (j & 1) * 2 + (c >> 1);
+  const uint32_t u = word == 0 ? v.x : word == 1 ? v.y : word == 2 ? v.z : v.w;
+  return (c & 1) ? (u >> 16) : (u & 0xffffu);
+}
+
+template <int KB, int R0, int NR>
+__device__ __forceinline__ void stem_store_block(const uint4 (&win)[NR][4], uint32_t dst_row, int row) {
+#pragma unroll
+  for (int ch = 0; ch < 8; ++ch) {
+    uint32_t wd[4];
+#pragma unroll
+    for (int e = 0; e < 4; ++e) {
+      const int col = KB * 64 + ch * 8 + 2 * e;
+      wd[e] = stem_col<R0, NR>(win, col) | (stem_col<R0, NR>(win, col + 1) << 16);
+    }
+    sts128(dst_row + ((uint32_t)(ch ^ (row & 7)) << 4), make_uint4(wd[0], wd[1], wd[2], wd[3]));
+  }
+}
 
 constexpr int kMaxCls = 4;
 
@@ -58,6 +123,7 @@
   const uint32_t* kmask;
   int kmask_words;
   TapEntry taps[kMaxTaps];
+  StemSrc stem;
 };
 
 __device__ __forceinline__ const uint32_t* live_kmask(const uint32_t* km, int words, int N) {
@@ -96,6 +162,7 @@
   const uint32_t* kmask;
   int kmask_words;
   TapEntry taps[kMaxTaps];
+  StemSrc stem;
 };
 
 struct WgItem {
@@ -121,10 +188,6 @@
   w.set_tile(tile - n_t * p.m_tiles, n_t, p.m_tiles, nb, p.chunks);
   w.kb0 = w.split * p.kb_per_split; w.kb1 = min(p.kblocks, w.kb0 + p.kb_per_split);
   return w;
-}
-
-__device__ __forceinline__ void decompose_pixel(int m, int P, int Q, int& n, int& p, int& q) {
-  q = m % Q; int t = m / Q; p = t % P; n = t / P;
 }
 
 struct AMaps { CUtensorMap m[kMaxCls]; };
@@ -162,7 +225,7 @@
   }
 }
 
-template <int BLOCK_N, bool MULTI, bool BNB, typename T = __nv_bfloat16>
+template <int BLOCK_N, bool MULTI, bool BNB, typename T = __nv_bfloat16, bool GATHER = false>
 __global__ void __launch_bounds__(kFwdThreads, 1)
 k_igemm_fwd(const __grid_constant__ AMaps tmA, const __grid_constant__ CUtensorMap tmB,
             const __grid_constant__ FwdParams p) {
@@ -170,6 +233,7 @@
   static_assert(!BNB || !MULTI, "BatchNorm-backward epilogue: single class");
   constexpr bool kF32 = sizeof(T) == 4;
   static_assert(!kF32 || !BNB, "fp32 operands: no BatchNorm-backward epilogue");
+  static_assert(!GATHER || (!MULTI && !BNB && !kF32), "stem gather: single class, bf16, statistics epilogue");
   constexpr int kKe = 128 / (int)sizeof(T);
   constexpr int kABytes = kBlockM * kBlockK * 2;
   constexpr int kBBytes = BLOCK_N * kBlockK * 2;
@@ -198,9 +262,9 @@
   };
 
   if (threadIdx.x == 0) {
-    for (int j = 0; j < p.ncls; ++j) prefetch_tmap(&tmA.m[j]);
+    if constexpr (!GATHER) for (int j = 0; j < p.ncls; ++j) prefetch_tmap(&tmA.m[j]);
     prefetch_tmap(&tmB);
-    for (int i = 0; i < kStages; ++i) { mbar_init(&full_bar[i], 1); mbar_init(&empty_bar[i], 1); }
+    for (int i = 0; i < kStages; ++i) { mbar_init(&full_bar[i], GATHER ? 129 : 1); mbar_init(&empty_bar[i], 1); }
     mbar_init(&order_bar[0], 1); mbar_init(&order_bar[1], 1);
     fence_mbar_init();
   }
@@ -208,6 +272,40 @@
   pdl_wait();
 
   if (warp < 4) {
+   if constexpr (GATHER) {
+    const int t = threadIdx.x;
+    int stage = 0; uint32_t phase = 0;
+    const uint32_t* const km = live_kmask(p.kmask, p.kmask_words, p.N);
+    for (int w = 0; w < my_items; ++w) {
+      int ci, m_g, n_t; get_tile(w, ci, m_g, n_t);
+      const int m = m_g * kBlockM + t;
+      const bool valid = m < p.M;
+      int n, oh, ow; decompose_pixel(valid ? m : 0, p.cls[0].P_it, p.cls[0].Q_it, n, oh, ow);
+      uint4 win[kStemR][4];
+      stem_load_windows<0, kStemR>(p.stem, valid, n, oh, ow, win);
+      KSkip ks; bool any = false;
+      if (km) ks.begin(km, p.kmask_words, n_t * BLOCK_N, BLOCK_N, p.N);
+      auto block = [&](auto kb_c) {
+        constexpr int KB = decltype(kb_c)::value;
+        if (km && !ks.take(KB, KB == kStemKBlocks - 1, any)) return;
+        any = true;
+        mbar_wait(&empty_bar[stage], phase ^ 1);
+        uint8_t* sA = smem + stage * kStageBytes;
+        if (t == 0) {
+          mbar_arrive_expect_tx(&full_bar[stage], kBBytes);
+          tma_load_2d(sA + kABytes, &tmB, &full_bar[stage], KB * kBlockK, n_t * BLOCK_N);
+        }
+        stem_store_block<KB, 0, kStemR>(win, smem_u32(sA) + (uint32_t)(t * 128), t);
+        fence_proxy_async();
+        mbar_arrive(&full_bar[stage]);
+        if (++stage == kStages) { stage = 0; phase ^= 1; }
+      };
+      static_assert(kStemKBlocks == 3, "stem K walk");
+      block(std::integral_constant<int, 0>{});
+      block(std::integral_constant<int, 1>{});
+      block(std::integral_constant<int, 2>{});
+    }
+   } else {
     setmaxnreg_dec<kFwdProducerRegs>();
     if (threadIdx.x == 0) {
       int stage = 0; uint32_t phase = 0;
@@ -253,8 +351,9 @@
         }
       }
     }
+   }
   } else {
-    setmaxnreg_inc<kFwdConsumerRegs>();
+    if constexpr (!GATHER) setmaxnreg_inc<kFwdConsumerRegs>();
     const int cw = (warp >> 2) - 1;
     const int q = warp & 3;
     const int wtid = threadIdx.x & 127;
@@ -581,11 +680,12 @@
   }
 }
 
-template <int NB>
-__global__ void __launch_bounds__(kThreads, 1)
+template <int NB, bool GATHER = false>
+__global__ void __launch_bounds__(GATHER ? kThreads + 96 : kThreads, 1)
 k_igemm_wgrad(const __grid_constant__ CUtensorMap tmA ,
               const __grid_constant__ CUtensorMap tmB ,
               const __grid_constant__ WgParams p) {
+  static_assert(!GATHER || NB == kStemKBlocks, "stem gather: one N tile of all three chunks");
   constexpr int kABytes = kBlockM * kBlockK * 2;
   constexpr int kChunkBytes = 64 * kBlockK * 2;
   constexpr int kMaxNb = 4;
@@ -602,15 +702,49 @@
   constexpr int ncols = NB * 64;
 
   if (threadIdx.x == 0) {
-    prefetch_tmap(&tmA); prefetch_tmap(&tmB);
-    for (int i = 0; i < kStages; ++i) { mbar_init(&full_bar[i], 1); mbar_init(&empty_bar[i], kConsumers / 128); }
+    prefetch_tmap(&tmA);
+    if constexpr (!GATHER) prefetch_tmap(&tmB);
+    for (int i = 0; i < kStages; ++i) { mbar_init(&full_bar[i], GATHER ? 65 : 1); mbar_init(&empty_bar[i], kConsumers / 128); }
     fence_mbar_init();
   }
   __syncthreads();
   pdl_wait();
   const uint32_t* const km = live_kmask(p.kmask, p.kmask_words, p.Mc);
 
-  if (warp == kProducerWarp) {
+  if (GATHER && warp >= kProducerWarp) {
+    const int u = threadIdx.x - kConsumers;
+    const int row = u & 63, half = u >> 6;
+    int g = 0;
+    for (int item = blockIdx.x; item < items; item += gridDim.x) {
+      const WgItem it = wg_item(p, NB, item);
+      if (km && it.empty(km, p.kmask_words, p.Mc)) continue;
+      for (int kb = it.kb0; kb < it.kb1; ++kb, ++g) {
+        if ((g & 1) != half) continue;
+        const int stage = g % kStages;
+        const uint32_t phase = (uint32_t)((g / kStages) & 1);
+        if (row == 0 && kb + 2 < it.kb1)
+          stem_prefetch_rows(p.stem, (kb + 2) * kBlockK, min((kb + 3) * kBlockK, p.Kpix) - 1, p.P_it, p.Q_it);
+        const int pix = kb * kBlockK + row;
+        const bool valid = pix < p.Kpix;
+        int n, oh, ow; decompose_pixel(valid ? pix : 0, p.P_it, p.Q_it, n, oh, ow);
+        uint4 win[kStemR][4];
+        stem_load_windows<0, kStemR>(p.stem, valid, n, oh, ow, win);
+        mbar_wait(&empty_bar[stage], phase ^ 1);
+        uint8_t* sA = smem + stage * kStageBytes;
+        if (row == 0) {
+          mbar_arrive_expect_tx(&full_bar[stage], kABytes);
+          tma_load_2d(sA, &tmA, &full_bar[stage], it.m_t * kBlockM, kb * kBlockK);
+          tma_load_2d(sA + kChunkBytes, &tmA, &full_bar[stage], it.m_t * kBlockM + 64, kb * kBlockK);
+        }
+        const uint32_t dst = smem_u32(sA + kABytes) + (uint32_t)(row * 128);
+        stem_store_block<0, 0, kStemR>(win, dst, row);
+        stem_store_block<1, 0, kStemR>(win, dst + kChunkBytes, row);
+        stem_store_block<2, 0, kStemR>(win, dst + 2 * kChunkBytes, row);
+        fence_proxy_async();
+        mbar_arrive(&full_bar[stage]);
+      }
+    }
+  } else if (warp == kProducerWarp) {
     if (lane == 0) {
       int stage = 0; uint32_t phase = 0;
       for (int item = blockIdx.x; item < items; item += gridDim.x) {
@@ -926,14 +1060,14 @@
 
 constexpr int kSmemMax = 232448;
 
-template <int BN, bool MULTI, bool BNB = false, typename T = __nv_bfloat16>
+template <int BN, bool MULTI, bool BNB = false, typename T = __nv_bfloat16, bool GATHER = false>
 static int launch_fwd(const AMaps& a, const CUtensorMap& b, FwdParams& p, cudaStream_t st) {
   constexpr int smem = fwd_smem(BN);
   static_assert(smem <= kSmemMax, "fwd smem budget");
   const int n_tiles = (p.N + BN - 1) / BN;
   static bool attr_set = false;
   if (!attr_set) {
-    TP_CUDA_CHECK(cudaFuncSetAttribute(k_igemm_fwd<BN, MULTI, BNB, T>, cudaFuncAttributeMaxDynamicSharedMemorySize, smem));
+    TP_CUDA_CHECK(cudaFuncSetAttribute(k_igemm_fwd<BN, MULTI, BNB, T, GATHER>, cudaFuncAttributeMaxDynamicSharedMemorySize, smem));
     attr_set = true;
   }
   long long ctiles = 0;
@@ -945,7 +1079,7 @@
   }
   if (ctiles > 0x7fffffffll || ctiles <= 0) return TP_ERR_UNSUPPORTED;
   const int grid = (int)(ctiles < sm_count() ? ctiles : sm_count());
-  TP_CUDA_CHECK(launch(k_igemm_fwd<BN, MULTI, BNB, T>, dim3(grid), dim3(kFwdThreads), (size_t)smem, st, a, b, p));
+  TP_CUDA_CHECK(launch(k_igemm_fwd<BN, MULTI, BNB, T, GATHER>, dim3(grid), dim3(kFwdThreads), (size_t)smem, st, a, b, p));
   TP_LAUNCH_CHECK();
   return TP_OK;
 }
@@ -980,15 +1114,15 @@
   return launch_fwd<64, false>(a, b, p, st);
 }
 
-template <int NB>
+template <int NB, bool GATHER = false>
 static int launch_wgrad(int grid, const CUtensorMap& ta, const CUtensorMap& tb, const WgParams& p, cudaStream_t st) {
   constexpr int smem = 4 * (kBlockM * kBlockK * 2 + 4 * 64 * kBlockK * 2) + 1024 + 256;
   static bool attr_set = false;
   if (!attr_set) {
-    TP_CUDA_CHECK(cudaFuncSetAttribute(k_igemm_wgrad<NB>, cudaFuncAttributeMaxDynamicSharedMemorySize, smem));
+    TP_CUDA_CHECK(cudaFuncSetAttribute(k_igemm_wgrad<NB, GATHER>, cudaFuncAttributeMaxDynamicSharedMemorySize, smem));
     attr_set = true;
   }
-  TP_CUDA_CHECK(launch(k_igemm_wgrad<NB>, dim3(grid), dim3(kThreads), (size_t)smem, st, ta, tb, p));
+  TP_CUDA_CHECK(launch(k_igemm_wgrad<NB, GATHER>, dim3(grid), dim3(GATHER ? kThreads + 96 : kThreads), (size_t)smem, st, ta, tb, p));
   TP_LAUNCH_CHECK();
   return TP_OK;
 }
@@ -1181,8 +1315,64 @@
   return run_fwd(ta, tb, p, bn, st, f32);
 }
 
+static bool stem_gather_geometry(const tp_conv_desc* d) {
+  return d->cin == kStemC && d->r == kStemR && d->s == kStemS && d->stride_h == 2 && d->stride_w == 2 && d->pad_h == 3 &&
+         d->pad_w == 3 && d->n > 0 && d->h > 0 && d->w > 0 && d->w % 2 == 0 && d->p == (d->h - 1) / 2 + 1 &&
+         d->q == (d->w - 1) / 2 + 1 && d->cout > 0 && d->cout % 8 == 0 && d->cout <= 64 &&
+         (long long)d->n * d->p * d->q <= 0x7fffffffll;
+}
+
+struct StemWgrad { StemSrc src; int p, q; };
+
+static int conv_wgrad_impl(const tp_conv_desc* d, const void* x, const void* dy, const void* mask, const void* kmask_f,
+                           int cin_real, void* dw, void* db, void* ws, size_t ws_bytes, void* stream, const StemWgrad* stem);
+
 int tp_conv_wgrad(const tp_conv_desc* d, const void* x, const void* dy, const void* mask, const void* kmask_f,
                   int cin_real, void* dw, void* db, void* ws, size_t ws_bytes, void* stream) {
+  return conv_wgrad_impl(d, x, dy, mask, kmask_f, cin_real, dw, db, ws, ws_bytes, stream, nullptr);
+}
+
+int tp_conv_fprop_stem_stats(const tp_conv_desc* d, const void* img, const void* wf, const void* kmask_f, const void* bias_f32,
+                             void* y, void* stats, void* stream) {
+  if (!d || !img || !wf || !y) return TP_ERR_INVALID;
+  if (!stem_gather_geometry(d)) return TP_ERR_UNSUPPORTED;
+  if (((((uintptr_t)img) | ((uintptr_t)y) | ((uintptr_t)stats)) & 15) != 0) return TP_ERR_UNSUPPORTED;
+  int rc = load_driver_fns(); if (rc) return rc;
+  rc = bind_device_of(img); if (rc) return rc;
+  const int kp = kStemK;
+  FwdParams p = {};
+  p.M = d->n * d->p * d->q; p.N = d->cout;
+  p.ncls = 1;
+  ClsEntry& ce = p.cls[0];
+  ce.M = p.M; ce.P_it = d->p; ce.Q_it = d->q; ce.ntaps = 1; ce.tap0 = 0; ce.oah = 0; ce.oaw = 0;
+  p.cchunks = kStemKBlocks;
+  p.out_img_pix = (long long)d->p * d->q; p.out_row_pix = d->q;
+  p.osh = 1; p.osw = 1; p.linear = 1; p.staged_store = 1;
+  p.ldc = d->cout; p.out = (__nv_bfloat16*)y; p.bias = (const float*)bias_f32;
+  p.stats = (float*)stats;
+  p.kmask = (const uint32_t*)kmask_f; p.kmask_words = (int)tp_kblock_mask_words(kp);
+  fill_taps(p.taps, 1, 1, kp);
+  p.stem.img = (const uint4*)img; p.stem.h = d->h; p.stem.w = d->w;
+  AMaps ta = {};
+  CUtensorMap tb;
+  rc = make_tiled_map(&tb, wf, (uint64_t)kp, (uint64_t)d->cout, (uint64_t)kp, 64u); if (rc) return rc;
+  return launch_fwd<64, false, false, __nv_bfloat16, true>(ta, tb, p, (cudaStream_t)stream);
+}
+
+int tp_conv_wgrad_stem(const tp_conv_desc* d, const void* img, const void* dy, const void* mask, void* dw, void* db,
+                       void* ws, size_t ws_bytes, void* stream) {
+  if (!d || !img) return TP_ERR_INVALID;
+  if (!stem_gather_geometry(d)) return TP_ERR_UNSUPPORTED;
+  if ((((uintptr_t)img) & 15) != 0) return TP_ERR_UNSUPPORTED;
+  const int kp = kStemK;
+  const tp_conv_desc g = {d->n * d->p * d->q, 1, 1, kp, d->cout, 1, 1, 1, 1, 0, 0, 1, 1};
+  StemWgrad sw;
+  sw.src.img = (const uint4*)img; sw.src.h = d->h; sw.src.w = d->w; sw.p = d->p; sw.q = d->q;
+  return conv_wgrad_impl(&g, img, dy, mask, nullptr, kp, dw, db, ws, ws_bytes, stream, &sw);
+}
+
+static int conv_wgrad_impl(const tp_conv_desc* d, const void* x, const void* dy, const void* mask, const void* kmask_f,
+                           int cin_real, void* dw, void* db, void* ws, size_t ws_bytes, void* stream, const StemWgrad* stem) {
   if (!d || !x || !dy || !mask || !dw || !ws) return TP_ERR_INVALID;
   if (d->cin % 8 != 0 || d->cout % 8 != 0 || d->r * d->s > kMaxTaps || cin_real > d->cin) return TP_ERR_UNSUPPORTED;
   if (d->r * d->s > 1 && d->cin % 64 != 0) return TP_ERR_UNSUPPORTED;
@@ -1212,7 +1402,10 @@
   fill_taps(p.taps, d->r, d->s, d->cin);
   CUtensorMap ta, tb;
   rc = make_tiled_map(&ta, dy, (uint64_t)d->cout, (uint64_t)p.Kpix, (uint64_t)d->cout, 64); if (rc) return rc;
-  if (is_plain_gemm(d)) {
+  if (stem) {
+    if (p.nb != kStemKBlocks || p.n_tiles != 1) return TP_ERR_UNSUPPORTED;
+    p.stem = stem->src; p.P_it = stem->p; p.Q_it = stem->q;
+  } else if (is_plain_gemm(d)) {
     p.b_mode = 0;
     rc = make_tiled_map(&tb, x, (uint64_t)d->cin, (uint64_t)p.Kpix, (uint64_t)d->cin, 64); if (rc) return rc;
   } else {
@@ -1223,7 +1416,8 @@
   }
   const int items = p.m_tiles * p.n_tiles * splits;
   const int grid = items < sms ? items : sms;
-  switch (p.nb) {
+  if (stem) rc = launch_wgrad<kStemKBlocks, true>(grid, ta, tb, p, st);
+  else switch (p.nb) {
     case 1: rc = launch_wgrad<1>(grid, ta, tb, p, st); break;
     case 2: rc = launch_wgrad<2>(grid, ta, tb, p, st); break;
     case 3: rc = launch_wgrad<3>(grid, ta, tb, p, st); break;
diff --git a/turboprune_b200/csrc/tp_optim.cu b/turboprune_b200/csrc/tp_optim.cu
--- a/turboprune_b200/csrc/tp_optim.cu
+++ b/turboprune_b200/csrc/tp_optim.cu
@@ -297,6 +297,22 @@
 #pragma unroll
     for (int j = 0; j < 4; ++j) hv[j] = __floats2bfloat162_rn(f[2 * j], f[2 * j + 1]);
     xcol[i] = v;
+  }
+}
+
+template <typename T>
+__global__ void __launch_bounds__(256) k_stem_image(const T* __restrict__ src, long long sn, long long sc, long long sh, long long sw,
+                                                    int n, int c, int h, int w, uint2* __restrict__ img) {
+  pdl_enter();
+  const long long total = (long long)n * h * w;
+  const long long step = (long long)gridDim.x * blockDim.x;
+  for (long long i = blockIdx.x * (long long)blockDim.x + threadIdx.x; i < total; i += step) {
+    const int wi = (int)(i % w); const long long t = i / w;
+    const int hi = (int)(t % h); const int ni = (int)(t / h);
+    const T* px = src + ni * sn + hi * sh + wi * sw;
+    unsigned short b[4] = {0, 0, 0, 0};
+    for (int ch = 0; ch < c; ++ch) b[ch] = __bfloat16_as_ushort(__float2bfloat16_rn((float)px[ch * sc]));
+    img[i] = make_uint2((uint32_t)b[0] | ((uint32_t)b[1] << 16), (uint32_t)b[2] | ((uint32_t)b[3] << 16));
   }
 }
 
@@ -706,6 +722,21 @@
   return TP_OK;
 }
 
+int tp_stem_image(const void* src, int src_dtype, int64_t sn, int64_t sc, int64_t sh, int64_t sw,
+                  int n, int c, int h, int w, void* img, void* stream) {
+  if (!src || !img || n <= 0 || c <= 0 || c > 4 || h <= 0 || w <= 0) return TP_ERR_INVALID;
+  cudaStream_t st = (cudaStream_t)stream;
+  const long long total = (long long)n * h * w;
+  const unsigned grid = (unsigned)min((total + 255) / 256, (long long)sm_count() * 32);
+  if (src_dtype == 0)
+    launch(k_stem_image<float>, grid, 256, 0, st, (const float*)src, sn, sc, sh, sw, n, c, h, w, (uint2*)img);
+  else if (src_dtype == 1)
+    launch(k_stem_image<__nv_bfloat16>, grid, 256, 0, st, (const __nv_bfloat16*)src, sn, sc, sh, sw, n, c, h, w, (uint2*)img);
+  else return TP_ERR_INVALID;
+  TP_LAUNCH_CHECK();
+  return TP_OK;
+}
+
 int tp_sgd_momentum(void* const* w, const void* const* g, void* const* buf, const int64_t* numel,
                     int n_seg, const float* lr_dev, float momentum, float weight_decay,
                     int first_step, int table_cached, void* ws, size_t ws_bytes, void* stream) {
diff --git a/turboprune_b200/ops.py b/turboprune_b200/ops.py
--- a/turboprune_b200/ops.py
+++ b/turboprune_b200/ops.py
@@ -643,6 +643,63 @@
     return out
 
 
+def stem_gather_ok(desc, plan):
+    return (plan.stem and plan.cin_p == 3 and plan.wf_ld == 152 and (desc.r, desc.s) == (7, 7) and desc.cin == 3
+            and (desc.stride_h, desc.stride_w, desc.pad_h, desc.pad_w) == (2, 2, 3, 3) and desc.w % 2 == 0
+            and desc.cout % 8 == 0 and desc.cout <= 64 and desc.n * desc.p * desc.q < 2 ** 31)
+
+
+def stem_image(x):
+    lib = _cabi.load()
+    n, c, h, w = x.shape
+    if x.dtype not in (torch.float32, torch.bfloat16):
+        x = x.float()
+    img = torch.empty(n, h, w, 4, dtype=torch.bfloat16, device=x.device)
+    sn, sc, sh, sw = x.stride()
+    with torch.cuda.device(x.device):
+        rc = lib.tp_stem_image(c_void_p(x.data_ptr()), 0 if x.dtype == torch.float32 else 1, sn, sc, sh, sw, n, c, h, w,
+                               c_void_p(img.data_ptr()), _cabi.stream_ptr(x.device))
+    _cabi.check(rc, "tp_stem_image")
+    _count()
+    return img
+
+
+def conv_fprop_stem(desc, img, wf, bias=None, out=None, want_stats=False):
+    lib = _cabi.load()
+    dev = img.device
+    y = out if out is not None else torch.empty(desc.n, desc.p, desc.q, desc.cout, dtype=torch.bfloat16, device=dev)
+    stats = None
+    if want_stats:
+        stats = torch.empty(int(lib.tp_conv_stats_rows(ctypes.byref(desc))), 2, desc.cout, dtype=torch.float32, device=dev)
+    gdesc = _cabi.ConvDesc(desc.n * desc.p * desc.q, 1, 1, wf.shape[1], desc.cout, 1, 1, 1, 1, 0, 0, 1, 1)
+    with torch.cuda.device(dev), _Timed("fprop", gdesc):
+        km = getattr(wf, "kmask", None) if KBLOCK_SKIP else None
+        rc = lib.tp_conv_fprop_stem_stats(ctypes.byref(desc), c_void_p(img.data_ptr()), c_void_p(wf.data_ptr()),
+                                          c_void_p(km.data_ptr()) if km is not None else None,
+                                          c_void_p(bias.data_ptr()) if bias is not None else None, c_void_p(y.data_ptr()),
+                                          c_void_p(stats.data_ptr()) if stats is not None else None, _cabi.stream_ptr(dev))
+    _cabi.check(rc, "tp_conv_fprop_stem_stats")
+    _count()
+    return (y, stats) if want_stats else y
+
+
+def conv_wgrad_stem(desc, img, dy_nhwc, mask, kp, want_db=False):
+    lib = _cabi.load()
+    dev = img.device
+    gdesc = _cabi.ConvDesc(desc.n * desc.p * desc.q, 1, 1, kp, desc.cout, 1, 1, 1, 1, 0, 0, 1, 1)
+    dw = torch.empty(desc.cout, kp, 1, 1, dtype=torch.float32, device=dev)
+    db = torch.empty(desc.cout, dtype=torch.float32, device=dev) if want_db else None
+    wsb = _workspace(lib.tp_conv_workspace_bytes(ctypes.byref(gdesc), 2), dev, "wgrad")
+    with torch.cuda.device(dev), _Timed("wgrad", gdesc):
+        rc = lib.tp_conv_wgrad_stem(ctypes.byref(desc), c_void_p(img.data_ptr()), c_void_p(dy_nhwc.data_ptr()),
+                                    c_void_p(mask.data_ptr()), c_void_p(dw.data_ptr()),
+                                    c_void_p(db.data_ptr()) if db is not None else None,
+                                    c_void_p(wsb.data_ptr()), wsb.numel(), _cabi.stream_ptr(dev))
+    _cabi.check(rc, "tp_conv_wgrad_stem")
+    _count(3 if want_db else 2)
+    return dw, db
+
+
 def conv_fprop(desc, x_nhwc, wf, bias=None, out=None, want_stats=False):
     lib = _cabi.load()
     dev = x_nhwc.device
@@ -889,7 +946,10 @@
         m32 = mask.detach().contiguous()
         plan = ctx.plan = layer_plan(cout, cin, r, s, need_dx)
         desc, fdesc, ctx.wdesc, ctx.xdesc = _layer_descs(plan, weight.shape, x.shape, stride, padding)
-        if plan.stem:
+        ctx.gather = P.act == torch.bfloat16 and stem_gather_ok(desc, plan)
+        if ctx.gather:
+            xin = stem_image(x)
+        elif plan.stem:
             xin = P.im2col(x, desc, plan.wf_ld, plan.cin_p)
         else:
             xin = P.nhwc(x, plan.cin_p)
@@ -900,7 +960,10 @@
                              wf_ld=plan.wf_ld if plan.stem else 0)
         y = empty_cl(n, cout, desc.p, desc.q, x.device, P.act)
         stats = None
-        if want_stats:
+        if ctx.gather:
+            stats = conv_fprop_stem(desc, xin, wf, bias, out=y, want_stats=want_stats)
+            stats = stats[1] if want_stats else None
+        elif want_stats:
             _, stats = conv_fprop(fdesc, xin, wf, bias, out=y, want_stats=True)
         else:
             P.fprop(fdesc, xin, wf, bias, out=y)
@@ -910,7 +973,11 @@
             ctx.bn_src = bn_src
         ctx.wd_kmask = getattr(wd, "kmask", None)
         ctx.wf_kmask = getattr(wf, "kmask", None)
-        ctx.save_for_backward(xin.view(-1, plan.wf_ld, 1, 1) if plan.stem else xin.permute(0, 3, 1, 2), m32, wd)
+        if ctx.gather:
+            xsave = xin
+        else:
+            xsave = xin.view(-1, plan.wf_ld, 1, 1) if plan.stem else xin.permute(0, 3, 1, 2)
+        ctx.save_for_backward(xsave, m32, wd)
         ctx.desc = desc
         ctx.cin = cin
         ctx.has_bias = bias is not None
@@ -958,7 +1025,10 @@
             m, kmask = (_ones_like_mask(m32), None) if ctx.dense else (m32, ctx.wf_kmask)
             if plan.stem:
                 ones = torch.ones(cout, plan.wf_ld, 1, 1, dtype=torch.float32, device=m32.device)
-                dwm, db = P.wgrad(ctx.wdesc, xa, dya, ones, plan.wf_ld, want_db)
+                if ctx.gather:
+                    dwm, db = conv_wgrad_stem(desc, x, dyl, ones, plan.wf_ld, want_db)
+                else:
+                    dwm, db = P.wgrad(ctx.wdesc, xa, dya, ones, plan.wf_ld, want_db)
                 cin, r, s = m32.shape[1:]
                 dw = dwm[:, :r * s * cin].reshape(cout, r * s, cin).permute(0, 2, 1).reshape(cout, cin, r, s)
                 if not ctx.dense:
```

Measured after the change: 6872 (median of 6 runs). +2.4%, better.
